# TencentARC/HOSNeRF

Hardware: AMD Instinct MI355X
Metric: train rays/sec (stage3: forward + losses + backward + gradient all-reduce + Adam; LPIPS term OFF in this line -- stages.stage3_with_lpips carries it) (higher is better)
Workload: dtype f32 (fp16/bf16 hi-lo split MFMA x3, fp32 accumulate)

## Files before the change

hosnerf_amd/_lib.py:

```python
from __future__ import annotations

import ctypes
import os
from ctypes import c_char_p, c_float, c_int, c_int64, c_void_p

import torch

_HERE = os.path.dirname(os.path.abspath(__file__))
LIB_PATH = os.environ.get("HOS_LIB_PATH", os.path.join(_HERE, "lib", "libhosrender.so"))


class HosLibraryError(RuntimeError):
    pass


_P, _I, _F, _L = c_void_p, c_int, c_float, c_int64

PROTOTYPES = {
    "hos_version": [],
    "hos_device_count": [],
    "hos_error_string": [_I],
    "hos_set_gemm_mode": [_I],
    "hos_set_thread_gemm_mode": [_I],
    "hos_get_gemm_mode": [],
    "hos_set_range_flag": [_P],
    "hos_linear_fwd": [_P, _I, _I, _P, _I, _I, _P, _I, _P, _P, _I, _I, _I, _I, _P, _I, _F, _F, _P, _P],
    "hos_linear_fwd_splitk": [_P, _I, _P, _I, _P, _I, _I, _I, _I, _P],
    "hos_linear_fwd_splitk_ws_floats": [_I, _I, _I],
    "hos_linear_fwd_splitk_det": [_P, _I, _P, _I, _P, _I, _P, _I, _I, _I, _I, _P, _L, _P],
    "hos_linear_dgrad": [_P, _I, _P, _I, _I, _P, _I, _P, _I, _I, _I, _I, _P],
    "hos_linear_wgrad": [_P, _I, _P, _I, _P, _I, _P, _I, _I, _I, _I, _P],
    "hos_linear_wgrad_rows": [_P, _I, _P, _I, _P, _I, _P, _I, _I, _I, _I, _P, _P],
    "hos_thin_linear_fwd": [_P, _I, _P, _I, _P, _P, _I, _I, _I, _I, _I, _P, _P],
    "hos_thin_linear_dgrad": [_P, _I, _P, _I, _I, _P, _I, _P, _P, _I, _I, _I, _P],
    "hos_thin_linear_fwd_rows": [_P, _I, _P, _I, _P, _P, _I, _I, _I, _I, _I, _P, _P, _P],
    "hos_thin_linear_dgrad_rows": [_P, _I, _P, _I, _I, _P, _I, _P, _P, _I, _I, _I, _P, _P],
    "hos_canonical_fold_pack": [_P, _I, _P, _P, _I, _P, _P, _I, _I, _I, _I, _P, _P, _P, _P, _P],
    "hos_canonical_fold_unfold": [_P, _P, _P, _P, _P, _I, _P, _I, _P, _I, _I, _I, _I, _P, _P, _P, _P, _P, _P],
    "hos_mlp_bwd_defer": [_I],
    "hos_mlp_bwd_flush": [_P],
    "hos_mlp_bwd_ws_floats": [_I, _I, _I, _I],
    "hos_linear_wgrad_tr": [_P, _I, _P, _I, _P, _I, _P, _I, _I, _I, _P, _L, _P],
    "hos_linear_wgrad_tr_rows": [_P, _I, _P, _I, _P, _I, _P, _I, _I, _I, _P, _L, _P, _P],
    "hos_linear_bwd_fused": [_P, _I, _P, _I, _P, _I, _P, _I, _P, _I, _P, _I, _I, _I, _I, _P, _L, _P, _P],
    "hos_stage1_loss_fwd": [_P, _P, _I, _P, _P, _I, _P, _F, _F, _F, _F, _P, _P],
    "hos_stage1_loss_bwd": [_P, _P, _I, _I, _P, _P, _F, _F, _F, _F, _P, _P, _P, _P],
    "hos_lpips_prep": [_P, _L, _P, _P],
    "hos_im2col3x3": [_P, _I, _I, _I, _I, _P, _I, _P],
    "hos_col2im3x3": [_P, _I, _I, _I, _I, _I, _P, _P, _P],
    "hos_maxpool2x2_fwd": [_P, _I, _I, _I, _I, _P, _P],
    "hos_maxpool2x2_bwd": [_P, _P, _I, _I, _I, _I, _P, _P],
    "hos_lpips_head_fwd": [_P, _P, _I, _I, _I, _F, _P, _P],
    "hos_lpips_head_bwd": [_P, _P, _I, _I, _I, _F, _P, _I, _P, _P],
    "hos_lpips_finish": [_P, _I, _P, _P],
    "hos_lpips_part_floats": [_I],
    "hos_bias_relu": [_P, _P, _L, _I, _P],
    "hos_unpack_patches_fwd": [_P, _P, _P, _F, _L, _P, _P],
    "hos_unpack_patches_bwd": [_P, _P, _L, _F, _F, _F, _P, _P],
    "hos_camera_rays": [_P, _P, _P, _I, _I, _P, _P, _P, _P, _P],
    "hos_rays_aabb": [_P, _P, _L, _P, _P, _P, _P, _P],
    "hos_frame_rays_compact": [_P, _P, _P, _P, _I, _I, _P, _P, _P, _P, _P, _P, _P, _P, _P],
    "hos_frame_paint": [_P, _P, _I, _P, _I, _I, _P, _P, _P],
    "hos_raybank_index": [_P, _I, _I, _I, _P, _L, _P, _P, _P, _P],
    "hos_raybank_gather": [_P, _P, _P, _P, _P, _P, _P, _P, _L, _I, _I, _I, _L, _P, _P, _P, _P, _P, _P, _P],
    "hos_raybank_frame": [_P, _F, _I, _I, _L, _L, _P, _P, _P, _P, _P, _P, _P, _P],
    "hos_deconv3d_col2im": [_P, _P, _I, _I, _F, _I, _P, _P],
    "hos_deconv3d_im2col": [_P, _I, _I, _P, _P],
    "hos_bias_lrelu": [_P, _P, _L, _I, _F, _I, _P],
    "hos_shard_interleave": [_P, _I, _I, _I, _P, _P],
    "hos_deconv3d_dpre": [_P, _P, _L, _I, _F, _I, _P, _P, _P],
    "hos_gemv_ws_floats": [_I, _I],
    "hos_gemv_rowvec": [_P, _P, _I, _I, _I, _P, _I, _F, _I, _P, _P, _P],
    "hos_outer_accum": [_P, _I, _P, _I, _P, _I, _I, _I, _I, _P],
    "hos_split_planes": [_P, _I, _I, _I, _I, _P, _I, _P, _I, _P],
    "hos_linearp_fwd": [_P, _I, _I, _P, _I, _I, _P, _I, _P, _I, _I, _I, _P, _I, _P, _I, _P, _P, _I, _I, _P, _I, _F, _P],
    "hos_split_planes_t_batch": [_I, _P, _P, _P, _P, _P, _P, _P],
    "hos_split_planes2": [_P, _I, _I, _I, _P, _I, _P, _I, _P],
    "hos_planes_rowdot": [_P, _I, _I, _P, _P, _F, _I, _L, _P, _P],
    "hos_planes_rowdot_b": [_P, _I, _I, _P, _P, _F, _I, _L, _P, _P],
    "hos_linearp_fwd_b": [_P, _I, _I, _P, _I, _I, _P, _I, _P, _I, _I, _I, _P, _I, _P, _P, _I, _I, _P, _I, _F, _P],
    "hos_linearp_dgrad": [_P, _I, _P, _I, _I, _P, _I, _P, _I, _I, _P, _I, _P],
    "hos_linearp_wgrad": [_P, _I, _P, _I, _I, _P, _I, _P, _I, _I, _I, _I, _P, _L, _P],
    "hos_resample": [_P, _P, _I, _I, _I, _F, _F, _P, _F, _F, _P, _P, _F, _F, _F, _P, _P, _P, _P],
    "hos_encode_ipe": [_P, _P, _P, _P, _P, _P, _I, _I, _P, _I, _P],
    "hos_encode_ipe_planes": [_P, _P, _P, _P, _P, _P, _I, _I, _P, _P, _I, _P],
    "hos_encode_viewdirs": [_P, _I, _I, _P, _I, _I, _P],
    "hos_alpha_weights_fwd": [_P, _P, _P, _I, _I, _I, _P, _P],
    "hos_alpha_weights_bwd": [_P, _P, _P, _P, _I, _I, _I, _P, _P],
    "hos_volrender_fwd": [_P, _P, _I, _I, _F, _P, _P],
    "hos_volrender_bwd": [_P, _P, _P, _I, _I, _F, _P, _P, _P],
    "hos_interlevel_fwd": [_P, _P, _P, _P, _I, _I, _I, _P, _P, _P, _P],
    "hos_interlevel_bwd": [_P, _P, _P, _P, _I, _I, _I, _F, _P, _P],
    "hos_distortion_fwd": [_P, _P, _I, _I, _P, _P],
    "hos_distortion_bwd": [_P, _P, _I, _I, _F, _P, _P],
    "hos_head_grad": [_P, _P, _P, _P, _I, _F, _P, _I, _I, _P, _I, _P],
    "hos_human_sample_warp": [_P, _P, _P, _P, _P, _P, _P, _P, _P, _I, _P, _P, _I, _I, _I, _P, _P, _P, _P, _P],
    "hos_lbs_forward": [_P, _P, _P, _P, _I, _I, _P, _P, _L, _I, _P, _P, _P],
    "hos_embed_hannw": [_P, _P, _I, _P, _I, _L, _P, _I, _P, _I, _P, _P],
    "hos_embed_fourier": [_P, _I, _P, _I, _L, _P, _I, _P, _I, _P],
    "hos_embed_fourier_rows": [_P, _I, _P, _I, _L, _P, _I, _P, _I, _P, _P],
    "hos_human_sample_warp_bwd": [_P, _P, _P, _P, _I, _P, _P, _L, _I, _P, _P, _P, _P, _P, _P, _P, _P, _P],
    "hos_lbs_forward_bwd": [_P, _P, _P, _P, _I, _I, _P, _P, _L, _I, _P, _P, _P, _P, _P, _P, _P],
    "hos_embed_bwd": [_P, _P, _I, _I, _P, _I, _I, _P, _I, _I, _L, _P, _I, _P, _P],
    "hos_slice_mask": [_P, _I, _I, _P, _I, _I, _L, _I, _P, _I, _P, _P],
    "hos_slice_pad": [_P, _I, _I, _L, _I, _P, _I, _P, _P],
    "hos_rgbsigma_grad": [_P, _P, _L, _P, _I, _P],
    "hos_rgbsigma_grad_rows": [_P, _P, _L, _P, _I, _P, _P],
    "hos_raw2outputs_fwd": [_P, _I, _P, _I, _P, _P, _P, _P, _F, _I, _I, _P, _P, _P, _P, _P],
    "hos_raw2outputs_bwd": [_P, _P, _P, _I, _P, _I, _P, _P, _P, _P, _F, _I, _I, _P, _I, _P, _I, _P, _P],
    "hos_merge_composite_fwd": [_P, _P, _P, _P, _P, _P, _P, _P, _P, _P, _I, _I, _I, _F, _P, _P, _P, _P, _P, _P],
    "hos_merge_composite_maps_fwd": [_P, _P, _P, _P, _P, _P, _P, _P, _P, _P, _I, _I, _I, _F, _P, _P, _P, _P, _P, _P, _P, _P, _P, _P],
    "hos_merge_composite_bwd": [_P, _P, _P, _P, _P, _P, _P, _P, _P, _P, _P, _P, _I, _I, _I, _F, _P, _P, _P, _P, _P],
    "hos_mlp_chain_weight_bytes": [],
    "hos_mlp_chain_aux_floats": [],
    "hos_mlp_chain_pack": [_P, _P, _P, _P, _P, _P],
    "hos_mlp_chain_pack_fold": [_P, _P, _P, _P, _I, _I, _P, _P, _P, _P],
    "hos_mlp_chain_unfold_grad": [_P, _P, _P, _I, _I, _P, _I, _P, _P],
    "hos_mlp_chain128_fwd": [_P, _I, _P, _I, _P, _P, _P, _P, _I, _P, _L, _P, _P],
    "hos_mlp_chain_bwd_steps": [_I],
    "hos_mlp_chain_bwd_image_bytes": [_I, _I],
    "hos_mlp_chain_bwd_ws_floats": [_I, _I],
    "hos_mlp_chain_bwd_pack": [_I, _P, _P, _P, _P, _P, _P, _P, _P],
    "hos_mlp_chain_bwd": [_I, _P, _I, _I, _P, _P, _P, _P, _P, _P, _P, _P, _P, _P, _P, _P, _L, _P],
    "hos_compact_workspace_ints": [],
    "hos_compact_rows": [_P, _F, _P, _P, _L, _P, _P, _P, _P, _P, _P],
    "hos_scatter_rows": [_P, _P, _P, _L, _P, _P],
    "hos_select_live_rays": [_P, _F, _I, _I, _P, _P, _P, _P],
    "hos_gather_rays": [_P, _P, _P, _I, _I, _I, _P, _P],
    "hos_scatter_rays": [_P, _P, _P, _P, _I, _I, _I, _P, _P],
    "hos_pose_refine_saved_floats": [],
    "hos_pose_refine_fwd": [_P, _P, _P, _P, _I, _I, _I, _P, _P, _P, _P],
    "hos_pose_refine_workspace_floats": [],
    "hos_pose_refine_bwd": [_P, _P, _P, _P, _P, _P, _P, _I, _I, _I, _P, _P],
    "hos_motion_basis_fwd": [_P, _P, _P, _I, _I, _P, _P, _P, _P, _P],
    "hos_motion_basis_bwd": [_P, _P, _P, _P, _P, _P, _P, _I, _I, _P, _P, _P],
    "hos_train_losses_workspace_floats": [],
    "hos_train_losses_fwd": [_P, _P, _L, _F, _F, _P, _P, _P, _P, _P, _P, _I, _P, _P, _L, _P, _F, _F, _F, _P, _P, _P],
    "hos_train_losses_bwd": [_P, _P, _P, _P, _L, _F, _P, _P, _P, _P, _P, _P, _I, _P, _P, _L, _P, _F, _F, _F, _P, _P, _P, _P, _P],
    "hos_sumsq": [_P, _L, _P, _P],
    "hos_adam_step": [_P, _P, _P, _P, _L, _F, _F, _F, _F, _I, _F, _P, _F, _P],
    "hos_adam_step_dyn": [_P, _P, _P, _P, _L, _P, _F, _F, _F, _F, _P, _F, _P],
    "hos_rowdot_lrelu_fwd": [_P, _P, _I, _P, _I, _I, _F, _P, _P],
    "hos_rowdot_lrelu_bwd": [_P, _P, _P, _P, _I, _I, _I, _F, _P, _I, _P, _P, _P],
    "hos_volume_softmax_fwd": [_P, _P, _I, _L, _P, _P],
    "hos_volume_softmax_bwd": [_P, _P, _I, _L, _P, _P],
    "hos_volume_channel_last": [_P, _I, _L, _P, _P],
    "hos_volume_pair_bwd": [_P, _P, _I, _I, _L, _P, _P],
    "hos_copy_or_zero_n": [_I, _P, _P, _P, _P],
    "hos_debug_stamp": [_P, _I, _P],
    "hos_clear_last_error": [],
    "hos_add_n": [_I, _P, _L, _P, _P],
    "hos_any_abs_below": [_P, _L, _F, _P, _P],
    "hos_state_embed_grad": [_P, _P, _I, _I, _I, _I, _P, _P, _P],
    "hos_embed_bwd_res": [_P, _P, _I, _I, _P, _I, _I, _P, _I, _I, _L, _P, _P, _P, _P],
    "hos_head_grad_padded": [_P, _P, _P, _P, _I, _F, _P, _I, _I, _P, _I, _P],
    "hos_sumsq_blocks": [],
    "hos_sumsq_partials": [_I, _P, _P, _P, _P],
    "hos_adam_multi": [_I, _P, _P, _P, _P, _P, _P, _P, _I, _F, _F, _F, _F, _P, _F, _P, _P, _P],
    "hos_adam_multi_lazy": [_I, _P, _P, _P, _P, _P, _P, _P, _P, _P, _I, _F, _F, _F, _F, _P, _F, _P, _P, _P],
    "hos_adam_lazy_prepare": [_I, _P, _P, _P, _F, _F, _P, _P],
}
_RESTYPES = {"hos_error_string": c_char_p, "hos_mlp_bwd_ws_floats": c_int64, "hos_train_losses_workspace_floats": c_int64,
             "hos_pose_refine_saved_floats": c_int64, "hos_compact_workspace_ints": c_int64,
             "hos_pose_refine_workspace_floats": c_int64, "hos_mlp_chain_weight_bytes": c_int64,
             "hos_mlp_chain_aux_floats": c_int64, "hos_gemv_ws_floats": c_int64,
             "hos_mlp_chain_bwd_image_bytes": c_int64, "hos_mlp_chain_bwd_ws_floats": c_int64,
             "hos_linear_fwd_splitk_ws_floats": c_int64}

_lib = None


def load() -> ctypes.CDLL:
    global _lib
    if _lib is not None:
        return _lib
    if not os.path.exists(LIB_PATH):
        raise HosLibraryError(
            f"{LIB_PATH} not found: build it with `make` (or `python -c 'import __graft_entry__ as g; g.build()'`). "
            "hosnerf_amd has no CPU fallback.")
    try:
        lib = ctypes.CDLL(LIB_PATH)
    except OSError as e:
        raise HosLibraryError(f"cannot load {LIB_PATH}: {e}") from e
    for name, argtypes in PROTOTYPES.items():
        try:
            fn = getattr(lib, name)
        except AttributeError as e:
            raise HosLibraryError(f"{LIB_PATH} does not export {name}; rebuild the library") from e
        fn.argtypes = argtypes
        fn.restype = _RESTYPES.get(name, c_int)
    _lib = lib
    return lib


def check(code: int, what: str):
    if code != 0:
        msg = load().hos_error_string(int(code))
        raise HosLibraryError(f"{what} failed with code {code}: {msg.decode() if msg else '?'}")


def require_gpu():
    if not torch.cuda.is_available():
        raise HosLibraryError("no HIP device visible: hosnerf_amd ops run on MI355X only (no CPU fallback)")


def stream_ptr() -> int:
    return torch.cuda.current_stream().cuda_stream


def ptr(t, dtype=torch.float32) -> int:
    if t is None:
        return 0
    if not isinstance(t, torch.Tensor):
        raise HosLibraryError(f"expected a tensor, got {type(t)}")
    if not t.is_cuda:
        raise HosLibraryError("hosnerf_amd ops take HIP (device='cuda') tensors only -- there is no CPU path")
    if t.dtype != dtype:
        raise HosLibraryError(f"expected dtype {dtype}, got {t.dtype}")
    if not t.is_contiguous():
        raise HosLibraryError("expected a contiguous tensor")
    return t.data_ptr()


def call(name: str, *args):
    lib = load()
    code = getattr(lib, name)(*args, stream_ptr())
    check(code, name)
```

hosnerf_amd/csrc/hos_compact.hip:

```cpp
#include "hos_common.h"

namespace {

constexpr int CT = 256;
constexpr int CPT = 4;
constexpr int CB = CT * CPT;
constexpr int CMAXB = 4096;

__global__ __launch_bounds__(CT) void compact_count_kernel(const float* mask, float thr, long P, int* blk_off, unsigned int* ticket,
                                                          int* count) {
    __shared__ int sh[CT / 64];
    __shared__ bool last;
    const int tid = threadIdx.x;
    const long base = (long)blockIdx.x * CB + tid * CPT;
    int c = 0;
#pragma unroll
    for (int k = 0; k < CPT; ++k) c += (base + k < P && mask[base + k] > thr) ? 1 : 0;
    for (int o = 32; o > 0; o >>= 1) c += __shfl_xor(c, o, 64);
    if ((tid & 63) == 0) sh[tid >> 6] = c;
    __syncthreads();
    if (tid == 0) {
        int tot = 0;
        for (int w = 0; w < CT / 64; ++w) tot += sh[w];
        blk_off[blockIdx.x] = tot;
        __threadfence();
        last = atomicAdd(ticket, 1u) == gridDim.x - 1;
    }
    __syncthreads();
    if (!last) return;
    __threadfence();
    __shared__ int tsum[CT];
    const int nb = gridDim.x, per = (nb + CT - 1) / CT;
    int loc = 0;
    for (int k = 0; k < per; ++k) {
        const int b = tid * per + k;
        if (b < nb) loc += ((volatile int*)blk_off)[b];
    }
    tsum[tid] = loc;
    __syncthreads();
    if (tid == 0) {
        int run = 0;
        for (int t = 0; t < CT; ++t) { const int v = tsum[t]; tsum[t] = run; run += v; }
        *count = run;
        *ticket = 0u;
    }
    __syncthreads();
    int run = tsum[tid];
    for (int k = 0; k < per; ++k) {
        const int b = tid * per + k;
        if (b < nb) { const int v = ((volatile int*)blk_off)[b]; blk_off[b] = run; run += v; }
    }
}

__global__ __launch_bounds__(CT) void compact_scatter_kernel(const float* mask, float thr, long P, const int* blk_off, const int* count,
                                                            const float* src_a, const float* src_b, int* sel, float* out_a, float* out_b) {
    __shared__ int sh[CT / 64];
    const int tid = threadIdx.x, lane = tid & 63, wave = tid >> 6;
    const long base = (long)blockIdx.x * CB + tid * CPT;
    bool f[CPT];
    int c = 0;
#pragma unroll
    for (int k = 0; k < CPT; ++k) { f[k] = base + k < P && mask[base + k] > thr; c += f[k] ? 1 : 0; }
    int incl = c;
    for (int o = 1; o < 64; o <<= 1) { const int n = __shfl_up(incl, o, 64); if (lane >= o) incl += n; }
    if (lane == 63) sh[wave] = incl;
    __syncthreads();
    int pos = blk_off[blockIdx.x] + incl - c;
    for (int w = 0; w < wave; ++w) pos += sh[w];
#pragma unroll
    for (int k = 0; k < CPT; ++k) {
        if (f[k]) {
            const long i = base + k;
            if (sel) sel[pos] = (int)i;
#pragma unroll
            for (int e = 0; e < 3; ++e) {
                if (out_a) out_a[3L * pos + e] = src_a[3 * i + e];
                if (out_b) out_b[3L * pos + e] = src_b[3 * i + e];
            }
            ++pos;
        }
    }
    const int n = *count;
#pragma unroll
    for (int k = 0; k < CPT; ++k) {
        const long i = base + k;
        if (i >= n && i < P) {
            if (sel) sel[i] = -1;
#pragma unroll
            for (int e = 0; e < 3; ++e) {
                if (out_a) out_a[3 * i + e] = 0.f;
                if (out_b) out_b[3 * i + e] = 0.f;
            }
        }
    }
}

__global__ __launch_bounds__(256) void zero_kernel(float* __restrict__ p, long n) {
    for (long i = (long)blockIdx.x * blockDim.x + threadIdx.x; i < n; i += (long)gridDim.x * blockDim.x) p[i] = 0.f;
}

__global__ __launch_bounds__(CT) void scatter_rows_kernel(const float* src, const int* sel, const int* count, long P, float* dst) {
    const long i = (long)blockIdx.x * CT + threadIdx.x;
    if (i >= P) return;
    if (i < *count) {
        const long d = sel[i];
#pragma unroll
        for (int e = 0; e < 3; ++e) dst[3 * d + e] = src[3 * i + e];
    }
}

constexpr int LT = 1024;

__global__ __launch_bounds__(256) void live_flag_kernel(const float* __restrict__ mask, float thr, int B, int S, int* __restrict__ flag) {
    const int lane = threadIdx.x & 63, ray = blockIdx.x * 4 + (threadIdx.x >> 6);
    if (ray >= B) return;
    const bool fg = ray_is_foreground(mask, ray, S, thr, lane);
    if (lane == 0) flag[ray] = fg ? 1 : 0;
}

__global__ __launch_bounds__(LT) void live_scan_kernel(const int* __restrict__ flag, int B, int S, int* __restrict__ ray_ids,
                                                       int* __restrict__ rows_live) {
    __shared__ int wsum[LT / 64];
    __shared__ int total;
    const int t = threadIdx.x, lane = t & 63, wave = t >> 6;
    const int per = (B + LT - 1) / LT;
    const int r0 = t * per;
    int c = 0;
    for (int k = 0; k < per; ++k) c += (r0 + k < B && flag[r0 + k] != 0) ? 1 : 0;
    int incl = c;
    for (int o = 1; o < 64; o <<= 1) { const int n = __shfl_up(incl, o, 64); if (lane >= o) incl += n; }
    if (lane == 63) wsum[wave] = incl;
    __syncthreads();
    int pos = incl - c;
    for (int w = 0; w < wave; ++w) pos += wsum[w];
    if (t == LT - 1) { total = pos + c; *rows_live = (pos + c) * S; }
    for (int k = 0; k < per; ++k)
        if (r0 + k < B && flag[r0 + k] != 0) ray_ids[pos++] = r0 + k;
    __syncthreads();
    const int n = total;
    for (int i = n + t; i < B; i += LT) ray_ids[i] = -1;
}

__global__ __launch_bounds__(256) void gather_rays_kernel(const float* __restrict__ src, const int* __restrict__ ray_ids,
                                                         const int* __restrict__ rows_live, long P, int S, int C, float* __restrict__ dst) {
    const long total = P * C;
    const long live = min((long)*rows_live, P) * C;
    for (long i = (long)blockIdx.x * blockDim.x + threadIdx.x; i < total; i += (long)gridDim.x * blockDim.x) {
        float v = 0.f;
        if (i < live) {
            const long j = i / C;
            const int c = (int)(i - j * C);
            const long ray = ray_ids[j / S];
            v = src[(ray * S + j % S) * C + c];
        }
        dst[i] = v;
    }
}

__global__ __launch_bounds__(256) void scatter_rays_kernel(const float* __restrict__ src, const int* __restrict__ ray_ids,
                                                          const int* __restrict__ flag, const int* __restrict__ rows_live, long P, int S,
                                                          int C, float* __restrict__ dst) {
    const long total = P * C;
    const long live = min((long)*rows_live, P) * C;
    for (long i = (long)blockIdx.x * blockDim.x + threadIdx.x; i < total; i += (long)gridDim.x * blockDim.x) {
        const long j = i / C;
        const int c = (int)(i - j * C);
        if (i < live) {
            const long ray = ray_ids[j / S];
            dst[(ray * S + j % S) * C + c] = src[i];
        }
        if (flag[j / S] == 0) dst[i] = 0.f;
    }
}

inline int rays_grid(long total) {
    long b = (total + 255) / 256;
    return (int)(b > 4096 ? 4096 : (b < 1 ? 1 : b));
}

}

extern "C" int hos_select_live_rays(const float* mask, float thr, int B, int S, int32_t* ray_ids, int32_t* flag, int32_t* rows_live,
                                    hos_stream_t stream) {
    if (!mask || !ray_ids || !flag || !rows_live || B <= 0 || S <= 0) return HOS_E_ARG;
    if ((long long)B * S > 0x7fffffffLL) return HOS_E_SHAPE;
    hipStream_t s = static_cast<hipStream_t>(stream);
    hipLaunchKernelGGL(live_flag_kernel, dim3((unsigned)((B + 3) / 4)), dim3(256), 0, s, mask, thr, B, S, flag);
    hipLaunchKernelGGL(live_scan_kernel, dim3(1), dim3(LT), 0, s, flag, B, S, ray_ids, rows_live);
    return hos_launch_status();
}

extern "C" int hos_gather_rays(const float* src, const int32_t* ray_ids, const int32_t* rows_live, int B, int S, int C, float* dst,
                               hos_stream_t stream) {
    if (!src || !ray_ids || !rows_live || !dst || B <= 0 || S <= 0 || C <= 0) return HOS_E_ARG;
    const long P = (long)B * S;
    hipLaunchKernelGGL(gather_rays_kernel, dim3(rays_grid(P * C)), dim3(256), 0, static_cast<hipStream_t>(stream), src, ray_ids, rows_live,
                       P, S, C, dst);
    return hos_launch_status();
}

extern "C" int hos_scatter_rays(const float* src, const int32_t* ray_ids, const int32_t* flag, const int32_t* rows_live, int B, int S,
                                int C, float* dst, hos_stream_t stream) {
    if (!src || !ray_ids || !flag || !rows_live || !dst || B <= 0 || S <= 0 || C <= 0) return HOS_E_ARG;
    const long P = (long)B * S;
    hipLaunchKernelGGL(scatter_rays_kernel, dim3(rays_grid(P * C)), dim3(256), 0, static_cast<hipStream_t>(stream), src, ray_ids, flag,
                       rows_live, P, S, C, dst);
    return hos_launch_status();
}

extern "C" long long hos_compact_workspace_ints(void) { return CMAXB + 4; }

extern "C" int hos_compact_rows(const float* mask, float thr, const float* src_a, const float* src_b, int64_t P, int32_t* count,
                                int32_t* sel, float* out_a, float* out_b, int32_t* workspace, hos_stream_t stream) {
    if (!mask || !count || !workspace || P <= 0) return HOS_E_ARG;
    if ((out_a && !src_a) || (out_b && !src_b)) return HOS_E_ARG;
    const long nb = (P + CB - 1) / CB;
    if (nb > CMAXB) return HOS_E_SHAPE;
    hipStream_t s = static_cast<hipStream_t>(stream);
    hipLaunchKernelGGL(compact_count_kernel, dim3((unsigned)nb), dim3(CT), 0, s, mask, thr, (long)P, workspace,
                       reinterpret_cast<unsigned int*>(workspace + CMAXB), count);
    hipLaunchKernelGGL(compact_scatter_kernel, dim3((unsigned)nb), dim3(CT), 0, s, mask, thr, (long)P, workspace, count, src_a, src_b,
                       sel, out_a, out_b);
    return hos_launch_status();
}

extern "C" int hos_scatter_rows(const float* src, const int32_t* sel, const int32_t* count, int64_t P, float* dst, hos_stream_t stream) {
    if (!src || !sel || !count || !dst || P <= 0) return HOS_E_ARG;
    hipStream_t s = static_cast<hipStream_t>(stream);
    {
        long blocks = (P * 3 + 255) / 256;
        if (blocks > 2048) blocks = 2048;
        hipLaunchKernelGGL(zero_kernel, dim3((unsigned)blocks), dim3(256), 0, s, dst, (long)P * 3);
    }
    hipLaunchKernelGGL(scatter_rows_kernel, dim3((unsigned)((P + CT - 1) / CT)), dim3(CT), 0, s, src, sel, count, (long)P, dst);
    return hos_launch_status();
}
```

hosnerf_amd/csrc/hos_human.hip:

```cpp
#include "hos_common.h"

constexpr long persist_grid = 768;

namespace {

constexpr int KMAX = 32;

__device__ __forceinline__ float trilinear_zero(const float* __restrict__ vol, int V, float gx, float gy, float gz) {
    const float ix = ((gx + 1.f) / 2.f) * (float)(V - 1);
    const float iy = ((gy + 1.f) / 2.f) * (float)(V - 1);
    const float iz = ((gz + 1.f) / 2.f) * (float)(V - 1);
    const float fx = floorf(ix), fy = floorf(iy), fz = floorf(iz);
    if (!(fx >= -1.f && fx <= (float)V && fy >= -1.f && fy <= (float)V && fz >= -1.f && fz <= (float)V)) return 0.f;
    const int x0 = (int)fx, y0 = (int)fy, z0 = (int)fz;
    const float wx1 = ix - fx, wy1 = iy - fy, wz1 = iz - fz;
    const float wx0 = (fx + 1.f) - ix, wy0 = (fy + 1.f) - iy, wz0 = (fz + 1.f) - iz;
    float out = 0.f;
#pragma unroll
    for (int dz = 0; dz < 2; ++dz)
#pragma unroll
        for (int dy = 0; dy < 2; ++dy)
#pragma unroll
            for (int dx = 0; dx < 2; ++dx) {
                const int x = x0 + dx, y = y0 + dy, z = z0 + dz;
// ... 99 lines not shown
            const float qy = (r[3] * px + r[4] * py + r[5] * pz) + sT[i * 3 + 1];
            const float qz = (r[6] * px + r[7] * py + r[8] * pz) + sT[i * 3 + 2];
            wsum += w[i];
            ax += w[i] * qx; ay += w[i] * qy; az += w[i] * qz;
        }
    }
    const float den = fmaxf(wsum, 1e-4f);
    x_def[p * 3] = ax / den; x_def[p * 3 + 1] = ay / den; x_def[p * 3 + 2] = az / den;
}

__global__ __launch_bounds__(256) void embed_hannw_kernel(const float* __restrict__ x, const float* __restrict__ band_w,
                                                          int F, const float* __restrict__ cond, int C, long P,
                                                          float* __restrict__ E, int lde, float* __restrict__ PE, int ldpe,
                                                          const int* __restrict__ p_dev) {
    if (p_dev) P = min(P, (long)*p_dev);
    const int W = max(lde, PE ? C + ldpe : 0);
    const long total = P * W;
    for (long it = (long)blockIdx.x * blockDim.x + threadIdx.x; it < total; it += (long)gridDim.x * blockDim.x) {
        const long p = it / W;
        const int c = (int)(it % W);
        float v = 0.f;
        const int f = c - C;
        if (c < C) {
            v = cond[c];
        } else if (f < 6 * F) {
            const int j = f / 6, r = f % 6, ax = r % 3;
            const float a = x[p * 3 + ax] * (float)(1 << j);
            v = band_w[j] * ((r < 3) ? sinf(a) : cosf(a));
        }
        if (c < lde) E[p * lde + c] = v;
        if (PE && f >= 0 && f < ldpe) PE[p * ldpe + f] = v;
    }
}

__global__ __launch_bounds__(256) void embed_fourier_kernel(const float* __restrict__ x, int F,
                                                            const float* __restrict__ state, int NE, long P,
                                                            float* __restrict__ E, int lde, float* __restrict__ E2, int lde2,
                                                            const int* __restrict__ p_dev) {
    if (p_dev) P = min(P, (long)*p_dev);
    const long total = P * lde;
    const int nf = 3 + 6 * F;
    for (long it = (long)blockIdx.x * blockDim.x + threadIdx.x; it < total; it += (long)gridDim.x * blockDim.x) {
        const long p = it / lde;
        const int c = (int)(it % lde);
        float v = 0.f;
        if (c < 3) {
            v = x[p * 3 + c];
        } else if (c < nf) {
            const int f = c - 3, j = f / 6, r = f % 6, ax = r % 3;
            const float a = x[p * 3 + ax] * (float)(1 << j);
            v = (r < 3) ? sinf(a) : cosf(a);
        } else if (c < nf + NE) {
            v = state[c - nf];
        }
        E[it] = v;
        if (E2 && c < nf + NE) E2[p * lde2 + c] = v;
    }
}

constexpr int EM_RB = 64;
constexpr int EM_FMAX = 100;

__global__ __launch_bounds__(256) void embed_hannw_tiled_kernel(const float* __restrict__ x, const float* __restrict__ band_w,
                                                                int F, const float* __restrict__ cond, int C, long P,
                                                                float* __restrict__ E, int lde, float* __restrict__ PE, int ldpe,
                                                                const int* __restrict__ p_dev) {
    __shared__ float sF[EM_RB][EM_FMAX + 1];
    if (p_dev) P = min(P, (long)*p_dev);
    const int t = threadIdx.x, nf = 6 * F;
    for (long row0 = (long)blockIdx.x * EM_RB; row0 < P; row0 += (long)gridDim.x * EM_RB) {
        const int rows = (int)min((long)EM_RB, P - row0);
        for (int i = t; i < rows * 3 * F; i += 256) {
            const int r = i / (3 * F), e = i - r * (3 * F);
            const int j = e / 3, ax = e - j * 3;
            const float a = x[(row0 + r) * 3 + ax] * (float)(1 << j);
            float sn, cs;
            sincosf(a, &sn, &cs);
            sF[r][j * 6 + ax] = band_w[j] * sn;
            sF[r][j * 6 + 3 + ax] = band_w[j] * cs;
        }
        __syncthreads();
        const int qe = lde >> 2;
        for (int i = t; i < rows * qe; i += 256) {
            const int r = i / qe, c0 = (i - r * qe) * 4;
            float v[4];
#pragma unroll
            for (int k = 0; k < 4; ++k) {
                const int c = c0 + k, f = c - C;
                v[k] = c < C ? cond[c] : (f < nf ? sF[r][f] : 0.f);
            }
            *reinterpret_cast<float4*>(E + (row0 + r) * lde + c0) = make_float4(v[0], v[1], v[2], v[3]);
        }
        if (PE != nullptr) {
            const int qp = ldpe >> 2;
            for (int i = t; i < rows * qp; i += 256) {
                const int r = i / qp, c0 = (i - r * qp) * 4;
                float v[4];
#pragma unroll
                for (int k = 0; k < 4; ++k) v[k] = (c0 + k < nf) ? sF[r][c0 + k] : 0.f;
                *reinterpret_cast<float4*>(PE + (row0 + r) * ldpe + c0) = make_float4(v[0], v[1], v[2], v[3]);
            }
        }
        __syncthreads();
    }
}

__global__ __launch_bounds__(256) void embed_fourier_tiled_kernel(const float* __restrict__ x, int F,
                                                                  const float* __restrict__ state, int NE, long P,
                                                                  float* __restrict__ E, int lde, float* __restrict__ E2, int lde2,
                                                                  const int* __restrict__ p_dev) {
    __shared__ float sF[EM_RB][EM_FMAX + 1];
    if (p_dev) P = min(P, (long)*p_dev);
    const int t = threadIdx.x, nf = 3 + 6 * F, nv = nf + NE;
    for (long row0 = (long)blockIdx.x * EM_RB; row0 < P; row0 += (long)gridDim.x * EM_RB) {
        const int rows = (int)min((long)EM_RB, P - row0);
        for (int i = t; i < rows * 3 * (F + 1); i += 256) {
            const int r = i / (3 * (F + 1)), e = i - r * (3 * (F + 1));
            if (e < 3) {
                sF[r][e] = x[(row0 + r) * 3 + e];
            } else {
                const int j = (e - 3) / 3, ax = (e - 3) - j * 3;
                const float a = x[(row0 + r) * 3 + ax] * (float)(1 << j);
                float sn, cs;
                sincosf(a, &sn, &cs);
                sF[r][3 + j * 6 + ax] = sn;
                sF[r][3 + j * 6 + 3 + ax] = cs;
            }
        }
        __syncthreads();
        const int qe = lde >> 2;
        for (int i = t; i < rows * qe; i += 256) {
            const int r = i / qe, c0 = (i - r * qe) * 4;
            float v[4];
#pragma unroll
            for (int k = 0; k < 4; ++k) {
                const int c = c0 + k;
                v[k] = c < nf ? sF[r][c] : (c < nv ? state[c - nf] : 0.f);
            }
            *reinterpret_cast<float4*>(E + (row0 + r) * lde + c0) = make_float4(v[0], v[1], v[2], v[3]);
            if (E2 != nullptr && c0 < nv) {
                float* d = E2 + (row0 + r) * lde2 + c0;
                if (c0 + 3 < nv) *reinterpret_cast<float4*>(d) = make_float4(v[0], v[1], v[2], v[3]);
                else {
#pragma unroll
                    for (int k = 0; k < 4; ++k) if (c0 + k < nv) d[k] = v[k];
                }
            }
        }
        __syncthreads();
    }
}

inline bool em_al16(const void* p) { return (reinterpret_cast<uintptr_t>(p) & 15u) == 0; }
inline int em_grid(long P) {
    const long b = (P + EM_RB - 1) / EM_RB;
    return (int)(b > 4096 ? 4096 : (b < 1 ? 1 : b));
}

inline int grid_for(long total) {
    long b = (total + 255) / 256;
    return (int)(b > 8192 ? 8192 : (b < 1 ? 1 : b));
}

}

extern "C" int hos_human_sample_warp(const float* rays_o, const float* rays_d, const float* near_, const float* far_,
                                     const float* t_vals, const float* t_rand, const float* R, const float* T,
                                     const float* vol, int V, const float* bbox_min, const float* bbox_scale,
                                     int B, int N, int K, float* z_vals, float* pts, float* x_skel, float* mask,
                                     hos_stream_t stream) {
    if (!rays_o || !rays_d || !near_ || !far_ || !t_vals || !R || !T || !vol || !bbox_min || !bbox_scale || !x_skel || !mask)
        return HOS_E_ARG;
    if (B <= 0 || N <= 0 || K <= 0 || K > KMAX || V < 2) return HOS_E_SHAPE;
    const long P = (long)B * N;
    hipLaunchKernelGGL(human_sample_warp_kernel, dim3((unsigned)((P + 255) / 256)), dim3(256), 0,
                       static_cast<hipStream_t>(stream), rays_o, rays_d, near_, far_, t_vals, t_rand, R, T, vol, V,
                       bbox_min, bbox_scale, B, N, K, z_vals, pts, x_skel, mask);
    return hos_launch_status();
}

extern "C" int hos_lbs_forward(const float* cnl_pts, const float* R_fwd, const float* T_fwd, const float* vol_cl,
                               int V, int CL, const float* bbox_min, const float* bbox_scale, int64_t P, int K,
                               float* x_deform, const int32_t* rows_dev, hos_stream_t stream) {
    if (!cnl_pts || !R_fwd || !T_fwd || !vol_cl || !bbox_min || !bbox_scale || !x_deform || P <= 0) return HOS_E_ARG;
    if (K <= 0 || K > KMAX || CL < K || (CL & 3) || V < 2) return HOS_E_SHAPE;
    HOS_CHECK_ALIGN16(vol_cl);
    hipLaunchKernelGGL(lbs_forward_kernel, dim3((unsigned)((P + 255) / 256)), dim3(256), 0,
                       static_cast<hipStream_t>(stream), cnl_pts, R_fwd, T_fwd, vol_cl, V, CL, bbox_min, bbox_scale,
                       (long)P, K, x_deform, rows_dev);
    return hos_launch_status();
}

extern "C" int hos_embed_hannw(const float* x, const float* band_w, int num_freqs, const float* cond, int cond_size,
                               int64_t P, float* E, int lde, float* PE, int ldpe, const int32_t* rows_dev, hos_stream_t stream) {
    if (!x || !band_w || !E || P <= 0 || (cond_size > 0 && !cond)) return HOS_E_ARG;
    if (num_freqs < 1 || num_freqs > 16 || lde < cond_size + 6 * num_freqs || (PE && ldpe < 6 * num_freqs)) return HOS_E_SHAPE;
    if (!(lde & 3) && em_al16(E) && (!PE || (!(ldpe & 3) && em_al16(PE))) && 6 * num_freqs <= EM_FMAX) {
        hipLaunchKernelGGL(embed_hannw_tiled_kernel, dim3(em_grid(P)), dim3(256), 0, static_cast<hipStream_t>(stream),
                           x, band_w, num_freqs, cond, cond_size, (long)P, E, lde, PE, ldpe, rows_dev);
        return hos_launch_status();
    }
    hipLaunchKernelGGL(embed_hannw_kernel, dim3(grid_for(P * (lde > cond_size + ldpe ? lde : cond_size + ldpe))), dim3(256), 0, static_cast<hipStream_t>(stream),
                       x, band_w, num_freqs, cond, cond_size, (long)P, E, lde, PE, ldpe, rows_dev);
    return hos_launch_status();
}

extern "C" int hos_embed_fourier_rows(const float* x, int num_freqs, const float* state, int state_size, int64_t P,
                                      float* E, int lde, float* E2, int lde2, const int32_t* rows_dev, hos_stream_t stream) {
    if (!x || !E || P <= 0 || (state_size > 0 && !state)) return HOS_E_ARG;
    if (num_freqs < 1 || num_freqs > 16 || lde < 3 + 6 * num_freqs + state_size) return HOS_E_SHAPE;
    if (E2 && lde2 < 3 + 6 * num_freqs + state_size) return HOS_E_SHAPE;
    if (!(lde & 3) && em_al16(E) && (!E2 || (!(lde2 & 3) && em_al16(E2))) && 3 + 6 * num_freqs <= EM_FMAX) {
        hipLaunchKernelGGL(embed_fourier_tiled_kernel, dim3(em_grid(P)), dim3(256), 0, static_cast<hipStream_t>(stream),
                           x, num_freqs, state, state_size, (long)P, E, lde, E2, lde2, rows_dev);
        return hos_launch_status();
    }
    hipLaunchKernelGGL(embed_fourier_kernel, dim3(grid_for(P * lde)), dim3(256), 0, static_cast<hipStream_t>(stream),
                       x, num_freqs, state, state_size, (long)P, E, lde, E2, lde2, rows_dev);
    return hos_launch_status();
}

extern "C" int hos_embed_fourier(const float* x, int num_freqs, const float* state, int state_size, int64_t P,
                                 float* E, int lde, float* E2, int lde2, hos_stream_t stream) {
    return hos_embed_fourier_rows(x, num_freqs, state, state_size, P, E, lde, E2, lde2, nullptr, stream);
}

namespace {

__device__ __forceinline__ float trilinear_zero_grad(const float* __restrict__ vol, float* __restrict__ g_vol, int V,
                                                     float gx, float gy, float gz, float g_out, float (&dgrid)[3], bool scatter) {
    const int lane = threadIdx.x & 63;
    const float half = 0.5f * (float)(V - 1);
    const float ix = ((gx + 1.f) / 2.f) * (float)(V - 1);
    const float iy = ((gy + 1.f) / 2.f) * (float)(V - 1);
    const float iz = ((gz + 1.f) / 2.f) * (float)(V - 1);
    const float fx = floorf(ix), fy = floorf(iy), fz = floorf(iz);
    dgrid[0] = dgrid[1] = dgrid[2] = 0.f;
    const bool inside = (fx >= -1.f && fx <= (float)V && fy >= -1.f && fy <= (float)V && fz >= -1.f && fz <= (float)V);
    const int x0 = inside ? (int)fx : 0, y0 = inside ? (int)fy : 0, z0 = inside ? (int)fz : 0;
    const float wx1 = ix - fx, wy1 = iy - fy, wz1 = iz - fz;
    const float wx0 = (fx + 1.f) - ix, wy0 = (fy + 1.f) - iy, wz0 = (fz + 1.f) - iz;
    float out = 0.f;
    float contrib[8];
#pragma unroll
    for (int dz = 0; dz < 2; ++dz)
#pragma unroll
        for (int dy = 0; dy < 2; ++dy)
#pragma unroll
            for (int dx = 0; dx < 2; ++dx) {
                const int x = x0 + dx, y = y0 + dy, z = z0 + dz;
                float cw = 0.f;
                if (inside && x >= 0 && x < V && y >= 0 && y < V && z >= 0 && z < V) {
                    const float wx = dx ? wx1 : wx0, wy = dy ? wy1 : wy0, wz = dz ? wz1 : wz0;
                    const size_t idx = ((size_t)z * V + y) * V + x;
                    const float v = vol[idx];
                    out += v * (wx * wy * wz);
                    dgrid[0] += v * (dx ? 1.f : -1.f) * wy * wz;
                    dgrid[1] += v * wx * (dy ? 1.f : -1.f) * wz;
                    dgrid[2] += v * wx * wy * (dz ? 1.f : -1.f);
                    cw = g_out * (wx * wy * wz);
                }
                contrib[dz * 4 + dy * 2 + dx] = cw;
            }
    dgrid[0] *= half; dgrid[1] *= half; dgrid[2] *= half;
    if (g_vol != nullptr) {
        const bool act = scatter && inside && g_out != 0.f;
        const int key = act ? ((z0 + 1) * (V + 2) + (y0 + 1)) * (V + 2) + (x0 + 1) : -1 - lane;
        const int key_prev = __shfl_up(key, 1, 64);
        int flag = (lane == 0 || key != key_prev) ? 1 : 0;
        const int key_next = __shfl_down(key, 1, 64);
        const bool tail = (lane == 63) || (key_next != key);
#pragma unroll
        for (int off = 1; off < 64; off <<= 1) {
            const int f_up = __shfl_up(flag, off, 64);
#pragma unroll
            for (int t = 0; t < 8; ++t) {
                const float v_up = __shfl_up(contrib[t], off, 64);
                if (lane >= off && !flag) contrib[t] += v_up;
            }
            if (lane >= off) flag |= f_up;
        }
        if (act && tail) {
#pragma unroll
            for (int dz = 0; dz < 2; ++dz)
#pragma unroll
                for (int dy = 0; dy < 2; ++dy)
#pragma unroll
                    for (int dx = 0; dx < 2; ++dx) {
                        const int x = x0 + dx, y = y0 + dy, z = z0 + dz;
                        const float cw = contrib[dz * 4 + dy * 2 + dx];
                        if (x >= 0 && x < V && y >= 0 && y < V && z >= 0 && z < V && cw != 0.f)
                            __hip_atomic_fetch_add(g_vol + ((size_t)z * V + y) * V + x, cw, __ATOMIC_RELAXED, __HIP_MEMORY_SCOPE_AGENT);
                    }
        }
    }
    return out;
}

__global__ __launch_bounds__(256) void human_sample_warp_bwd_kernel(
    const float* __restrict__ pts, const float* __restrict__ R, const float* __restrict__ T,
    const float* __restrict__ vol, int V, const float* __restrict__ bbox_min, const float* __restrict__ bbox_scale,
    long P, int K, const float* __restrict__ g_xskel, const float* __restrict__ g_mask,
    float* __restrict__ g_vol, float* __restrict__ g_R, float* __restrict__ g_T, float* __restrict__ aux,
    const float* __restrict__ fwd_xskel, const float* __restrict__ fwd_mask) {
    __shared__ float sR[KMAX * 9], sT[KMAX * 3], sB[6], sAcc[KMAX * 12];
    for (int i = threadIdx.x; i < K * 9; i += blockDim.x) sR[i] = R[i];
    for (int i = threadIdx.x; i < K * 3; i += blockDim.x) sT[i] = T[i];
    for (int i = threadIdx.x; i < K * 12; i += blockDim.x) sAcc[i] = 0.f;
    if (threadIdx.x < 3) { sB[threadIdx.x] = bbox_min[threadIdx.x]; sB[3 + threadIdx.x] = bbox_scale[threadIdx.x]; }
    __syncthreads();
    const long nchunks = (P + 255) / 256;
    for (long chunk = blockIdx.x; chunk < nchunks; chunk += gridDim.x) {
    const long p = chunk * 256 + threadIdx.x;
    const bool live = p < P;
    const long pp = live ? p : P - 1;
    const int lane = threadIdx.x & 63;
    const float px = pts[pp * 3], py = pts[pp * 3 + 1], pz = pts[pp * 3 + 2];
    const size_t V3 = (size_t)V * V * V;
    float wsum, xs, ys, zs;
    if (fwd_xskel != nullptr) {
        wsum = fwd_mask[pp];
        xs = fwd_xskel[pp * 3]; ys = fwd_xskel[pp * 3 + 1]; zs = fwd_xskel[pp * 3 + 2];
    } else {
        float ax = 0.f, ay = 0.f, az = 0.f;
        wsum = 0.f;
        for (int i = 0; i < K; ++i) {
            const float* r = sR + i * 9;
            const float qx = (r[0] * px + r[1] * py + r[2] * pz) + sT[i * 3 + 0];
            const float qy = (r[3] * px + r[4] * py + r[5] * pz) + sT[i * 3 + 1];
            const float qz = (r[6] * px + r[7] * py + r[8] * pz) + sT[i * 3 + 2];
            const float w = trilinear_zero(vol + i * V3, V, (qx - sB[0]) * sB[3] - 1.f, (qy - sB[1]) * sB[4] - 1.f, (qz - sB[2]) * sB[5] - 1.f);
            wsum += w; ax += w * qx; ay += w * qy; az += w * qz;
        }
        const float d0 = fmaxf(wsum, 1e-4f);
        xs = ax / d0; ys = ay / d0; zs = az / d0;
    }
    const float den = fmaxf(wsum, 1e-4f);
    const float clampg = (wsum >= 1e-4f) ? 1.f : 0.f;
    const float gx_ = live ? g_xskel[pp * 3] : 0.f, gy_ = live ? g_xskel[pp * 3 + 1] : 0.f, gz_ = live ? g_xskel[pp * 3 + 2] : 0.f;
    const float gm = live ? g_mask[pp] : 0.f;
    const float gdot_xs = gx_ * xs + gy_ * ys + gz_ * zs;
    if (aux != nullptr && live) { aux[pp * 2] = den; aux[pp * 2 + 1] = clampg * gdot_xs; }
    __shared__ float sQ[256][49];
    __shared__ float sP[256][3];
    sP[threadIdx.x][0] = px; sP[threadIdx.x][1] = py; sP[threadIdx.x][2] = pz;
    for (int i0 = 0; i0 < K; i0 += 16) {
        for (int ii = 0; ii < 16; ++ii) {
            const int i = i0 + ii;
            float gq[3] = {0.f, 0.f, 0.f};
            if (i < K) {
                const float* r = sR + i * 9;
                const float qx = (r[0] * px + r[1] * py + r[2] * pz) + sT[i * 3 + 0];
                const float qy = (r[3] * px + r[4] * py + r[5] * pz) + sT[i * 3 + 1];
                const float qz = (r[6] * px + r[7] * py + r[8] * pz) + sT[i * 3 + 2];
                const float gw = ((gx_ * qx + gy_ * qy + gz_ * qz) - clampg * gdot_xs) / den + gm;
                float dg[3];
                const float w = trilinear_zero_grad(vol + i * V3, g_vol + i * V3, V, (qx - sB[0]) * sB[3] - 1.f,
                                                    (qy - sB[1]) * sB[4] - 1.f, (qz - sB[2]) * sB[5] - 1.f, gw, dg, live);
                gq[0] = gx_ * w / den + gw * dg[0] * sB[3];
                gq[1] = gy_ * w / den + gw * dg[1] * sB[4];
                gq[2] = gz_ * w / den + gw * dg[2] * sB[5];
            }
            sQ[threadIdx.x][ii * 3 + 0] = gq[0]; sQ[threadIdx.x][ii * 3 + 1] = gq[1]; sQ[threadIdx.x][ii * 3 + 2] = gq[2];
        }
        __syncthreads();
        {
            const int e = threadIdx.x & 63, chunk = threadIdx.x >> 6;
            const int bone = i0 + e / 3, comp = e % 3;
            if (e < 48 && bone < K) {
                float a0 = 0.f, a1 = 0.f, a2 = 0.f, a3 = 0.f;
                for (int j = 0; j < 64; ++j) {
                    const int q = chunk * 64 + j;
                    const float v = sQ[q][e];
                    a0 += v * sP[q][0]; a1 += v * sP[q][1]; a2 += v * sP[q][2]; a3 += v;
                }
                atomicAdd(&sAcc[bone * 12 + comp * 3 + 0], a0);
                atomicAdd(&sAcc[bone * 12 + comp * 3 + 1], a1);
                atomicAdd(&sAcc[bone * 12 + comp * 3 + 2], a2);
                atomicAdd(&sAcc[bone * 12 + 9 + comp], a3);
            }
        }
        __syncthreads();
    }
    }
    __syncthreads();
    for (int i = threadIdx.x; i < K * 12; i += blockDim.x) {
        const int b = i / 12, c = i % 12;
        const float v = sAcc[i];
        if (v != 0.f) {
            if (c < 9) __hip_atomic_fetch_add(g_R + b * 9 + c, v, __ATOMIC_RELAXED, __HIP_MEMORY_SCOPE_AGENT);
            else __hip_atomic_fetch_add(g_T + b * 3 + (c - 9), v, __ATOMIC_RELAXED, __HIP_MEMORY_SCOPE_AGENT);
        }
    }
}

__global__ __launch_bounds__(1024) void sample_warp_vol_scatter_kernel(
    const float* __restrict__ pts, const float* __restrict__ R, const float* __restrict__ T, int V,
    const float* __restrict__ bbox_min, const float* __restrict__ bbox_scale, long P,
    const float* __restrict__ g_xskel, const float* __restrict__ g_mask, const float* __restrict__ aux,
    float* __restrict__ g_vol) {
    extern __shared__ float s_gvol[];
    const int i = blockIdx.y;
    const int V3 = V * V * V;
    for (int k = threadIdx.x; k < V3; k += blockDim.x) s_gvol[k] = 0.f;
    float r[9], tt[3], bm[3], bs[3];
#pragma unroll
    for (int k = 0; k < 9; ++k) r[k] = R[i * 9 + k];
#pragma unroll
    for (int k = 0; k < 3; ++k) { tt[k] = T[i * 3 + k]; bm[k] = bbox_min[k]; bs[k] = bbox_scale[k]; }
    __syncthreads();
    const int lane = threadIdx.x & 63;
    const long span = (long)gridDim.x * blockDim.x;
    const long p_end = ((P + span - 1) / span) * span;
    for (long p = (long)blockIdx.x * blockDim.x + threadIdx.x; p < p_end; p += span) {
        const bool live = p < P;
        const long pp = live ? p : P - 1;
        const float px = pts[pp * 3], py = pts[pp * 3 + 1], pz = pts[pp * 3 + 2];
        const float qx = (r[0] * px + r[1] * py + r[2] * pz) + tt[0];
        const float qy = (r[3] * px + r[4] * py + r[5] * pz) + tt[1];
        const float qz = (r[6] * px + r[7] * py + r[8] * pz) + tt[2];
        const float gw = ((g_xskel[pp * 3] * qx + g_xskel[pp * 3 + 1] * qy + g_xskel[pp * 3 + 2] * qz) - aux[pp * 2 + 1]) / aux[pp * 2] + g_mask[pp];
        const float gx = (qx - bm[0]) * bs[0] - 1.f, gy = (qy - bm[1]) * bs[1] - 1.f, gz = (qz - bm[2]) * bs[2] - 1.f;
        const float ix = ((gx + 1.f) / 2.f) * (float)(V - 1), iy = ((gy + 1.f) / 2.f) * (float)(V - 1), iz = ((gz + 1.f) / 2.f) * (float)(V - 1);
        const float fx = floorf(ix), fy = floorf(iy), fz = floorf(iz);
        const bool act = live && gw != 0.f && (fx >= -1.f && fx <= (float)V && fy >= -1.f && fy <= (float)V && fz >= -1.f && fz <= (float)V);
        const int x0 = act ? (int)fx : 0, y0 = act ? (int)fy : 0, z0 = act ? (int)fz : 0;
        const float wx1 = ix - fx, wy1 = iy - fy, wz1 = iz - fz;
        const float wx0 = (fx + 1.f) - ix, wy0 = (fy + 1.f) - iy, wz0 = (fz + 1.f) - iz;
        float contrib[8];
#pragma unroll
        for (int t8 = 0; t8 < 8; ++t8) {
            const int dx = t8 & 1, dy = (t8 >> 1) & 1, dz = t8 >> 2;
            contrib[t8] = act ? gw * ((dx ? wx1 : wx0) * (dy ? wy1 : wy0) * (dz ? wz1 : wz0)) : 0.f;
        }
        const int key = act ? ((z0 + 1) * (V + 2) + (y0 + 1)) * (V + 2) + (x0 + 1) : -1 - lane;
        const int key_prev = __shfl_up(key, 1, 64);
        int flag = (lane == 0 || key != key_prev) ? 1 : 0;
        const int key_next = __shfl_down(key, 1, 64);
        const bool tail = (lane == 63) || (key_next != key);
#pragma unroll
        for (int off = 1; off < 64; off <<= 1) {
            const int f_up = __shfl_up(flag, off, 64);
#pragma unroll
            for (int t8 = 0; t8 < 8; ++t8) {
                const float v_up = __shfl_up(contrib[t8], off, 64);
                if (lane >= off && !flag) contrib[t8] += v_up;
            }
            if (lane >= off) flag |= f_up;
        }
        if (act && tail) {
#pragma unroll
            for (int t8 = 0; t8 < 8; ++t8) {
                const int x = x0 + (t8 & 1), y = y0 + ((t8 >> 1) & 1), z = z0 + (t8 >> 2);
                if (x >= 0 && x < V && y >= 0 && y < V && z >= 0 && z < V && contrib[t8] != 0.f)
                    atomicAdd(&s_gvol[(z * V + y) * V + x], contrib[t8]);
            }
        }
    }
    __syncthreads();
    float* const out = g_vol + (size_t)i * V3;
    for (int k = threadIdx.x; k < V3; k += blockDim.x) {
        const float v = s_gvol[k];
        if (v != 0.f) __hip_atomic_fetch_add(out + k, v, __ATOMIC_RELAXED, __HIP_MEMORY_SCOPE_AGENT);
    }
}

__global__ __launch_bounds__(256) void lbs_forward_bwd_kernel(
    const float* __restrict__ cnl, const float* __restrict__ R, const float* __restrict__ T,
    const float* __restrict__ vol_cl, int V, int CL, const float* __restrict__ bbox_min,
    const float* __restrict__ bbox_scale, long P, int K, const float* __restrict__ g_xdef,
    float* __restrict__ g_cnl, float* __restrict__ g_vol_cl, float* __restrict__ g_R, float* __restrict__ g_T,
    const int* __restrict__ p_dev) {
    __shared__ float sR[KMAX * 9], sT[KMAX * 3], sB[6], sAcc[KMAX * 12];
    if (p_dev) P = min(P, (long)*p_dev);
    for (int i = threadIdx.x; i < K * 9; i += blockDim.x) sR[i] = R[i];
    for (int i = threadIdx.x; i < K * 3; i += blockDim.x) sT[i] = T[i];
    for (int i = threadIdx.x; i < K * 12; i += blockDim.x) sAcc[i] = 0.f;
    if (threadIdx.x < 3) { sB[threadIdx.x] = bbox_min[threadIdx.x]; sB[3 + threadIdx.x] = bbox_scale[threadIdx.x]; }
    __syncthreads();
    const long nchunks = (P + 255) / 256;
    for (long chunk = blockIdx.x; chunk < nchunks; chunk += gridDim.x) {
    const long p = chunk * 256 + threadIdx.x;
    const bool live = p < P;
    const long pp = live ? p : P - 1;
    const int lane = threadIdx.x & 63;
    const float px = cnl[pp * 3], py = cnl[pp * 3 + 1], pz = cnl[pp * 3 + 2];
    const float gx = (px - sB[0]) * sB[3] - 1.f, gy = (py - sB[1]) * sB[4] - 1.f, gz = (pz - sB[2]) * sB[5] - 1.f;
    const float half = 0.5f * (float)(V - 1);
    const float ix = ((gx + 1.f) / 2.f) * (float)(V - 1), iy = ((gy + 1.f) / 2.f) * (float)(V - 1), iz = ((gz + 1.f) / 2.f) * (float)(V - 1);
    const float fx = floorf(ix), fy = floorf(iy), fz = floorf(iz);
    const bool inside = (fx >= -1.f && fx <= (float)V && fy >= -1.f && fy <= (float)V && fz >= -1.f && fz <= (float)V);
    const int x0 = inside ? (int)fx : 0, y0 = inside ? (int)fy : 0, z0 = inside ? (int)fz : 0;
    const float wx1 = ix - fx, wy1 = iy - fy, wz1 = iz - fz;
    const float wx0 = (fx + 1.f) - ix, wy0 = (fy + 1.f) - iy, wz0 = (fz + 1.f) - iz;
    float w[KMAX];
#pragma unroll
    for (int i = 0; i < KMAX; ++i) w[i] = 0.f;
    if (inside) {
        for (int t = 0; t < 8; ++t) {
            const int dx = t & 1, dy = (t >> 1) & 1, dz = t >> 2;
            const int x = x0 + dx, y = y0 + dy, z = z0 + dz;
            if (x >= 0 && x < V && y >= 0 && y < V && z >= 0 && z < V) {
                const float tw = (dx ? wx1 : wx0) * (dy ? wy1 : wy0) * (dz ? wz1 : wz0);
                const float4* vp = reinterpret_cast<const float4*>(vol_cl + (((size_t)z * V + y) * V + x) * CL);
#pragma unroll
                for (int q = 0; q < KMAX / 4; ++q) {
                    if (q * 4 < K) { const float4 v = vp[q]; w[q * 4] += v.x * tw; w[q * 4 + 1] += v.y * tw; w[q * 4 + 2] += v.z * tw; w[q * 4 + 3] += v.w * tw; }
                }
            }
        }
    }
    float wsum = 0.f, ax = 0.f, ay = 0.f, az = 0.f;
#pragma unroll
    for (int i = 0; i < KMAX; ++i) {
        if (i < K) {
            const float* r = sR + i * 9;
            wsum += w[i];
            ax += w[i] * ((r[0] * px + r[1] * py + r[2] * pz) + sT[i * 3 + 0]);
            ay += w[i] * ((r[3] * px + r[4] * py + r[5] * pz) + sT[i * 3 + 1]);
            az += w[i] * ((r[6] * px + r[7] * py + r[8] * pz) + sT[i * 3 + 2]);
        }
    }
    const float den = fmaxf(wsum, 1e-4f);
    const float xd = ax / den, yd = ay / den, zd = az / den;
    const float clampg = (wsum >= 1e-4f) ? 1.f : 0.f;
    const float g0 = live ? g_xdef[pp * 3] : 0.f, g1 = live ? g_xdef[pp * 3 + 1] : 0.f, g2 = live ? g_xdef[pp * 3 + 2] : 0.f;
    const float gdot = g0 * xd + g1 * yd + g2 * zd;
    __shared__ float sGw[256][33];
    __shared__ float sPG[256][6];
    float gw[KMAX];
    float gc[3] = {0.f, 0.f, 0.f};
#pragma unroll
    for (int i = 0; i < KMAX; ++i) {
        gw[i] = 0.f;
        float sfac = 0.f;
        if (i < K) {
            const float* r = sR + i * 9;
            const float qx = (r[0] * px + r[1] * py + r[2] * pz) + sT[i * 3 + 0];
            const float qy = (r[3] * px + r[4] * py + r[5] * pz) + sT[i * 3 + 1];
            const float qz = (r[6] * px + r[7] * py + r[8] * pz) + sT[i * 3 + 2];
            gw[i] = ((g0 * qx + g1 * qy + g2 * qz) - clampg * gdot) / den;
            sfac = w[i] / den;
            const float gq[3] = {g0 * sfac, g1 * sfac, g2 * sfac};
            gc[0] += r[0] * gq[0] + r[3] * gq[1] + r[6] * gq[2];
            gc[1] += r[1] * gq[0] + r[4] * gq[1] + r[7] * gq[2];
            gc[2] += r[2] * gq[0] + r[5] * gq[1] + r[8] * gq[2];
        }
        if (i < 32) sGw[threadIdx.x][i] = sfac;
    }
    sPG[threadIdx.x][0] = px; sPG[threadIdx.x][1] = py; sPG[threadIdx.x][2] = pz;
    sPG[threadIdx.x][3] = g0; sPG[threadIdx.x][4] = g1; sPG[threadIdx.x][5] = g2;
    __syncthreads();
    {
        const int bone = threadIdx.x & 31, chunk = threadIdx.x >> 5;
        if (bone < K) {
            float a[12];
#pragma unroll
            for (int c = 0; c < 12; ++c) a[c] = 0.f;
            for (int j = 0; j < 32; ++j) {
                const int q = chunk * 32 + j;
                const float sf = sGw[q][bone];
                const float qx_ = sPG[q][0], qy_ = sPG[q][1], qz_ = sPG[q][2];
                const float e0 = sPG[q][3] * sf, e1 = sPG[q][4] * sf, e2 = sPG[q][5] * sf;
                a[0] += e0 * qx_; a[1] += e0 * qy_; a[2] += e0 * qz_;
                a[3] += e1 * qx_; a[4] += e1 * qy_; a[5] += e1 * qz_;
                a[6] += e2 * qx_; a[7] += e2 * qy_; a[8] += e2 * qz_;
                a[9] += e0; a[10] += e1; a[11] += e2;
            }
#pragma unroll
            for (int c = 0; c < 12; ++c) atomicAdd(&sAcc[bone * 12 + c], a[c]);
        }
    }
    __syncthreads();
    __shared__ int sBase[256][8];
    __shared__ float sTw[256][8];
    __shared__ int sKey[256];
    {
        const bool act = inside && live;
        sKey[threadIdx.x] = act ? (((z0 + 1) * (V + 2) + (y0 + 1)) * (V + 2) + (x0 + 1)) : -1;
#pragma unroll
        for (int i = 0; i < KMAX; ++i) if (i < 32) sGw[threadIdx.x][i] = (act && i < K) ? gw[i] : 0.f;
        float dgx = 0.f, dgy = 0.f, dgz = 0.f;
        for (int t = 0; t < 8; ++t) {
            const int dx = t & 1, dy = (t >> 1) & 1, dz = t >> 2;
            const int x = x0 + dx, y = y0 + dy, z = z0 + dz;
            int tap_base = -1;
            float tap_w = 0.f;
            if (act && x >= 0 && x < V && y >= 0 && y < V && z >= 0 && z < V) {
                const float wx = dx ? wx1 : wx0, wy = dy ? wy1 : wy0, wz = dz ? wz1 : wz0;
                const size_t base = (((size_t)z * V + y) * V + x) * CL;
                float dot = 0.f;
                for (int i = 0; i < K; ++i) dot += gw[i] * vol_cl[base + i];
                tap_base = (int)base;
                tap_w = wx * wy * wz;
                dgx += dot * (dx ? 1.f : -1.f) * wy * wz;
                dgy += dot * wx * (dy ? 1.f : -1.f) * wz;
                dgz += dot * wx * wy * (dz ? 1.f : -1.f);
            }
            sBase[threadIdx.x][t] = tap_base;
            sTw[threadIdx.x][t] = tap_w;
        }
        if (act) { gc[0] += dgx * half * sB[3]; gc[1] += dgy * half * sB[4]; gc[2] += dgz * half * sB[5]; }
    }
    __syncthreads();
    if (g_vol_cl != nullptr) {
        const int c = lane & 31, hw = lane >> 5, w0 = (threadIdx.x >> 6) * 64 + 32 * hw;
        float run[8];
        int rbase[8];
#pragma unroll
        for (int t = 0; t < 8; ++t) { run[t] = 0.f; rbase[t] = -1; }
        int rkey = -1;
        auto flush = [&]() {
#pragma unroll
            for (int t = 0; t < 8; ++t) {
                if (rbase[t] >= 0 && c < K) __hip_atomic_fetch_add(g_vol_cl + rbase[t] + c, run[t], __ATOMIC_RELAXED, __HIP_MEMORY_SCOPE_AGENT);
                run[t] = 0.f;
            }
        };
        for (int j = 0; j < 32; ++j) {
            const int q = w0 + j;
            const int key = sKey[q];
            if (key != rkey) {
                if (rkey >= 0) flush();
                rkey = key;
#pragma unroll
                for (int t = 0; t < 8; ++t) rbase[t] = sBase[q][t];
            }
            if (key >= 0) {
                const float gv = sGw[q][c];
#pragma unroll
                for (int t = 0; t < 8; ++t) run[t] += gv * sTw[q][t];
            }
        }
        if (rkey >= 0) flush();
    }
    if (live && g_cnl) { g_cnl[pp * 3] = gc[0]; g_cnl[pp * 3 + 1] = gc[1]; g_cnl[pp * 3 + 2] = gc[2]; }
    __syncthreads();
    }
    for (int i = threadIdx.x; i < K * 12; i += blockDim.x) {
        const int b = i / 12, c = i % 12;
        const float v = sAcc[i];
        if (v != 0.f) {
            if (c < 9) __hip_atomic_fetch_add(g_R + b * 9 + c, v, __ATOMIC_RELAXED, __HIP_MEMORY_SCOPE_AGENT);
            else __hip_atomic_fetch_add(g_T + b * 3 + (c - 9), v, __ATOMIC_RELAXED, __HIP_MEMORY_SCOPE_AGENT);
        }
    }
}

__global__ __launch_bounds__(256) void embed_bwd_tiled_kernel(const float* __restrict__ x, const float* __restrict__ band_w, int F,
                                                              int identity, const float* __restrict__ dA, int lda, int colA,
                                                              const float* __restrict__ dB, int ldb, int colB, long P,
                                                              float* __restrict__ g_x, int accumulate, const int* __restrict__ p_dev,
                                                              const float* __restrict__ res) {
    __shared__ float sG[64][101];
    const long P_full = P;
    if (p_dev) P = min(P, (long)*p_dev);
    const int t = threadIdx.x, nf = (identity ? 3 : 0) + 6 * F;
    if (res != nullptr)
        for (long it = P * 3 + (long)blockIdx.x * 256 + t; it < P_full * 3; it += (long)gridDim.x * 256) g_x[it] = res[it];
    for (long row0 = (long)blockIdx.x * 64; row0 < P; row0 += (long)gridDim.x * 64) {
        const int rows = (int)min(64L, P - row0);
        for (int i = t; i < rows * nf; i += 256) {
            const int r = i / nf, c = i - r * nf;
            float v = dA[(row0 + r) * lda + colA + c];
            if (dB) v += dB[(row0 + r) * ldb + colB + c];
            sG[r][c] = v;
        }
        __syncthreads();
        if (t < rows * 3) {
            const int r = t / 3, ax = t - r * 3;
            const long it = (row0 + r) * 3 + ax;
            const float xv = x[it];
            float g = 0.f;
            int base = 0;
            if (identity) { g += sG[r][ax]; base = 3; }
            for (int j = 0; j < F; ++j) {
                const float fr = (float)(1 << j);
                const float a = xv * fr;
                const float wj = band_w ? band_w[j] : 1.f;
                float sn, cs;
                sincosf(a, &sn, &cs);
                g += wj * fr * (cs * sG[r][base + j * 6 + ax] - sn * sG[r][base + j * 6 + 3 + ax]);
            }
            g_x[it] = res != nullptr ? res[it] + g : (accumulate ? g_x[it] + g : g);
        }
        __syncthreads();
    }
}

__global__ __launch_bounds__(256) void slice_mask_kernel(const float* __restrict__ src, int lds, int col0,
                                                         const float* __restrict__ msk, int ldm, int mcol0, long P,
                                                         int width, float* __restrict__ out, int ldo, const int* __restrict__ p_dev) {
    if (p_dev) P = min(P, (long)*p_dev);
    const long total = P * width;
    for (long it = (long)blockIdx.x * blockDim.x + threadIdx.x; it < total; it += (long)gridDim.x * blockDim.x) {
        const long p = it / width;
        const int c = (int)(it % width);
        float v = src[p * lds + col0 + c];
        if (msk && !(msk[p * ldm + mcol0 + c] > 0.f)) v = 0.f;
        out[p * ldo + c] = v;
    }
}

__global__ __launch_bounds__(256) void rgbsigma_grad_kernel(const float* __restrict__ g, const float* __restrict__ y, long P,
                                                            float* __restrict__ out, int ldo, const int* __restrict__ p_dev) {
    if (p_dev) P = min(P, (long)*p_dev);
    const int q = ldo >> 2;
    const long total = P * q;
    for (long it = (long)blockIdx.x * blockDim.x + threadIdx.x; it < total; it += (long)gridDim.x * blockDim.x) {
        const long p = it / q;
        const int c4 = (int)(it % q);
        float4 o = make_float4(0.f, 0.f, 0.f, 0.f);
        if (c4 == 0) {
            const float4 yv = *reinterpret_cast<const float4*>(y + p * 4), gv = *reinterpret_cast<const float4*>(g + p * 4);
            o = make_float4(gv.x * yv.x * (1.f - yv.x), gv.y * yv.y * (1.f - yv.y), gv.z * yv.z * (1.f - yv.z), yv.w > 0.f ? gv.w : 0.f);
        }
        *reinterpret_cast<float4*>(out + p * ldo + c4 * 4) = o;
    }
}

__global__ __launch_bounds__(256) void slice_pad_kernel(const float* __restrict__ src, int lds, int col0, long P, int width,
                                                        float* __restrict__ out, int ldo, const int* __restrict__ p_dev) {
    if (p_dev) P = min(P, (long)*p_dev);
    const int q = ldo >> 2;
    const long total = P * q;
    for (long it = (long)blockIdx.x * blockDim.x + threadIdx.x; it < total; it += (long)gridDim.x * blockDim.x) {
        const long p = it / q;
        const int c4 = (int)(it % q);
        float v[4] = {0.f, 0.f, 0.f, 0.f};
        if (c4 == 0) {
#pragma unroll
            for (int c = 0; c < 4; ++c) if (c < width) v[c] = src[p * lds + col0 + c];
        }
        *reinterpret_cast<float4*>(out + p * ldo + c4 * 4) = make_float4(v[0], v[1], v[2], v[3]);
    }
}

}

extern "C" int hos_human_sample_warp_bwd(const float* pts, const float* R, const float* T, const float* vol, int V,
                                         const float* bbox_min, const float* bbox_scale, int64_t P, int K,
                                         const float* g_x_skel, const float* g_mask, float* g_vol, float* g_R,
                                         float* g_T, float* scratch, const float* fwd_x_skel, const float* fwd_mask,
                                         hos_stream_t stream) {
    if (!pts || !R || !T || !vol || !bbox_min || !bbox_scale || !g_x_skel || !g_mask || !g_vol || !g_R || !g_T || P <= 0)
        return HOS_E_ARG;
    if (K <= 0 || K > KMAX || V < 2) return HOS_E_SHAPE;
    hipStream_t s = static_cast<hipStream_t>(stream);
    const long sw_chunks = (P + 255) / 256;
    const dim3 grid((unsigned)(sw_chunks < persist_grid ? sw_chunks : persist_grid));
    const size_t vol_bytes = (size_t)V * V * V * sizeof(float);
    const bool split = scratch != nullptr && vol_bytes <= 128 * 1024 && P >= 8192;
    hipLaunchKernelGGL(human_sample_warp_bwd_kernel, grid, dim3(256), 0, s, pts, R, T, vol, V, bbox_min, bbox_scale, (long)P, K,
                       g_x_skel, g_mask, split ? (float*)nullptr : g_vol, g_R, g_T, split ? scratch : (float*)nullptr,
                       (fwd_x_skel && fwd_mask) ? fwd_x_skel : (const float*)nullptr, (fwd_x_skel && fwd_mask) ? fwd_mask : (const float*)nullptr);
    if (split) {
        static bool attr_set = false;
        if (!attr_set) {
            hipError_t e = hipFuncSetAttribute(reinterpret_cast<const void*>(&sample_warp_vol_scatter_kernel),
                                               hipFuncAttributeMaxDynamicSharedMemorySize, 128 * 1024);
            if (e != hipSuccess) return (int)e;
            attr_set = true;
        }
        const int nb = 256 / K > 0 ? 256 / K : 1;
        hipLaunchKernelGGL(sample_warp_vol_scatter_kernel, dim3(nb, K), dim3(1024), vol_bytes, s, pts, R, T, V, bbox_min,
                           bbox_scale, (long)P, g_x_skel, g_mask, scratch, g_vol);
    }
    return hos_launch_status();
}

extern "C" int hos_lbs_forward_bwd(const float* cnl_pts, const float* R_fwd, const float* T_fwd, const float* vol_cl,
                                   int V, int CL, const float* bbox_min, const float* bbox_scale, int64_t P, int K,
                                   const float* g_x_deform, float* g_cnl, float* g_vol_cl, float* g_R, float* g_T,
                                   const int32_t* rows_dev, hos_stream_t stream) {
    if (!cnl_pts || !R_fwd || !T_fwd || !vol_cl || !bbox_min || !bbox_scale || !g_x_deform || !g_R || !g_T || P <= 0)
        return HOS_E_ARG;
    if (K <= 0 || K > KMAX || CL < K || (CL & 3) || V < 2) return HOS_E_SHAPE;
    const long lb_chunks = (P + 255) / 256;
    hipLaunchKernelGGL(lbs_forward_bwd_kernel, dim3((unsigned)(lb_chunks < persist_grid ? lb_chunks : persist_grid)), dim3(256), 0,
                       static_cast<hipStream_t>(stream), cnl_pts, R_fwd, T_fwd, vol_cl, V, CL, bbox_min, bbox_scale,
                       (long)P, K, g_x_deform, g_cnl, g_vol_cl, g_R, g_T, rows_dev);
    return hos_launch_status();
}

static int embed_bwd_launch(const float* x, const float* band_w, int num_freqs, int identity, const float* dA, int lda,
                            int colA, const float* dB, int ldb, int colB, int64_t P, float* g_x, int accumulate,
                            const int32_t* rows_dev, const float* res, hos_stream_t stream);

extern "C" int hos_embed_bwd(const float* x, const float* band_w, int num_freqs, int identity, const float* dA, int lda,
                             int colA, const float* dB, int ldb, int colB, int64_t P, float* g_x, int accumulate,
                             const int32_t* rows_dev, hos_stream_t stream) {
    return embed_bwd_launch(x, band_w, num_freqs, identity, dA, lda, colA, dB, ldb, colB, P, g_x, accumulate, rows_dev, nullptr, stream);
}

extern "C" int hos_embed_bwd_res(const float* x, const float* band_w, int num_freqs, int identity, const float* dA, int lda,
                                 int colA, const float* dB, int ldb, int colB, int64_t P, const float* res, float* g_x,
                                 const int32_t* rows_dev, hos_stream_t stream) {
    if (!res) return HOS_E_ARG;
    return embed_bwd_launch(x, band_w, num_freqs, identity, dA, lda, colA, dB, ldb, colB, P, g_x, 0, rows_dev, res, stream);
}

static int embed_bwd_launch(const float* x, const float* band_w, int num_freqs, int identity, const float* dA, int lda,
                            int colA, const float* dB, int ldb, int colB, int64_t P, float* g_x, int accumulate,
                            const int32_t* rows_dev, const float* res, hos_stream_t stream) {
    if (!x || !dA || !g_x || P <= 0) return HOS_E_ARG;
    if (num_freqs < 1 || num_freqs > 16) return HOS_E_SHAPE;
    const long b = (P + 63) / 64;
    hipLaunchKernelGGL(embed_bwd_tiled_kernel, dim3((unsigned)(b > 8192 ? 8192 : b)), dim3(256), 0, static_cast<hipStream_t>(stream), x,
                       band_w, num_freqs, identity, dA, lda, colA, dB, ldb, colB, (long)P, g_x, accumulate, rows_dev, res);
    return hos_launch_status();
}

extern "C" int hos_slice_mask(const float* src, int lds, int col0, const float* mask_src, int ldm, int mcol0, int64_t P,
                              int width, float* out, int ldo, const int32_t* rows_dev, hos_stream_t stream) {
    if (!src || !out || P <= 0 || width <= 0) return HOS_E_ARG;
    hipLaunchKernelGGL(slice_mask_kernel, dim3(grid_for(P * width)), dim3(256), 0, static_cast<hipStream_t>(stream), src, lds,
                       col0, mask_src, ldm, mcol0, (long)P, width, out, ldo, rows_dev);
    return hos_launch_status();
}

extern "C" int hos_rgbsigma_grad_rows(const float* g_rgbsigma, const float* rgbsigma, int64_t P, float* dz, int ldz,
                                      const int32_t* rows_dev, hos_stream_t stream) {
    if (!g_rgbsigma || !rgbsigma || !dz || P <= 0 || ldz < 4) return HOS_E_ARG;
    if ((ldz & 3) || (((uintptr_t)g_rgbsigma | (uintptr_t)rgbsigma | (uintptr_t)dz) & 15u)) return HOS_E_ALIGN;
    hipLaunchKernelGGL(rgbsigma_grad_kernel, dim3(grid_for(P * (ldz >> 2))), dim3(256), 0, static_cast<hipStream_t>(stream),
                       g_rgbsigma, rgbsigma, (long)P, dz, ldz, rows_dev);
    return hos_launch_status();
}

extern "C" int hos_rgbsigma_grad(const float* g_rgbsigma, const float* rgbsigma, int64_t P, float* dz, int ldz,
                                 hos_stream_t stream) {
    return hos_rgbsigma_grad_rows(g_rgbsigma, rgbsigma, P, dz, ldz, nullptr, stream);
}

extern "C" int hos_slice_pad(const float* src, int lds, int col0, int64_t P, int width, float* out, int ldo,
                             const int32_t* rows_dev, hos_stream_t stream) {
    if (!src || !out || P <= 0 || width <= 0) return HOS_E_ARG;
    if (width > 4 || ldo < 4) return HOS_E_SHAPE;
    if ((ldo & 3) || ((uintptr_t)out & 15u)) return HOS_E_ALIGN;
    hipLaunchKernelGGL(slice_pad_kernel, dim3(grid_for(P * (ldo >> 2))), dim3(256), 0, static_cast<hipStream_t>(stream), src, lds,
                       col0, (long)P, width, out, ldo, rows_dev);
    return hos_launch_status();
}
```

hosnerf_amd/human_nerf.py:

```python
from __future__ import annotations

import json
import math
import os
from types import SimpleNamespace
from typing import Dict, List, Optional

import numpy as np
import torch
import torch.nn as nn
import torch.nn.functional as F

from . import ops
from .flat import FlatModule, FlatStore, Region
from .mipnerf360 import select_state, _Lin

SMPL_PARENT = {1: 0, 2: 0, 3: 0, 4: 1, 5: 2, 6: 3, 7: 4, 8: 5, 9: 6, 10: 7, 11: 8, 12: 9, 13: 9, 14: 9, 15: 12,
               16: 13, 17: 14, 18: 16, 19: 17, 20: 18, 21: 19, 22: 20, 23: 21, 24: 23, 25: 22}


class Cfg(dict):

    def __getattr__(self, k):
        try:
# ... 423 lines not shown
        ops.embed_hannw(x, band_w, cond.reshape(-1), E, PE, rows_dev=rows_dev)
        if chain:
            key = id(specs)
            bufs = self._chain_bufs.get(key)
            if bufs is None or bufs[0].device != dev:
                bufs = self._chain_bufs[key] = ops.mlp_chain_buffers(dev)
            ws = [self._w(L) for L in specs]
            ops.mlp_chain_pack([w for w, _ in ws], [b_ for _, b_ in ws], bufs[0], bufs[1])
            acts = [torch.empty(Pn, 128, device=dev) for _ in range(6)]
            xyz = torch.empty(Pn, 3, device=dev)
            ops.mlp_chain128_fwd(E, PE, x, bufs[0], bufs[1], acts, xyz, rows_dev=rows_dev)
            return xyz, ((E, PE, acts, None) if save else None)
        acts = []
        h = E
        for i in range(6):
            L = specs[i]
            Wt, bt = self._w(L)
            out = torch.empty(Pn, 128, device=dev)
            if i == 4:
                ops.linear_fwd(h, 128, Wt, bt, 128, out, ops.EPI_RELU, A1=PE, K1=NR_LDPE, rows_dev=rows_dev)
            else:
                ops.linear_fwd(h, L.Kpad, Wt, bt, 128, out, ops.EPI_RELU, rows_dev=rows_dev)
            acts.append(out)
            h = out
        Wt, bt = self._w(specs[6])
        xyz = torch.empty(Pn, 3, device=dev)
        ops.linear_fwd(h, 128, Wt, bt, 3, xyz, ops.EPI_RESIDUAL, aux=x, rows_dev=rows_dev)
        return xyz, ((E, PE, acts, None) if save else None)

    def _canonical_fwd(self, cnl: torch.Tensor, state: int, save: bool, rows_dev=None):
        Pn = cnl.shape[0]
        dev = cnl.device
        embed = self._embeds.view(self.store.param)[state]
        fold = None
        if rows_dev is not None and not ops.thin_dgrad_rows(Pn):
            raise ValueError("_canonical_fwd(rows_dev=...): the row bound exists on the thin-kernel path only (ops.thin_dgrad_rows)")
        if ops.CNL_FOLD and ops.thin_dgrad_rows(Pn):
            fkey = ("cnl_fold",) + ops._stream_key(dev)
            fb = self._chain_bufs.get(fkey)
            if fb is None:
                fb = self._chain_bufs[fkey] = torch.empty(256 * (2 * CNL_NFP + 256 + 2), device=dev)
            fw = ops.cnl_fold_views(fb, 256, CNL_NFP, 256)
            (W0, b0), (W5, b5) = self._w(self._cnl[0]), self._w(self._cnl[5])
            ops.canonical_fold_pack(W0, b0, W5, b5, embed, 256, CNL_NF, 256, fw)
            E = torch.empty(Pn, CNL_NFP, device=dev)
            CAT = torch.empty(Pn, CNL_NFP + 256, device=dev)
            ops.embed_fourier(cnl, 10, ops.zero1(dev), E, CAT, rows_dev=rows_dev)
            fold = (fw, embed)
        else:
            E = torch.empty(Pn, CNL_LDE, device=dev)
            CAT = torch.empty(Pn, CNL_CAT, device=dev)
            CAT[:, CNL_CAT - 1].zero_()
            ops.embed_fourier(cnl, 10, embed, E, CAT, rows_dev=rows_dev)
        acts, bits = [], []
        h = E
        want_bits = save and ops.thin_dgrad_rows(Pn)
        for i in range(8):
            L = self._cnl[i]
            Wt, bt = self._w(L)
            K = L.Kpad
            if fold is not None and i in (0, 5):
                Wt, bt = (fold[0][0], fold[0][1]) if i == 0 else (fold[0][2], fold[0][3])
                K = Wt.shape[1]
            rb = ops.thin_relu_bits(Pn, dev) if (want_bits and K <= 320) else None
            if i == 4:
                ops.linear_fwd(h, K, Wt, bt, 256, CAT, ops.EPI_RELU, out_col0=CNL_NFP if fold is not None else 127, relu_bits=rb,
                               rows_dev=rows_dev)
                acts.append(CAT)
                h = CAT
            else:
                out = torch.empty(Pn, 256, device=dev)
                ops.linear_fwd(h, K, Wt, bt, 256, out, ops.EPI_RELU, relu_bits=rb, rows_dev=rows_dev)
                acts.append(out)
                h = out
            bits.append(rb)
        Wt, bt = self._w(self._cnl[8])
        raw = torch.empty(Pn, 4, device=dev)
        ops.linear_fwd(h, 256, Wt, bt, 4, raw, ops.EPI_SIGMOID_RELU4, rows_dev=rows_dev)
        return raw, ((E, acts, bits, fold) if save else None)

    def _nonrigid_bwd(self, specs: List[_LayerSpec], saved, x: torch.Tensor, band_w: torch.Tensor, g_xyz: torch.Tensor, rows_dev=None):
        E, PE, acts, fold = saved
        Pn, dev = x.shape[0], x.device

        def layer_bwd(dz, X, spec, N, K, out, relu_mask, w_col0=0, bias=True, override=None):
            if override is not None:
                Wt, gW, gb = override
            else:
                Wt, _ = self._w(spec)
                gW, gb = self._w(spec, grad=True)
            ops.linear_bwd_fused(dz, X, Wt, gW, gb if bias else None, N, K, out, relu_mask, w_col0=w_col0, rows_dev=rows_dev)
            return out

        dz6 = torch.empty(Pn, 32, device=dev)
        ops.slice_pad(g_xyz, 0, 3, dz6, rows_dev=rows_dev)
        if fold is not None:
            gfold = ops.zero_(ops.fold_grad_workspace(dev))
            gw0h, db0 = gfold[:128 * 64].view(128, 64), gfold[128 * 64:]
        if (fold is not None and ops.MLP_CHAIN_BWD and Pn >= ops.MLP_CHAIN_BWD_MIN_ROWS
                and ops.get_gemm_mode() != ops.GEMM_FP32):
            Wm = [self._w(L)[0] for L in specs]
            G = [self._w(L, grad=True) for L in specs]
            im = ops.mlp_chain_bwd_images(id(specs), (0, 1, 2), dev)
            ops.mlp_chain_bwd_pack([
                (0, 0, Wm[6], 0, 3, 128, im[0][0]), (0, 1, Wm[5], 0, 128, 128, im[0][1]),
                (1, 0, Wm[4], 128, 128, NR_LDPE, im[1][0]), (1, 1, Wm[4], 0, 128, 128, im[1][1]), (1, 2, Wm[3], 0, 128, 128, im[1][2]),
                (2, 0, Wm[2], 0, 128, 128, im[2][0]), (2, 1, Wm[1], 0, 128, 128, im[2][1]), (2, 2, fold[0], 0, 128, NR_LDPE, im[2][2])])
            dPE = torch.empty(Pn, NR_LDPE, device=dev)
            dE = torch.empty(Pn, NR_LDPE, device=dev)
            dz4 = torch.empty(Pn, 128, device=dev)
            dz2 = torch.empty(Pn, 128, device=dev)
            with ops.deferred_bwd_reduce():
                ops.mlp_chain_bwd(0, dz6, [acts[5], acts[4]], im[0], [None, dz4], [G[6][0], G[5][0]], [0, 0], [G[6][1], G[5][1]],
                                  [3, 128], [128, 128], rows_dev=rows_dev)
                ops.mlp_chain_bwd(1, dz4, [PE, acts[3], acts[2]], im[1], [dPE, None, dz2], [G[4][0], G[4][0], G[3][0]], [128, 0, 0],
                                  [None, G[4][1], G[3][1]], [128, 128, 128], [NR_LDPE, 128, 128], rows_dev=rows_dev)
                ops.mlp_chain_bwd(2, dz2, [acts[1], acts[0], PE], im[2], [None, None, dE], [G[2][0], G[1][0], gw0h], [0, 0, 0],
                                  [G[2][1], G[1][1], db0], [128, 128, 128], [128, 128, NR_LDPE], rows_dev=rows_dev)
            res = g_xyz.contiguous()
            gW0, gb0 = self._w(specs[0], grad=True)
            ops.mlp_chain_unfold_grad(gw0h, db0, fold[1], 6 * band_w.numel(), gW0, gb0)
            return ops.embed_bwd_res(x, band_w, band_w.numel(), False, dE, 0, dPE, 0, res, rows_dev=rows_dev)
        with ops.deferred_bwd_reduce():
            dz = layer_bwd(dz6, acts[5], specs[6], 3, 128, torch.empty(Pn, 128, device=dev), True)
            dPE = dE = None
            for i in range(5, -1, -1):
                if i == 4:
                    dPE = layer_bwd(dz, PE, specs[4], 128, NR_LDPE, torch.empty(Pn, NR_LDPE, device=dev), False, w_col0=128, bias=False)
                    dz = layer_bwd(dz, acts[3], specs[4], 128, 128, torch.empty(Pn, 128, device=dev), True)
                elif i == 0 and fold is not None:
                    dE = layer_bwd(dz, PE, specs[0], 128, NR_LDPE, torch.empty(Pn, NR_LDPE, device=dev), False, override=(fold[0], gw0h, db0))
                elif i == 0:
                    dE = layer_bwd(dz, E, specs[0], 128, NR_LDE, torch.empty(Pn, NR_LDE, device=dev), False)
                else:
                    dz = layer_bwd(dz, acts[i - 1], specs[i], 128, 128, torch.empty(Pn, 128, device=dev), True)
        res = g_xyz.contiguous()
        if fold is not None:
            gW0, gb0 = self._w(specs[0], grad=True)
            ops.mlp_chain_unfold_grad(gw0h, db0, fold[1], 6 * band_w.numel(), gW0, gb0)
            return ops.embed_bwd_res(x, band_w, band_w.numel(), False, dE, 0, dPE, 0, res, rows_dev=rows_dev)
        return ops.embed_bwd_res(x, band_w, band_w.numel(), False, dE, 75, dPE, 0, res, rows_dev=rows_dev)

    def _canonical_bwd(self, saved, cnl: torch.Tensor, raw: torch.Tensor, g_raw: torch.Tensor, state: int, rows_dev=None):
        E, acts, bits, fold = saved
        rd = rows_dev
        CAT = acts[4]
        Pn, dev = cnl.shape[0], cnl.device
        dz8 = torch.empty(Pn, 32, device=dev)
        ops.rgbsigma_grad(g_raw.contiguous(), raw, dz8, rows_dev=rd)
        Wt, _ = self._w(self._cnl[8])
        gW, gb = self._w(self._cnl[8], grad=True)
        ops.linear_wgrad(dz8, acts[7], gW, gb, 4, 256, rows_dev=rd)
        dz = torch.empty(Pn, 256, device=dev)
        ops.linear_dgrad(dz8, Wt, 32, 256, dz, mask_src=acts[7], mask_bits=bits[7], rows_dev=rd)
        dCAT = dE = None
        tmp_b = {}
        if fold is not None:
            gws = ops.zero_(ops.cnl_fold_grad_workspace(dev, 256, CNL_NFP, 256))
            gfold = ops.cnl_fold_views(gws, 256, CNL_NFP, 256)
        with ops.deferred_bwd_reduce():
            for i in range(7, -1, -1):
                L = self._cnl[i]
                Wt, _ = self._w(L)
                gW, gb = self._w(L, grad=True)
                if i == 5 and fold is not None:
                    W5f = fold[0][2]
                    ops.linear_wgrad(dz, CAT, gfold[2], gfold[3], 256, CNL_NFP + 256, rows_dev=rd)
                    nxt = torch.empty(Pn, 256, device=dev)
                    dCAT = torch.empty(Pn, CNL_NFP, device=dev)
                    ops.linear_dgrad(dz, W5f, 256, CNL_NFP, dCAT, thin=True, rows_dev=rd)
                    ops.linear_dgrad(dz, W5f, 256, 256, nxt, mask_src=CAT, w_col0=CNL_NFP, mask_col0=CNL_NFP, mask_bits=bits[4], rows_dev=rd)
                    dz = nxt
                elif i == 0 and fold is not None:
                    ops.linear_wgrad(dz, E, gfold[0], gfold[1], 256, CNL_NFP, rows_dev=rd)
                    dE = torch.empty(Pn, CNL_NFP, device=dev)
                    ops.linear_dgrad(dz, fold[0][0], 256, CNL_NFP, dE, thin=True, rows_dev=rd)
                elif i == 5:
                    tmp_b[5] = ops.zeros(L.Npad, dev)
                    ops.linear_wgrad(dz, CAT, gW, tmp_b[5], 256, CNL_CAT, rows_dev=rd)
                    nxt = torch.empty(Pn, 256, device=dev)
                    if ops.thin_dgrad_rows(Pn):
                        dCAT = torch.empty(Pn, 64, device=dev)
                        ops.linear_dgrad(dz, Wt, 256, 64, dCAT, thin=True, rows_dev=rd)
                        ops.linear_dgrad(dz, Wt, 256, 256, nxt, mask_src=CAT, w_col0=127, mask_col0=127, mask_bits=bits[4], rows_dev=rd)
                    else:
                        dCAT = torch.empty(Pn, CNL_CAT, device=dev)
                        ops.linear_dgrad(dz, Wt, 256, CNL_CAT, dCAT, rows_dev=rd)
                        ops.slice_mask(dCAT, 127, CAT, 127, 256, nxt, rows_dev=rd)
                    dz = nxt
                elif i == 0:
                    tmp_b[0] = ops.zeros(L.Npad, dev)
                    ops.linear_wgrad(dz, E, gW, tmp_b[0], 256, CNL_LDE, rows_dev=rd)
                    dE = torch.empty(Pn, CNL_LDE, device=dev)
                    ops.linear_dgrad(dz, Wt, 256, CNL_LDE, dE, rows_dev=rd)
                else:
                    inp = acts[i - 1]
                    ops.linear_wgrad(dz, inp, gW, gb, 256, 256, rows_dev=rd)
                    nxt = torch.empty(Pn, 256, device=dev)
                    ops.linear_dgrad(dz, Wt, 256, 256, nxt, mask_src=inp, mask_bits=bits[i - 1], rows_dev=rd)
                    dz = nxt
        g_embed = self._embeds.view(self.store.grad)[state]
        if fold is not None:
            (W0, _), (W5, _) = self._w(self._cnl[0]), self._w(self._cnl[5])
            (gW0, gb0), (gW5, gb5) = self._w(self._cnl[0], grad=True), self._w(self._cnl[5], grad=True)
            ops.canonical_fold_unfold(gfold, W0, W5, fold[1], 256, CNL_NF, 256, gW0, gb0, gW5, gb5, g_embed)
        else:
            for i in (0, 5):
                Wt, _ = self._w(self._cnl[i])
                _, gb = self._w(self._cnl[i], grad=True)
                gb += tmp_b[i]
                g_embed.addmv_(Wt[:256, 63:127].t(), tmp_b[i][:256])
        g_cnl = torch.empty(Pn, 3, device=dev)
        ops.embed_bwd(cnl, None, 10, True, dE, 0, dCAT, 0, g_cnl, False, rows_dev=rd)
        return g_cnl

    def frame_prologue(self, dst_Rs, dst_Ts, cnl_gtfms, motion_weights_priors, dst_posevec=None, iter_val=1e7, **kwargs):
        cfg = self.cfg
        K = cfg.total_bones
        iter_v = float(torch.as_tensor(iter_val).reshape(-1)[0])
        time = float(kwargs["time"])
        is_train = bool(kwargs["is_train"])
        flow = time > 0.005 and is_train
        nr_kick = cfg.non_rigid_motion_mlp.kick_in_iter

        def cond_of(pv):
            return torch.zeros_like(pv) * pv if iter_v < nr_kick else pv

        if flow and dst_Rs.is_cuda and not (dst_Rs.requires_grad or dst_Ts.requires_grad or dst_posevec.requires_grad):
            nR, nT, nP = dst_Rs.numel(), dst_Ts.numel(), dst_posevec.numel()
            pad4 = lambda n: (2 * n + 3) // 4 * 4
            buf = torch.empty(pad4(nR) + pad4(nT) + pad4(nP), device=dst_Rs.device)
            Rs = buf[:2 * nR].view((2,) + tuple(dst_Rs.shape))
            Ts = buf[pad4(nR):pad4(nR) + 2 * nT].view((2,) + tuple(dst_Ts.shape))
            pv = buf[pad4(nR) + pad4(nT):pad4(nR) + pad4(nT) + 2 * nP].view(2, nP)
            c = lambda t_: t_.detach().float().contiguous()
            ops.copy_or_zero_n([Rs[0], Rs[1], Ts[0], Ts[1], pv[0], pv[1]],
                               [c(dst_Rs), c(kwargs["dst_Rs_prev"]), c(dst_Ts), c(kwargs["dst_Ts_prev"]), c(dst_posevec).reshape(-1),
                                c(kwargs["dst_posevec_prev"]).reshape(-1)])
        elif flow:
            Rs = torch.stack([dst_Rs, kwargs["dst_Rs_prev"]], 0)
            Ts = torch.stack([dst_Ts, kwargs["dst_Ts_prev"]], 0)
            pv = torch.stack([dst_posevec.reshape(-1), kwargs["dst_posevec_prev"].reshape(-1)], 0)
        else:
            Rs, Ts, pv = dst_Rs[None], dst_Ts[None], dst_posevec.reshape(1, -1)
        if iter_v >= cfg.pose_decoder.get("kick_in_iter", 0):
            Rs, Ts = self._pose_refine(Rs, Ts, pv)
        Rb_, Tb_, Rf_, Tf_ = self._motion_basis(Rs, Ts, cnl_gtfms)
        vol = self._motion_weight_volume(motion_weights_priors)
        if self.split_decoder_backward and torch.is_grad_enabled() and vol.requires_grad:
            self._fwd_stream = torch.cuda.current_stream(vol.device) if vol.is_cuda else None
            leaf = vol.detach().requires_grad_(True)
            self._pending_vol = (vol, leaf)
            vol = leaf
        Rb, Tb, Rf, Tf = ops.unbind_frames_many(Rb_, Tb_, Rf_, Tf_)
        vol, vol_cl = ops.volume_pair(vol, K)
        pro = {"flow": flow, "state": select_state(time, self.transitions_times), "R_b": Rb[0], "T_b": Tb[0],
               "R_f": Rf[0], "T_f": Tf[0], "band_w": self._band_weights(iter_v, dst_Rs.device),
               "cond": cond_of(dst_posevec).contiguous(), "vol": vol, "vol_cl": vol_cl}
        if flow:
            pro.update(R_fp=Rf[1], T_fp=Tf[1], cond_prev=cond_of(kwargs["dst_posevec_prev"]).contiguous())
        return pro

    def forward(self, rays, dst_Rs=None, dst_Ts=None, cnl_gtfms=None, motion_weights_priors=None, dst_posevec=None, near=None,
                far=None, iter_val=1e7, t_rand=None, prologue=None, with_cycle: bool = True, static_cycle: bool = False,
                live_rays: bool = False, **kwargs):
        return ops.guarded_forward(self, rays.device, lambda: self._forward(
            rays, dst_Rs, dst_Ts, cnl_gtfms, motion_weights_priors, dst_posevec, near, far, iter_val, t_rand, prologue, with_cycle,
            static_cycle, live_rays, **kwargs))

    def _forward(self, rays, dst_Rs=None, dst_Ts=None, cnl_gtfms=None, motion_weights_priors=None, dst_posevec=None, near=None,
                 far=None, iter_val=1e7, t_rand=None, prologue=None, with_cycle: bool = True, static_cycle: bool = False,
                 live_rays: bool = False, **kwargs):
        cfg = self.cfg
        dev = rays.device
        K = cfg.total_bones
        pro = prologue if prologue is not None else self.frame_prologue(
            dst_Rs, dst_Ts, cnl_gtfms, motion_weights_priors, dst_posevec=dst_posevec, iter_val=iter_val, **kwargs)
        flow, state, band_w, cond, vol, vol_cl = pro["flow"], pro["state"], pro["band_w"], pro["cond"], pro["vol"], pro["vol_cl"]
        R_b, T_b, R_f, T_f = pro["R_b"], pro["T_b"], pro["R_f"], pro["T_f"]
        if flow:
            R_fp, T_fp, cond_prev = pro["R_fp"], pro["T_fp"], pro["cond_prev"]
        bmin = kwargs["cnl_bbox_min_xyz"].contiguous()
        bscale = kwargs["cnl_bbox_scale_xyz"].contiguous()

        rays_o = rays[0].reshape(-1, 3).float().contiguous()
        rays_d = rays[1].reshape(-1, 3).float().contiguous()
        B = rays_o.shape[0]
        N = cfg.N_samples
        if t_rand is None and cfg.perturb > 0.0:
            t_rand = torch.rand(B, N, device=dev)
        outs: Dict[str, List[torch.Tensor]] = {}
        chunk = int(cfg.chunk)
        live_rays = bool(live_rays and self.stage == 3 and B <= chunk and torch.is_grad_enabled() and ops.thin_dgrad_rows(B * N))
        for c0 in range(0, B, chunk):
            sl = slice(c0, min(B, c0 + chunk))
            tr = None if t_rand is None else t_rand[sl].contiguous()
            grad = torch.is_grad_enabled()
            live = rows_live = None
            if live_rays:
                z, pts, x_skel, mask = ops.human_sample_warp_ad(vol, R_b, T_b, rays_o[sl], rays_d[sl], near[sl].contiguous(),
                                                                far[sl].contiguous(), N, bmin, bscale, tr, K)
                live = ops.select_live_rays(mask.detach().view(-1, N))
                rows_live = live.rows
                x_c = ops.gather_rays(x_skel.reshape(-1, 3), live)
                mask_c = ops.gather_rays(mask.detach().reshape(-1, 1), live).view(-1)
                pts_c = ops.gather_rays(pts.detach().reshape(-1, 3), live)
                cnl = _NonRigidFn.apply(self._token, self, "nr", x_c, cond, band_w, rows_live)
                n_use = 1 + int(flow) + int(with_cycle)
                cnl_uses = list(ops.fanout(cnl, n_use))
                raw = ops.scatter_rays(_CanonicalFn.apply(self._token, self, cnl_uses.pop(), state, rows_live), live)
            elif grad:
                z, pts, x_skel, mask = ops.human_sample_warp_ad(vol, R_b, T_b, rays_o[sl], rays_d[sl], near[sl].contiguous(),
                                                                far[sl].contiguous(), N, bmin, bscale, tr, K)
                cnl = _NonRigidFn.apply(self._token, self, "nr", x_skel, cond, band_w, None)
                n_use = 1 + int(flow) + int(with_cycle)
                cnl_uses = list(ops.fanout(cnl, n_use))
                raw = _CanonicalFn.apply(self._token, self, cnl_uses.pop(), state)
            else:
                z, pts, x_skel, mask = ops.human_sample_warp(rays_o[sl], rays_d[sl], near[sl].contiguous(), far[sl].contiguous(),
                                                             N, R_b, T_b, vol, bmin, bscale, tr, K)
                cnl, _ = self._nonrigid_fwd(self._nr, x_skel, cond, band_w, save=False)
                cnl_uses = [cnl, cnl, cnl]
                raw, _ = self._canonical_fwd(cnl, state, save=False)
            b = z.shape[0]
            if self.stage == 2:
                rgb_map, acc_map, weights, depth_map = ops.raw2outputs(raw.view(b, N, 4), z, rays_d[sl], mask.view(b, N),
                                                                       kwargs["bgcolor"].to(dev))
                ret = {"rgb": rgb_map, "alpha": acc_map, "depth": depth_map, "weights": weights}
            else:
                ret = {"human_rgb": raw[:, :3].reshape(b, N, 3), "human_density": raw[:, 3].reshape(b, N),
                       "human_rgbsigma": raw.view(b, N, 4), "newsmpl_pts": pts, "pts_mask": mask.view(b, N)}

            def fwd_branch(c_pts, Rf_, Tf_, cond_, rows_dev=None):
                if grad:
                    d_ = ops.lbs_forward_ad(c_pts, vol_cl, Rf_, Tf_, bmin, bscale, K, rows_dev=rows_dev)
                    return _NonRigidFn.apply(self._token, self, "nrf", d_, cond_, band_w, rows_dev)
                d_ = ops.lbs_forward(c_pts, Rf_, Tf_, vol_cl, bmin, bscale, K, rows_dev=rows_dev)
                return self._nonrigid_fwd(self._nrf, d_, cond_, band_w, save=False, rows_dev=rows_dev)[0]

            if flow and live is not None:
                ret["deform_pts_prev_final"] = ops.scatter_rays(fwd_branch(cnl_uses.pop(), R_fp, T_fp, cond_prev, rows_dev=rows_live),
                                                                live).view(b, N, 3)
            elif flow:
                ret["deform_pts_prev_final"] = fwd_branch(cnl_uses.pop(), R_fp, T_fp, cond_prev).view(b, N, 3)
            cyc_mask, cyc_pts = (mask_c, pts_c) if live is not None else (mask, pts)
            if with_cycle and static_cycle:
                if B > chunk:
                    raise ValueError("static_cycle needs the whole ray batch in one chunk (cfg.chunk >= number of rays)")
                sel_cnl, observe, _, count = ops.compact_rows(cyc_mask, 0.005, cnl_uses.pop(), cyc_pts)
                ret["deform_pts_final"] = fwd_branch(sel_cnl, R_f, T_f, cond, rows_dev=count)
                ret["observe_pts"] = observe
                ret["cycle_count"] = count
                if live is not None:
                    ret["live_ray_rows"] = rows_live
            elif with_cycle:
                sel = torch.nonzero(cyc_mask.detach().reshape(-1) > 0.005).reshape(-1)
                if sel.numel() > 0:
                    ret["deform_pts_final"] = fwd_branch(cnl_uses.pop().index_select(0, sel), R_f, T_f, cond)
                    ret["observe_pts"] = cyc_pts.view(-1, 3).index_select(0, sel)
                else:
                    ret["deform_pts_final"] = pts[0, 0][None]
                    ret["observe_pts"] = pts[0, 0][None]
            if not flow and self.stage != 2:
                ret["z_vals"] = z
                ret["rays_d"] = rays_d[sl]
            for k, v in ret.items():
                outs.setdefault(k, []).append(v)
        all_ret = {k: (v[0] if len(v) == 1 else torch.cat(v, 0)) for k, v in outs.items()}
        if self.stage != 2:
            all_ret["bgcolor"] = kwargs.get("bgcolor")
        return all_ret


class _NonRigidFn(torch.autograd.Function):

    @staticmethod
    def forward(ctx, token, net: Network, which: str, x, cond, band_w, rows_dev=None):
        specs = net._nr if which == "nr" else net._nrf
        x = x.contiguous()
        xyz, saved = net._nonrigid_fwd(specs, x, cond, band_w, save=True, rows_dev=rows_dev)
        ctx.net, ctx.specs, ctx.saved, ctx.x, ctx.band_w, ctx.rows_dev = net, specs, saved, x, band_w, rows_dev
        ctx.mode = ops.get_gemm_mode()
        return xyz

    @staticmethod
    def backward(ctx, g):
        with ops.gemm_mode(ctx.mode):
            g_x = ctx.net._nonrigid_bwd(ctx.specs, ctx.saved, ctx.x, ctx.band_w, g.contiguous(), rows_dev=ctx.rows_dev)
        ctx.saved = None
        return None, None, None, g_x, None, None, None


class _CanonicalFn(torch.autograd.Function):
    @staticmethod
    def forward(ctx, token, net: Network, cnl, state, rows_dev=None):
        cnl = cnl.contiguous()
        raw, saved = net._canonical_fwd(cnl, state, save=True, rows_dev=rows_dev)
        ctx.net, ctx.saved, ctx.cnl, ctx.raw, ctx.state, ctx.rows_dev = net, saved, cnl, raw, state, rows_dev
        ctx.mode = ops.get_gemm_mode()
        return raw

    @staticmethod
    def backward(ctx, g):
        with ops.gemm_mode(ctx.mode):
            g_cnl = ctx.net._canonical_bwd(ctx.saved, ctx.cnl, ctx.raw, g.contiguous(), ctx.state, rows_dev=ctx.rows_dev)
        ctx.saved = ctx.raw = None
        return None, None, g_cnl, None, None
```

hosnerf_amd/ops.py:

```python
from __future__ import annotations

import os
import threading

import math
from typing import Optional, Tuple

import numpy as np
import torch

from . import _lib
from ._lib import call, ptr

EPS = 1.1920929e-07

EPI_NONE, EPI_RELU, EPI_DENSITY, EPI_RGB, EPI_NERF_HEAD, EPI_SIGMOID_RELU4, EPI_RESIDUAL = 0, 1, 2, 3, 4, 5, 6


def round_up(x: int, m: int) -> int:
    return (x + m - 1) // m * m


class KernelEvents:

# ... 984 lines not shown


def sumsq_partials(spans, partial: torch.Tensor):
    import ctypes
    call("hos_sumsq_partials", len(spans), _table([ptr(t) for t in spans]), _table([t.numel() for t in spans], ctypes.c_longlong), ptr(partial))


def adam_multi(spans, step: int, beta1: float, beta2: float, eps: float, grad_scale: float, partial, max_norm: float, guard=(None, None)):
    import ctypes
    n = len(spans)
    col = lambda i: _table([ptr(sp[i]) for sp in spans])
    lazy = _table([ptr(sp[6]) if len(sp) > 6 else None for sp in spans]) if any(len(sp) > 6 and sp[6] is not None for sp in spans) else None
    rows = _table([int(sp[7]) if len(sp) > 7 and sp[7] else 0 for sp in spans], ctypes.c_int) if lazy is not None else None
    call("hos_adam_multi_lazy", n, col(0), col(1), col(2), col(3), _table([sp[0].numel() for sp in spans], ctypes.c_longlong),
         col(4), lazy, rows, _table([float(sp[5]) for sp in spans], ctypes.c_float), int(step), float(beta1), float(beta2), float(eps),
         float(grad_scale), ptr(partial), float(max_norm), ptr(guard[0], torch.int32), ptr(guard[1], torch.int32))


def adam_lazy_prepare(grads, states, beta1: float, beta2: float, guard=None):
    import ctypes
    for i in range(0, len(grads), 32):
        g_, s_ = grads[i:i + 32], states[i:i + 32]
        call("hos_adam_lazy_prepare", len(g_), _table([ptr(g) for g in g_]), _table([g.numel() for g in g_], ctypes.c_longlong),
             _table([ptr(s) for s in s_]), float(beta1), float(beta2), ptr(guard, torch.int32))


def adam_step(p, g, m, v, lr, beta1, beta2, eps, step, grad_scale=1.0, sumsq_buf=None, max_norm=0.0):
    call("hos_adam_step", ptr(p), ptr(g), ptr(m), ptr(v), p.numel(), float(lr), float(beta1), float(beta2),
         float(eps), int(step), float(grad_scale), ptr(sumsq_buf), float(max_norm))


_T_CACHE = {}


def _t_vals(N: int, device) -> torch.Tensor:
    key = (N, str(device))
    if key not in _T_CACHE:
        _T_CACHE[key] = torch.linspace(0.0, 1.0, steps=N).to(device)
    return _T_CACHE[key]


def human_sample_warp(rays_o, rays_d, near, far, N: int, R, T, vol, bbox_min, bbox_scale, t_rand=None, K: int = 26):
    B = rays_o.shape[0]
    dev = rays_o.device
    z = torch.empty(B, N, device=dev)
    pts = torch.empty(B, N, 3, device=dev)
    x_skel = torch.empty(B * N, 3, device=dev)
    mask = torch.empty(B * N, device=dev)
    V = vol.shape[-1]
    call("hos_human_sample_warp", ptr(rays_o), ptr(rays_d), ptr(near.reshape(-1)), ptr(far.reshape(-1)),
         ptr(_t_vals(N, dev)), ptr(None if t_rand is None else t_rand.reshape(-1)), ptr(R), ptr(T), ptr(vol), V,
         ptr(bbox_min), ptr(bbox_scale), B, N, K, ptr(z), ptr(pts), ptr(x_skel), ptr(mask))
    return z, pts, x_skel, mask


def lbs_forward(cnl_pts, R_f, T_f, vol_cl, bbox_min, bbox_scale, K: int = 26, rows_dev=None):
    P = cnl_pts.shape[0]
    out = torch.empty(P, 3, device=cnl_pts.device)
    V, CL = vol_cl.shape[0], vol_cl.shape[-1]
    call("hos_lbs_forward", ptr(cnl_pts), ptr(R_f), ptr(T_f), ptr(vol_cl), V, CL, ptr(bbox_min), ptr(bbox_scale), P, K, ptr(out),
         ptr(rows_dev, torch.int32))
    return out


def embed_hannw(x, band_w, cond, E, PE=None, rows_dev=None):
    P = x.shape[0]
    call("hos_embed_hannw", ptr(x), ptr(band_w), band_w.numel(), ptr(cond), 0 if cond is None else cond.numel(), P,
         ptr(E), E.stride(0), ptr(PE), 0 if PE is None else PE.stride(0), ptr(rows_dev, torch.int32))


def embed_fourier(x, num_freqs, state, E, E2=None, rows_dev=None):
    P = x.shape[0]
    call("hos_embed_fourier_rows", ptr(x), num_freqs, ptr(state), 0 if state is None else state.numel(), P,
         ptr(E), E.stride(0), ptr(E2), 0 if E2 is None else E2.stride(0), ptr(rows_dev, torch.int32))


class _Raw2Outputs(torch.autograd.Function):

    @staticmethod
    def forward(ctx, rgbsigma, z_vals, rays_d, mask, bgcolor, last_dist):
        B, S = z_vals.shape
        dev = z_vals.device
        rgb = torch.empty(B, 3, device=dev)
        acc = torch.empty(B, device=dev)
        w = torch.empty(B, S, device=dev)
        depth = torch.empty(B, device=dev)
        call("hos_raw2outputs_fwd", ptr(rgbsigma), 4, ptr(rgbsigma) + 12, 4, ptr(z_vals), ptr(rays_d), ptr(mask), ptr(bgcolor),
             float(last_dist), B, S, ptr(rgb), ptr(acc), ptr(w), ptr(depth))
        ctx.save_for_backward(rgbsigma, z_vals, rays_d, mask, bgcolor)
        ctx.last_dist = float(last_dist)
        ctx.mark_non_differentiable(acc, depth)
        ctx.set_materialize_grads(False)
        return rgb, acc, w, depth

    @staticmethod
    def backward(ctx, g_rgb, g_acc, g_w, g_depth):
        rgbsigma, z_vals, rays_d, mask, bgcolor = ctx.saved_tensors
        B, S = z_vals.shape
        g_rs = torch.empty_like(rgbsigma)
        g_mask = torch.empty(B, S, device=z_vals.device) if mask is not None else None
        g_rgb = zeros((rgbsigma.shape[0], 3), rgbsigma.device) if g_rgb is None else g_rgb.contiguous()
        g_w = None if g_w is None else g_w.contiguous()
        call("hos_raw2outputs_bwd", ptr(g_rgb), ptr(g_w), ptr(rgbsigma), 4,
             ptr(rgbsigma) + 12, 4, ptr(z_vals), ptr(rays_d), ptr(mask), ptr(bgcolor), ctx.last_dist, B, S,
             ptr(g_rs), 4, ptr(g_rs) + 12, 4, ptr(g_mask))
        return g_rs, None, None, g_mask, None, None


def raw2outputs(rgbsigma, z_vals, rays_d, mask=None, bgcolor=None, last_dist: float = 1e10):
    return _Raw2Outputs.apply(rgbsigma.contiguous(), z_vals.contiguous(), rays_d.contiguous(),
                              None if mask is None else mask.contiguous(),
                              None if bgcolor is None else bgcolor.contiguous().float(), last_dist)


class _MergeComposite(torch.autograd.Function):
    @staticmethod
    def forward(ctx, bkg_rgb, bkg_density, human_rgbsigma, pts_mask, bkg_tdist, pts, rays_o, rays_d, A, tiny_flag, thre_fg):
        B, Sb = bkg_density.shape
        Sh = pts_mask.shape[1]
        dev = bkg_density.device
        rgb = torch.empty(B, 3, device=dev)
        idx_fg = torch.empty(B, dtype=torch.int32, device=dev)
        order = torch.empty(B, Sb + Sh, dtype=torch.int32, device=dev)
        hw = torch.empty(B, Sh, device=dev)
        zh = torch.empty(B, Sh, device=dev)
        call("hos_merge_composite_fwd", ptr(bkg_tdist), ptr(bkg_rgb), ptr(bkg_density), ptr(human_rgbsigma), ptr(pts),
             ptr(pts_mask), ptr(rays_o), ptr(rays_d), ptr(A), ptr(tiny_flag, torch.int32), B, Sb, Sh, float(thre_fg),
             ptr(rgb), ptr(idx_fg, torch.int32), ptr(order, torch.int32), ptr(hw), ptr(zh))
        ctx.save_for_backward(bkg_rgb, bkg_density, human_rgbsigma, pts_mask, bkg_tdist, pts, rays_o, rays_d, A, tiny_flag)
        ctx.thre = float(thre_fg)
        ctx.mark_non_differentiable(idx_fg, order, zh)
        ctx.set_materialize_grads(False)
        return rgb, hw, idx_fg, order, zh

    @staticmethod
    def backward(ctx, g_rgb, g_hw, *_):
        bkg_rgb, bkg_density, human, mask, tdist, pts, ro, rd, A, flag = ctx.saved_tensors
        B, Sb = bkg_density.shape
        Sh = mask.shape[1]
        g_brgb = torch.empty_like(bkg_rgb)
        g_bden = torch.empty_like(bkg_density)
        g_h = torch.empty_like(human)
        g_m = torch.empty_like(mask)
        g_rgb = zeros((B, 3), mask.device) if g_rgb is None else g_rgb.contiguous()
        g_hw = None if g_hw is None else g_hw.contiguous()
        call("hos_merge_composite_bwd", ptr(g_rgb), ptr(g_hw),
             ptr(tdist), ptr(bkg_rgb), ptr(bkg_density), ptr(human), ptr(pts), ptr(mask), ptr(ro), ptr(rd), ptr(A),
             ptr(flag, torch.int32), B, Sb, Sh, ctx.thre, ptr(g_brgb), ptr(g_bden), ptr(g_h), ptr(g_m))
        return g_brgb, g_bden, g_h, g_m, None, None, None, None, None, None, None


def merge_composite(bkg_tdist, bkg_rgb, bkg_density, human_rgbsigma, newsmpl_pts, pts_mask, rays_o_bkg, rays_d_bkg,
                    newsmpl_to_scale_world, thre_fg: float = 5e-3):
    rd = rays_d_bkg.contiguous()
    tiny = torch.empty(1, dtype=torch.int32, device=rd.device)
    call("hos_any_abs_below", ptr(rd), rd.numel(), 1e-5, ptr(tiny, torch.int32))
    return _MergeComposite.apply(bkg_rgb.contiguous(), bkg_density.contiguous(), human_rgbsigma.contiguous(),
                                 pts_mask.contiguous(), bkg_tdist.contiguous(), newsmpl_pts.contiguous(),
                                 rays_o_bkg.contiguous(), rd, newsmpl_to_scale_world.contiguous().float(), tiny, thre_fg)


MAP_KEYS = ("acc", "depth", "rgb_human", "acc_human", "rgb_bkg", "acc_bkg")


def merge_composite_maps(bkg_tdist, bkg_rgb, bkg_density, human_rgbsigma, newsmpl_pts, pts_mask, rays_o_bkg, rays_d_bkg,
                         newsmpl_to_scale_world, thre_fg: float = 5e-3, want=MAP_KEYS):
    unknown = [k for k in want if k not in MAP_KEYS]
    if unknown:
        raise ValueError(f"merge_composite_maps: unknown map(s) {unknown}; choose from {MAP_KEYS}")
    det = lambda t: t.detach().contiguous()
    rd = det(rays_d_bkg)
    dev = rd.device
    B, Sb = bkg_density.shape
    Sh = pts_mask.shape[1]
    tiny = torch.empty(1, dtype=torch.int32, device=dev)
    call("hos_any_abs_below", ptr(rd), rd.numel(), 1e-5, ptr(tiny, torch.int32))
    out = {"rgb": torch.empty(B, 3, device=dev), "idx_fg": torch.empty(B, dtype=torch.int32, device=dev),
           "total_order": torch.empty(B, Sb + Sh, dtype=torch.int32, device=dev)}
    for k in want:
        out[k] = torch.empty((B, 3) if k.startswith("rgb") else (B,), device=dev)
    tens = [det(t) for t in (bkg_tdist, bkg_rgb, bkg_density, human_rgbsigma, newsmpl_pts, pts_mask, rays_o_bkg)]
    A = det(newsmpl_to_scale_world).float()
    call("hos_merge_composite_maps_fwd", *[ptr(t) for t in tens], ptr(rd), ptr(A), ptr(tiny, torch.int32), B, Sb, Sh,
         float(thre_fg), ptr(out["rgb"]), ptr(out["idx_fg"], torch.int32), ptr(out["total_order"], torch.int32),
         *[ptr(out.get(k)) for k in MAP_KEYS])
    return out


POSE_PARAM_ORDER = ("block_mlps.0", "block_mlps.2", "block_mlps.4", "block_mlps_dstR.0", "block_mlps_dstR.2", "block_mlps_dstT.0",
                    "block_mlps_dstT.2")


def _ptr_array(tensors):
    import ctypes
    return (ctypes.c_void_p * len(tensors))(*[ptr(t) for t in tensors])


class _PoseRefine(torch.autograd.Function):

    @staticmethod
    def forward(ctx, token, Rs, Ts, posevec, weights, grads):
        F_, K = Rs.shape[0], Rs.shape[1]
        Rs, Ts, posevec = Rs.contiguous(), Ts.contiguous(), posevec.contiguous()
        Ro, To = torch.empty_like(Rs), torch.empty_like(Ts)
        saved = torch.empty(F_, int(_lib.load().hos_pose_refine_saved_floats()), device=Rs.device)
        width = weights[0].shape[0]
        call("hos_pose_refine_fwd", ptr(posevec), ptr(Rs), ptr(Ts), _ptr_array(weights), F_, K, width, ptr(Ro), ptr(To), ptr(saved))
        ctx.save_for_backward(Rs, posevec, saved)
        ctx.weights, ctx.grads, ctx.dims = weights, grads, (F_, K, width)
        return Ro, To

    @staticmethod
    def backward(ctx, gR, gT):
        Rs, posevec, saved = ctx.saved_tensors
        F_, K, width = ctx.dims
        gR = zeros(tuple(Rs.shape), Rs.device) if gR is None else gR.contiguous()
        gT = zeros((F_, K, 3), Rs.device) if gT is None else gT.contiguous()
        ws = torch.empty(F_, int(_lib.load().hos_pose_refine_workspace_floats()), device=Rs.device)
        call("hos_pose_refine_bwd", ptr(gR), ptr(gT), ptr(posevec), ptr(Rs), ptr(saved), _ptr_array(ctx.weights), _ptr_array(ctx.grads),
             F_, K, width, ptr(ws))
        return None, None, None, None, None, None


def pose_refine(token, Rs, Ts, posevec, weights, grads):
    return _PoseRefine.apply(token, Rs, Ts, posevec, list(weights), list(grads))


class _MotionBasis(torch.autograd.Function):

    @staticmethod
    def forward(ctx, Rs, Ts, cnl_gtfms):
        F_, K = Rs.shape[0], Rs.shape[1]
        Rs, Ts, cnl = Rs.contiguous(), Ts.contiguous(), cnl_gtfms.contiguous()
        dev = Rs.device
        Rb, Tb = torch.empty(F_, K, 3, 3, device=dev), torch.empty(F_, K, 3, device=dev)
        Rf, Tf = torch.empty(F_, K, 3, 3, device=dev), torch.empty(F_, K, 3, device=dev)
        call("hos_motion_basis_fwd", ptr(Rs), ptr(Ts), ptr(cnl), F_, K, ptr(Rb), ptr(Tb), ptr(Rf), ptr(Tf))
        ctx.save_for_backward(Rs, Ts, cnl)
        return Rb, Tb, Rf, Tf

    @staticmethod
    def backward(ctx, gRb, gTb, gRf, gTf):
        Rs, Ts, cnl = ctx.saved_tensors
        F_, K = Rs.shape[0], Rs.shape[1]
        gRb, gTb, gRf, gTf = (None if g is None else g.contiguous() for g in (gRb, gTb, gRf, gTf))
        gRs, gTs = torch.empty_like(Rs), torch.empty_like(Ts)
        call("hos_motion_basis_bwd", ptr(gRb), ptr(gTb), ptr(gRf), ptr(gTf), ptr(Rs), ptr(Ts), ptr(cnl), F_, K, ptr(gRs), ptr(gTs))
        return gRs, gTs, None


def motion_basis(Rs, Ts, cnl_gtfms):
    return _MotionBasis.apply(Rs, Ts, cnl_gtfms)


_COMPACT_WS = {}


def _compact_workspace(device) -> torch.Tensor:
    key = _stream_key(device)
    if key not in _COMPACT_WS:
        _COMPACT_WS[key] = torch.zeros(int(_lib.load().hos_compact_workspace_ints()), dtype=torch.int32, device=device)
    return _COMPACT_WS[key]


class _CompactRows(torch.autograd.Function):

    @staticmethod
    def forward(ctx, mask, thr, a, b):
        P = mask.numel()
        dev = mask.device
        a_sel, b_sel = torch.empty(P, 3, device=dev), torch.empty(P, 3, device=dev)
        sel = torch.empty(P, dtype=torch.int32, device=dev)
        count = torch.empty(1, dtype=torch.int32, device=dev)
        call("hos_compact_rows", ptr(mask), float(thr), ptr(a), ptr(b), P, ptr(count, torch.int32), ptr(sel, torch.int32), ptr(a_sel),
             ptr(b_sel), ptr(_compact_workspace(dev), torch.int32))
        ctx.save_for_backward(sel, count)
        ctx.mark_non_differentiable(b_sel, sel, count)
        ctx.set_materialize_grads(False)
        return a_sel, b_sel, sel, count

    @staticmethod
    def backward(ctx, g_a, *_):
        if g_a is None:
            return None, None, None, None
        sel, count = ctx.saved_tensors
        P = sel.numel()
        g = torch.empty(P, 3, device=sel.device)
        g_a = g_a.contiguous()
        call("hos_scatter_rows", ptr(g_a), ptr(sel, torch.int32), ptr(count, torch.int32), P, ptr(g))
        return None, None, g, None


def compact_rows(mask, thr: float, a, b):
    return _CompactRows.apply(mask.detach().reshape(-1).contiguous(), thr, a.reshape(-1, 3).contiguous(), b.detach().reshape(-1, 3).contiguous())


class LiveRays:

    def __init__(self, mask: torch.Tensor, thr: float = 5e-3):
        B, S = mask.shape
        dev = mask.device
        self.B, self.S = B, S
        self.ray_ids = torch.empty(B, dtype=torch.int32, device=dev)
        self.flag = torch.empty(B, dtype=torch.int32, device=dev)
        self.rows = torch.empty(1, dtype=torch.int32, device=dev)
        call("hos_select_live_rays", ptr(mask.detach().contiguous()), float(thr), B, S, ptr(self.ray_ids, torch.int32),
             ptr(self.flag, torch.int32), ptr(self.rows, torch.int32))


def select_live_rays(mask: torch.Tensor, thr: float = 5e-3) -> LiveRays:
    return LiveRays(mask, thr)


def _gather_rays_raw(src: torch.Tensor, live: LiveRays) -> torch.Tensor:
    src = src.contiguous()
    C = src.numel() // (live.B * live.S)
    dst = torch.empty(live.B * live.S, C, device=src.device)
    call("hos_gather_rays", ptr(src), ptr(live.ray_ids, torch.int32), ptr(live.rows, torch.int32), live.B, live.S, C, ptr(dst))
    return dst


def _scatter_rays_raw(src: torch.Tensor, live: LiveRays) -> torch.Tensor:
    src = src.contiguous()
    C = src.numel() // (live.B * live.S)
    dst = torch.empty(live.B * live.S, C, device=src.device)
    call("hos_scatter_rays", ptr(src), ptr(live.ray_ids, torch.int32), ptr(live.flag, torch.int32), ptr(live.rows, torch.int32),
         live.B, live.S, C, ptr(dst))
    return dst


class _GatherRays(torch.autograd.Function):
    @staticmethod
    def forward(ctx, src, live):
        ctx.live = live
        return _gather_rays_raw(src, live)

    @staticmethod
    def backward(ctx, g):
        return _scatter_rays_raw(g, ctx.live), None


class _ScatterRays(torch.autograd.Function):
    @staticmethod
    def forward(ctx, src, live):
        ctx.live = live
        return _scatter_rays_raw(src, live)

    @staticmethod
    def backward(ctx, g):
        return _gather_rays_raw(g, ctx.live), None


def gather_rays(src: torch.Tensor, live: LiveRays) -> torch.Tensor:
    return _GatherRays.apply(src, live) if (src.requires_grad and torch.is_grad_enabled()) else _gather_rays_raw(src, live)


def scatter_rays(src: torch.Tensor, live: LiveRays) -> torch.Tensor:
    return _ScatterRays.apply(src, live) if (src.requires_grad and torch.is_grad_enabled()) else _scatter_rays_raw(src, live)


_LOSS_WS = {}


def _loss_workspace(device) -> torch.Tensor:
    key = _stream_key(device)
    if key not in _LOSS_WS:
        _LOSS_WS[key] = torch.zeros(int(_lib.load().hos_train_losses_workspace_floats()), device=device)
    return _LOSS_WS[key]


class _TrainLosses(torch.autograd.Function):

    @staticmethod
    def forward(ctx, rgb, target, mse_const, mse_count, pts_prev, weights, ray_grid, fg, cam, Kin, observe, deform, n_cyc_dev,
                w_mse, w_flow, w_cycle):
        B = rgb.shape[0]
        S = 0 if pts_prev is None else pts_prev.shape[1]
        n_cyc = 0 if observe is None else observe.shape[0]
        out = torch.empty(8, device=rgb.device)
        call("hos_train_losses_fwd", ptr(rgb), ptr(target), B, float(mse_const), float(mse_count), ptr(pts_prev), ptr(weights),
             ptr(ray_grid), ptr(fg, torch.int32), ptr(cam), ptr(Kin), S, ptr(observe), ptr(deform), n_cyc, ptr(n_cyc_dev, torch.int32),
             float(w_mse), float(w_flow), float(w_cycle), ptr(_loss_workspace(rgb.device)), ptr(out))
        ctx.save_for_backward(rgb, target, pts_prev, weights, ray_grid, fg, cam, Kin, observe, deform, n_cyc_dev, out)
        ctx.cfg = (float(mse_count), float(w_mse), float(w_flow), float(w_cycle))
        parts = out.detach().clone()
        ctx.mark_non_differentiable(parts)
        ctx.set_materialize_grads(False)
        return out[0], parts

    @staticmethod
    def backward(ctx, g_total, _g_parts):
        if g_total is None:
            return (None,) * 16
        rgb, target, pts_prev, weights, ray_grid, fg, cam, Kin, observe, deform, n_cyc_dev, out = ctx.saved_tensors
        mse_count, w_mse, w_flow, w_cycle = ctx.cfg
        B = rgb.shape[0]
        S = 0 if pts_prev is None else pts_prev.shape[1]
        n_cyc = 0 if observe is None else observe.shape[0]
        need = ctx.needs_input_grad
        g_rgb = torch.empty_like(rgb) if need[0] else None
        g_pts = torch.empty_like(pts_prev) if (pts_prev is not None and need[4]) else None
        g_w = torch.empty_like(weights) if (weights is not None and need[5]) else None
        g_def = torch.empty_like(deform) if (deform is not None and need[11]) else None
        g_total = g_total.contiguous()
        call("hos_train_losses_bwd", ptr(g_total), ptr(out), ptr(rgb), ptr(target), B, mse_count, ptr(pts_prev), ptr(weights),
             ptr(ray_grid), ptr(fg, torch.int32), ptr(cam), ptr(Kin), S, ptr(observe), ptr(deform), n_cyc, ptr(n_cyc_dev, torch.int32),
             w_mse, w_flow, w_cycle, ptr(g_rgb), ptr(g_pts), ptr(g_w), ptr(g_def))
        return (g_rgb, None, None, None, g_pts, g_w, None, None, None, None, None, g_def, None, None, None, None)


def train_losses(rgb, target, mse_const=0.0, mse_count=None, pts_prev=None, weights=None, ray_grid=None, fg=None, cam_prev=None,
                 intrinsics_prev=None, observe=None, deform=None, n_cyc_dev=None, w_mse=0.2, w_flow=0.01, w_cycle=0.01):
    c = lambda t: None if t is None else t.contiguous()
    mse_count = float(rgb.numel()) if mse_count is None else mse_count
    if pts_prev is None:
        weights = ray_grid = fg = cam_prev = intrinsics_prev = None
    return _TrainLosses.apply(c(rgb), c(target).to(rgb.dtype), mse_const, mse_count, c(pts_prev), c(weights), c(ray_grid),
                              None if fg is None else fg.to(torch.int32).contiguous(), c(cam_prev), c(intrinsics_prev),
                              c(observe), c(deform), n_cyc_dev, w_mse, w_flow, w_cycle)


def _zeros_like_many(*ts):
    return zeros_many([tuple(t.shape) for t in ts], ts[0].device, ts[0].dtype)


class _UnbindFrames(torch.autograd.Function):

    @staticmethod
    def forward(ctx, x):
        ctx.shape = x.shape
        return tuple(x[f] for f in range(x.shape[0]))

    @staticmethod
    def backward(ctx, *gs):
        if all(g is None for g in gs):
            return None
        ref = next(g for g in gs if g is not None)
        if len(gs) == 1:
            return gs[0].unsqueeze(0)
        return torch.stack([torch.zeros_like(ref) if g is None else g for g in gs], 0)


def unbind_frames(x: torch.Tensor):
    return _UnbindFrames.apply(x)


class _UnbindFramesMany(torch.autograd.Function):

    @staticmethod
    def forward(ctx, *xs):
        ctx.shapes = [tuple(x.shape) for x in xs]
        ctx.set_materialize_grads(False)
        out = []
        for x in xs:
            out += [x[f] for f in range(x.shape[0])]
        return tuple(out)

    @staticmethod
    def backward(ctx, *gs):
        if all(g is None for g in gs):
            return (None,) * len(ctx.shapes)
        dev = next(g for g in gs if g is not None).device
        outs = [torch.empty(sh, device=dev) for sh in ctx.shapes] if len(ctx.shapes) > 8 else None
        sizes = [int(np.prod(sh)) for sh in ctx.shapes]
        buf = torch.empty(sum((n + 3) // 4 * 4 for n in sizes), device=dev)
        outs, o = [], 0
        for sh, n in zip(ctx.shapes, sizes):
            outs.append(buf[o:o + n].view(sh))
            o += (n + 3) // 4 * 4
        dsts, srcs, k = [], [], 0
        for x_out in outs:
            for f in range(x_out.shape[0]):
                dsts.append(x_out[f])
                g = gs[k]
                srcs.append(None if g is None else g.contiguous())
                k += 1
        copy_or_zero_n(dsts, srcs)
        return tuple(outs)


def unbind_frames_many(*xs):
    F_ = xs[0].shape[0]
    if F_ == 1 or not (torch.is_grad_enabled() and any(x.requires_grad for x in xs)):
        return [tuple(x[f] for f in range(x.shape[0])) for x in xs]
    flat = _UnbindFramesMany.apply(*xs)
    out, k = [], 0
    for x in xs:
        out.append(tuple(flat[k:k + x.shape[0]]))
        k += x.shape[0]
    return out


class _SampleWarp(torch.autograd.Function):

    @staticmethod
    def forward(ctx, vol, R, T, rays_o, rays_d, near, far, N, bmin, bscale, t_rand, K):
        z, pts, x_skel, mask = human_sample_warp(rays_o, rays_d, near, far, N, R, T, vol, bmin, bscale, t_rand, K)
        ctx.save_for_backward(vol, R, T, pts, bmin, bscale, x_skel, mask)
        ctx.K = K
        ctx.mark_non_differentiable(z, pts)
        ctx.set_materialize_grads(False)
        return z, pts, x_skel, mask

    @staticmethod
    def backward(ctx, gz, gpts, g_xskel, g_mask):
        vol, R, T, pts, bmin, bscale, x_skel, mask = ctx.saved_tensors
        K = ctx.K
        P = pts.shape[0] * pts.shape[1]
        g_vol, g_R, g_T = _zeros_like_many(vol, R, T)
        gx = zeros((P, 3), pts.device) if g_xskel is None else g_xskel.contiguous()
        gm = zeros(P, pts.device) if g_mask is None else g_mask.contiguous()
        scratch = torch.empty(P, 2, device=pts.device)
        call("hos_human_sample_warp_bwd", ptr(pts), ptr(R), ptr(T), ptr(vol), vol.shape[-1], ptr(bmin), ptr(bscale), P, K,
             ptr(gx), ptr(gm), ptr(g_vol), ptr(g_R), ptr(g_T), ptr(scratch),
             ptr(x_skel), ptr(mask))
        return g_vol, g_R, g_T, None, None, None, None, None, None, None, None, None


def human_sample_warp_ad(vol, R, T, rays_o, rays_d, near, far, N, bmin, bscale, t_rand=None, K: int = 26):
    return _SampleWarp.apply(vol.contiguous(), R.contiguous(), T.contiguous(), rays_o, rays_d, near, far, N, bmin, bscale, t_rand, K)


class _LbsForward(torch.autograd.Function):
    @staticmethod
    def forward(ctx, cnl, vol_cl, R_f, T_f, bmin, bscale, K, rows_dev):
        out = lbs_forward(cnl, R_f, T_f, vol_cl, bmin, bscale, K, rows_dev)
        ctx.save_for_backward(cnl, vol_cl, R_f, T_f, bmin, bscale, rows_dev)
        ctx.K = K
        return out

    @staticmethod
    def backward(ctx, g):
        cnl, vol_cl, R_f, T_f, bmin, bscale, rows_dev = ctx.saved_tensors
        P = cnl.shape[0]
        g_cnl = torch.empty_like(cnl)
        g_vol, g_R, g_T = _zeros_like_many(vol_cl, R_f, T_f)
        g = g.contiguous()
        call("hos_lbs_forward_bwd", ptr(cnl), ptr(R_f), ptr(T_f), ptr(vol_cl), vol_cl.shape[0], vol_cl.shape[-1], ptr(bmin),
             ptr(bscale), P, ctx.K, ptr(g), ptr(g_cnl), ptr(g_vol), ptr(g_R), ptr(g_T), ptr(rows_dev, torch.int32))
        return g_cnl, g_vol, g_R, g_T, None, None, None, None


def lbs_forward_ad(cnl, vol_cl, R_f, T_f, bmin, bscale, K: int = 26, rows_dev=None):
    return _LbsForward.apply(cnl.contiguous(), vol_cl.contiguous(), R_f.contiguous(), T_f.contiguous(), bmin, bscale, K, rows_dev)


def embed_bwd(x, band_w, num_freqs, identity, dA, colA, dB, colB, g_x, accumulate, rows_dev=None):
    call("hos_embed_bwd", ptr(x), ptr(band_w), num_freqs, int(identity), ptr(dA), dA.stride(0), colA,
         ptr(dB), 0 if dB is None else dB.stride(0), colB, x.shape[0], ptr(g_x), int(accumulate), ptr(rows_dev, torch.int32))


def embed_bwd_res(x, band_w, num_freqs, identity, dA, colA, dB, colB, res, rows_dev=None):
    g_x = torch.empty(x.shape[0], 3, device=x.device)
    call("hos_embed_bwd_res", ptr(x), ptr(band_w), num_freqs, int(identity), ptr(dA), dA.stride(0), colA,
         ptr(dB), 0 if dB is None else dB.stride(0), colB, x.shape[0], ptr(res), ptr(g_x), ptr(rows_dev, torch.int32))
    return g_x


def slice_mask(src, col0, mask_src, mcol0, width, out, rows_dev=None):
    call("hos_slice_mask", ptr(src), src.stride(0), col0, ptr(mask_src), 0 if mask_src is None else mask_src.stride(0), mcol0,
         src.shape[0], width, ptr(out), out.stride(0), ptr(rows_dev, torch.int32))


def slice_pad(src, col0, width, out, rows_dev=None):
    call("hos_slice_pad", ptr(src), src.stride(0), col0, src.shape[0], width, ptr(out), out.stride(0), ptr(rows_dev, torch.int32))


def rgbsigma_grad(g, y, dz, rows_dev=None):
    call("hos_rgbsigma_grad_rows", ptr(g), ptr(y), y.shape[0], ptr(dz), dz.stride(0), ptr(rows_dev, torch.int32))


def adam_step_dyn(p, g, m, v, hyper, beta1, beta2, eps, grad_scale=1.0, sumsq_buf=None, max_norm=0.0):
    call("hos_adam_step_dyn", ptr(p), ptr(g), ptr(m), ptr(v), p.numel(), ptr(hyper), float(beta1), float(beta2),
         float(eps), float(grad_scale), ptr(sumsq_buf), float(max_norm))


class Planes:

    __slots__ = ("t", "rows", "cols", "bits")

    def __init__(self, t: torch.Tensor, rows: int, cols: int, bits: Optional[torch.Tensor] = None):
        assert t.dim() == 4 and t.shape[2] == 2 and t.shape[3] == 32
        self.t, self.rows, self.cols, self.bits = t, rows, cols, bits

    @staticmethod
    def empty(rows: int, ld: int, dtype, device, cols: Optional[int] = None, relu_bits: bool = False):
        assert ld % 32 == 0, "planes need a leading dimension that is a multiple of 32"
        bits = torch.empty((rows + 31) // 32, (ld + 63) // 64, 64, dtype=torch.int32, device=device) if relu_bits else None
        return Planes(torch.empty(rows, ld // 32, 2, 32, dtype=dtype, device=device), rows, ld if cols is None else cols, bits)

    @staticmethod
    def from_flat(flat16: torch.Tensor, offset: int, rows: int, ld: int, cols: Optional[int] = None):
        return Planes(flat16[2 * offset:2 * (offset + rows * ld)].view(rows, ld // 32, 2, 32), rows, ld if cols is None else cols)

    @property
    def hi(self):
        return self.t[:, :, 0, :].reshape(self.rows, -1)

    @property
    def lo(self):
        return self.t[:, :, 1, :].reshape(self.rows, -1)

    @property
    def ld(self) -> int:
        return self.t.shape[1] * 32

    def float(self) -> torch.Tensor:
        return (self.t[:, :, 0, :].float() + self.t[:, :, 1, :].float()).reshape(self.rows, -1)[:, :self.cols]


def _pp(x):
    if x is None:
        return 0
    t = x.t if isinstance(x, Planes) else x
    if not (t.is_cuda and t.is_contiguous() and t.element_size() == 2):
        raise _lib.HosLibraryError("expected a contiguous 16-bit HIP planes tensor")
    return t.data_ptr()


def split_planes(src: torch.Tensor, C: Optional[int] = None, dtype=torch.float16, ldo: Optional[int] = None,
                 transposed: bool = False, ldt: Optional[int] = None, row_major: bool = True):
    R = src.shape[0]
    C = src.shape[1] if C is None else C
    dev = src.device
    out = outT = None
    if row_major:
        ldo = round_up(C, 32) if ldo is None else ldo
        out = Planes.empty(R, ldo, dtype, dev, C)
    if transposed:
        ldt = round_up(R, 32) if ldt is None else ldt
        outT = Planes.empty(C, ldt, dtype, dev, R)
    call("hos_split_planes", ptr(src), src.stride(0), R, C, 0 if dtype == torch.float16 else 1,
         _pp(out), 0 if out is None else out.ld, _pp(outT), 0 if outT is None else outT.ld)
    return out, outT


def split_planes_T_batch(mats):
    import ctypes
    outs = []
    for i0 in range(0, len(mats), 12):
        chunk = mats[i0:i0 + 12]
        planes = [Planes.empty(m.shape[1], round_up(m.shape[0], 32), torch.bfloat16, m.device, m.shape[0]) for m in chunk]
        n = len(chunk)
        src = (ctypes.c_void_p * n)(*[ptr(m) for m in chunk])
        out = (ctypes.c_void_p * n)(*[_pp(p) for p in planes])
        ia = lambda vals: (ctypes.c_int * n)(*vals)
        call("hos_split_planes_t_batch", n, src, ia([m.stride(0) for m in chunk]), ia([m.shape[0] for m in chunk]),
             ia([m.shape[1] for m in chunk]), out, ia([p.ld for p in planes]))
        outs += planes
    return outs


def split_planes2(src: torch.Tensor, C: Optional[int] = None, ld: Optional[int] = None, want16: bool = True, wantb: bool = True):
    R = src.shape[0]
    C = src.shape[1] if C is None else C
    ld = round_up(C, 32) if ld is None else ld
    p16 = Planes.empty(R, ld, torch.float16, src.device, C) if want16 else None
    pb = Planes.empty(R, ld, torch.bfloat16, src.device, C) if wantb else None
    call("hos_split_planes2", ptr(src), src.stride(0), R, C, _pp(p16), ld, _pp(pb), ld)
    return p16, pb


def linearp_fwd(A: Planes, K0: int, W: Planes, bias, M: int, N: int, relu: bool = True, Y: Optional[Planes] = None,
                Yb: Optional[Planes] = None, A1: Optional[Planes] = None, K1: int = 0, C: Optional[torch.Tensor] = None,
                epilogue: int = EPI_NONE, aux=None, aux_col: int = -1, p0: float = 0.0):
    if epilogue == EPI_RESIDUAL:
        aux_col = aux.stride(0)
    if A.t.dtype == torch.bfloat16:
        if Y is not None or W.t.dtype != torch.bfloat16 or (A1 is not None and A1.t.dtype != torch.bfloat16):
            raise _lib.HosLibraryError("linearp_fwd: bf16 operands take bf16 weights and write ONE output format (Yb)")
        _timed(f"gemmp_fwd[M={M},N={N},K={K0 + K1}]", 2.0 * M * N * (K0 + K1), lambda: call(
            "hos_linearp_fwd_b", _pp(A), A.ld, K0, _pp(A1), 0 if A1 is None else A1.ld, K1, _pp(W), W.ld, ptr(bias), M, N, int(relu),
            _pp(Yb), 0 if Yb is None else Yb.ld,
            ptr(Yb.bits, torch.int32) if (relu and Yb is not None and Yb.bits is not None) else 0,
            ptr(C), 0 if C is None else C.stride(0), epilogue, ptr(aux), aux_col, float(p0)))
        return
    _timed(f"gemmp_fwd[M={M},N={N},K={K0 + K1}]", 2.0 * M * N * (K0 + K1), lambda: call(
        "hos_linearp_fwd", _pp(A), A.ld, K0, _pp(A1), 0 if A1 is None else A1.ld, K1, _pp(W), W.ld, ptr(bias), M, N, int(relu),
        _pp(Y), 0 if Y is None else Y.ld, _pp(Yb), 0 if Yb is None else Yb.ld,
        ptr(Y.bits, torch.int32) if (relu and Y is not None and Y.bits is not None) else 0,
        ptr(C), 0 if C is None else C.stride(0), epilogue, ptr(aux), aux_col, float(p0)))


def planes_rowdot(A: Planes, K: int, w: torch.Tensor, bias: Optional[torch.Tensor], out: torch.Tensor, p0: float = 0.0, softplus: bool = True):
    M = A.rows
    fn = "hos_planes_rowdot_b" if A.t.dtype == torch.bfloat16 else "hos_planes_rowdot"
    _timed(f"planes_rowdot[M={M},K={K}]", 2.0 * M * K, lambda: call(
        fn, _pp(A), A.ld, K, ptr(w), ptr(bias), float(p0), int(softplus), M, ptr(out)))
    return out


def linearp_dgrad(dZ: Planes, WT: Planes, Npad: int, M: int, K: int, mask: Optional[Planes] = None,
                  dX: Optional[Planes] = None):
    bits = None if mask is None else mask.bits
    _timed(f"gemmp_dgrad[M={M},N={K},K={Npad}]", 2.0 * M * K * Npad, lambda: call(
        "hos_linearp_dgrad", _pp(dZ), dZ.ld, _pp(WT), WT.ld, Npad, _pp(None if bits is not None else mask),
        0 if mask is None else mask.ld, ptr(bits, torch.int32), M, K, _pp(dX), dX.ld))


_wgrad_ws = {}
WGRAD_WS_FLOATS = 16 * 1024 * 1024 + 4096


def _wgrad_workspace(device: torch.device) -> torch.Tensor:
    key = _stream_key(device)
    ws = _wgrad_ws.get(key)
    if ws is None:
        ws = torch.empty(WGRAD_WS_FLOATS, dtype=torch.float32, device=device)
        _wgrad_ws[key] = ws
    return ws


def linearp_wgrad(dZ: Planes, X: Planes, dW: torch.Tensor, db, M: int, N: int, K: int, w_col0: int = 0, splits: int = 0,
                  x_col0: int = 0, use_ws: bool = False):
    ws = _wgrad_workspace(dW.device)
    _timed(f"gemmp_wgrad[M={N},N={K},K={M}]", 2.0 * M * N * K, lambda: call(
        "hos_linearp_wgrad", _pp(dZ), dZ.ld, _pp(X), X.ld, x_col0,
        ptr(dW) + 4 * w_col0, dW.stride(0), ptr(db), M, N, K, splits, ptr(ws), ws.numel()))
```

include/hosrender.h:

```cpp
#ifndef HOSRENDER_H
#define HOSRENDER_H

#include <stdint.h>

#ifdef __cplusplus
extern "C" {
#endif

#define HOS_OK 0
#define HOS_E_ARG (-1)
#define HOS_E_ALIGN (-2)
#define HOS_E_SHAPE (-3)
#define HOS_E_NODEVICE (-4)

typedef void* hos_stream_t;

int hos_version(void);
int hos_device_count(void);
const char* hos_error_string(int code);


#define HOS_GEMM_MODE_FP32 0
#define HOS_GEMM_MODE_BF16X3 1
int hos_set_gemm_mode(int mode);
int hos_set_thread_gemm_mode(int mode);
int hos_get_gemm_mode(void);

int hos_set_range_flag(unsigned int* flag);

#define HOS_EPI_NONE 0
#define HOS_EPI_RELU 1
#define HOS_EPI_DENSITY 2
#define HOS_EPI_RGB 3
#define HOS_EPI_NERF_HEAD 4
#define HOS_EPI_SIGMOID_RELU4 5
#define HOS_EPI_RESIDUAL 6

int hos_linear_fwd(const float* A0, int lda0, int K0, const float* A1, int lda1, int K1,
                   const float* W, int ldw, const float* bias, float* C, int ldc,
                   int M, int N, int epilogue, float* aux, int aux_col, float p0, float p1,
                   const int32_t* rows_dev, hos_stream_t stream);

int hos_linear_fwd_splitk(const float* A, int lda, const float* W, int ldw, float* C, int ldc, int M, int N, int K,
                          hos_stream_t stream);
long long hos_linear_fwd_splitk_ws_floats(int M, int N, int K);
int hos_linear_fwd_splitk_det(const float* A, int lda, const float* W, int ldw, const float* bias, int relu, float* C, int ldc,
                              int M, int N, int K, float* ws, long long ws_floats, hos_stream_t stream);

int hos_linear_dgrad(const float* dY, int lddy, const float* W, int ldw, int Npad,
                     const float* Xact, int ldx, float* dX, int lddx, int M, int K,
                     int accumulate, hos_stream_t stream);

int hos_linear_wgrad(const float* dY, int lddy, const float* X, int ldx, float* dW, int ldw,
                     float* db, int M, int N, int K, int splits, hos_stream_t stream);
int hos_linear_wgrad_rows(const float* dY, int lddy, const float* X, int ldx, float* dW, int ldw,
                          float* db, int M, int N, int K, int splits, const int32_t* rows_dev, hos_stream_t stream);

int hos_linear_bwd_fused(const float* dY, int lddy, const float* X, int ldx, const float* W, int ldw,
                         float* dX, int lddx, float* dW, int lddw, float* db, int M, int N, int K,
                         int relu_mask, float* ws, int64_t ws_floats, const int32_t* rows_dev,
                         hos_stream_t stream);

int hos_mlp_bwd_defer(int on);
int hos_mlp_bwd_flush(hos_stream_t stream);
long long hos_mlp_bwd_ws_floats(int M, int N, int K, int fused);

int hos_linear_wgrad_tr(const float* dY, int lddy, const float* X, int ldx, float* dW, int lddw, float* db,
                        int M, int N, int K, float* ws, int64_t ws_floats, hos_stream_t stream);
int hos_linear_wgrad_tr_rows(const float* dY, int lddy, const float* X, int ldx, float* dW, int lddw, float* db,
                             int M, int N, int K, float* ws, int64_t ws_floats, const int32_t* rows_dev, hos_stream_t stream);

int hos_thin_linear_fwd(const float* X, int ldx, const float* W, int ldw, const float* bias, float* Y, int ldy,
                        int M, int N, int K, int epilogue, void* relu_bits, hos_stream_t stream);
int hos_thin_linear_dgrad(const float* dY, int lddy, const float* W, int ldw, int Npad, const float* mask, int ldmask,
                          const void* mask_bits, float* dX, int lddx, int M, int K, hos_stream_t stream);
int hos_thin_linear_fwd_rows(const float* X, int ldx, const float* W, int ldw, const float* bias, float* Y, int ldy,
                             int M, int N, int K, int epilogue, void* relu_bits, const int32_t* rows_dev, hos_stream_t stream);
int hos_thin_linear_dgrad_rows(const float* dY, int lddy, const float* W, int ldw, int Npad, const float* mask, int ldmask,
                               const void* mask_bits, float* dX, int lddx, int M, int K, const int32_t* rows_dev, hos_stream_t stream);

int hos_canonical_fold_pack(const float* W0, int ld0, const float* b0, const float* W5, int ld5, const float* b5,
                            const float* embed, int n_out, int nf, int ne, int nh,
                            float* W0f, float* b0f, float* W5f, float* b5f, hos_stream_t stream);
int hos_canonical_fold_unfold(const float* gW0f, const float* db0, const float* gW5f, const float* db5,
                              const float* W0, int ld0, const float* W5, int ld5, const float* embed,
                              int n_out, int nf, int ne, int nh,
                              float* gW0, float* gb0, float* gW5, float* gb5, float* g_embed, hos_stream_t stream);


int hos_split_planes(const float* src, int lds, int R, int C, int dtype, void* out, int ldo,
                     void* outT, int ldt, hos_stream_t stream);

int hos_split_planes_t_batch(int n, const float* const* src, const int* lds, const int* R, const int* C, void* const* outT,
                             const int* ldt, hos_stream_t stream);

int hos_split_planes2(const float* src, int lds, int R, int C, void* p16, int ld16, void* pb, int ldb,
                      hos_stream_t stream);

int hos_linearp_fwd(const void* A, int lda, int K0, const void* A1, int lda1, int K1, const void* W, int ldw,
                    const float* bias, int M, int N, int relu, void* Y, int ldy, void* Yb, int ldyb, void* relu_bits,
                    float* C, int ldc, int epilogue, float* aux, int aux_col, float p0, hos_stream_t stream);

int hos_planes_rowdot(const void* A, int lda, int K, const float* w, const float* bias, float p0, int softplus, int64_t M,
                      float* out, hos_stream_t stream);

int hos_linearp_fwd_b(const void* A, int lda, int K0, const void* A1, int lda1, int K1, const void* W, int ldw,
                      const float* bias, int M, int N, int relu, void* Y, int ldy, void* relu_bits,
                      float* C, int ldc, int epilogue, float* aux, int aux_col, float p0, hos_stream_t stream);
int hos_planes_rowdot_b(const void* A, int lda, int K, const float* w, const float* bias, float p0, int softplus, int64_t M,
                        float* out, hos_stream_t stream);

int hos_linearp_dgrad(const void* dZ, int lddz, const void* WT, int ldwt, int Npad, const void* mask, int ldmask,
                      const void* mask_bits, int M, int K, void* dX, int lddx, hos_stream_t stream);

int hos_linearp_wgrad(const void* dZ, int lddz, const void* X, int ldx, int x_col0, float* dW, int ldw, float* db,
                      int M, int N, int K, int splits, float* ws, long long ws_floats, hos_stream_t stream);


int hos_camera_rays(const float* Kinv9, const float* R9, const float* T3, int H, int W, float* rays_o, float* rays_d,
                    float* viewdirs, float* radii, hos_stream_t stream);

int hos_rays_aabb(const float* rays_o, float* rays_d, int64_t n, const float* bounds6, float* near, float* far,
                  unsigned char* mask, hos_stream_t stream);

int hos_frame_rays_compact(const float* Kinv9, const float* R9, const float* T3, const float* bounds6, int H, int W,
                           float* rays_o, float* rays_d, float* near, float* far, int32_t* pix, int32_t* slot,
                           int32_t* count, int32_t* ws, hos_stream_t stream);

int hos_frame_paint(const int32_t* slot, const float* rgb, int count, const float* bg01, int H, int W, float* out_f32,
                    unsigned char* out_u8, hos_stream_t stream);


int hos_raybank_index(const unsigned char* keep, int N, int H, int W, int32_t* pix, int64_t cap, int32_t* counts,
                      int64_t* offsets, int32_t* ws, hos_stream_t stream);

int hos_raybank_gather(const float* cams, const float* times, const unsigned char* images, const int32_t* pix,
                       const int64_t* offsets, const int32_t* counts, const int32_t* img_id, const int32_t* rank,
                       int64_t B, int N, int H, int W, int64_t cap, float* rays_o, float* rays_d, float* viewdirs,
                       float* radii, float* times_out, float* target, hos_stream_t stream);

int hos_raybank_frame(const float* cam16, float time, int H, int W, int64_t start, int64_t n, const unsigned char* image,
                      float* rays_o, float* rays_d, float* viewdirs, float* radii, float* times_out, float* target,
                      hos_stream_t stream);


int hos_deconv3d_col2im(const float* ycol, const float* bias, int D, int Cout, float leaky_slope, int leaky,
                        float* out, hos_stream_t stream);

int hos_deconv3d_im2col(const float* dpre, int D, int Cout, float* dycol, hos_stream_t stream);
int hos_bias_lrelu(float* y, const float* bias, long long M, int N, float leaky_slope, int leaky, hos_stream_t stream);
int hos_shard_interleave(const float* parts, int world, int M, int cs, float* out, hos_stream_t stream);

int hos_deconv3d_dpre(const float* g, const float* out, long long R, int C, float leaky_slope, int leaky, float* dpre, float* db,
                      hos_stream_t stream);
int hos_outer_accum(const float* x, int ldx, const float* dy, int lddy, float* gW, int ldw, int M, int K, int N,
                    hos_stream_t stream);
long long hos_gemv_ws_floats(int K, int N);
int hos_gemv_rowvec(const float* x, const float* W, int ldw, int K, int N, const float* bias, int bias_mod,
                    float leaky_slope, int leaky, float* ws, float* y, hos_stream_t stream);


int hos_resample(const float* sdist_prev, const float* w_prev, int n_prev, int B, int S,
                 float dilation, float anneal, const float* train_frac_dev, float anneal_slope,
                 float resample_padding, const float* u_base, const float* jitter, float jitter_scale,
                 float near_, float far_, float* sdist, float* tdist, int32_t* bin_idx,
                 hos_stream_t stream);

int hos_encode_ipe(const float* tdist, const float* rays_o, const float* rays_d, const float* radii,
                   const float* basis, const float* embed, int B, int S, float* X, int ldx,
                   hos_stream_t stream);

int hos_encode_ipe_planes(const float* tdist, const float* rays_o, const float* rays_d, const float* radii,
                          const float* basis, const float* embed, int B, int S, void* p16, void* pb, int ld,
                          hos_stream_t stream);

int hos_encode_viewdirs(const float* viewdirs, int B, int S, float* Xv, int ldx, int col0,
                        hos_stream_t stream);

int hos_alpha_weights_fwd(const float* density, const float* tdist, const float* dirs, int B, int S,
                          int opaque_background, float* weights, hos_stream_t stream);
int hos_alpha_weights_bwd(const float* g_weights, const float* density, const float* tdist,
                          const float* dirs, int B, int S, int opaque_background, float* g_density,
                          hos_stream_t stream);

int hos_volrender_fwd(const float* rgbs, const float* weights, int B, int S, float bg, float* rgb,
                      hos_stream_t stream);
int hos_volrender_bwd(const float* g_rgb, const float* rgbs, const float* weights, int B, int S,
                      float bg, float* g_rgbs, float* g_weights, hos_stream_t stream);

int hos_interlevel_fwd(const float* c, const float* w, const float* cp, const float* wp, int B,
                       int Sc, int Sp, float* loss_ray, int32_t* idx_lo, int32_t* idx_hi,
                       hos_stream_t stream);
int hos_interlevel_bwd(const float* c, const float* w, const float* cp, const float* wp, int B,
                       int Sc, int Sp, float scale, float* g_wp, hos_stream_t stream);
int hos_distortion_fwd(const float* t, const float* w, int B, int S, float* loss_ray,
                       hos_stream_t stream);
int hos_distortion_bwd(const float* t, const float* w, int B, int S, float scale, float* g_w,
                       hos_stream_t stream);

int hos_head_grad(const float* g_density, const float* density, const float* g_rgb, const float* rgb,
                  int P, float rgb_padding, float* dz_density, int ld_dd, int col_dd,
                  float* dz_rgb, int ld_dr, hos_stream_t stream);


int hos_human_sample_warp(const float* rays_o, const float* rays_d, const float* near_, const float* far_,
                          const float* t_vals, const float* t_rand, const float* R, const float* T,
                          const float* vol, int V, const float* bbox_min, const float* bbox_scale,
                          int B, int N, int K, float* z_vals, float* pts, float* x_skel, float* mask,
                          hos_stream_t stream);

int hos_lbs_forward(const float* cnl_pts, const float* R_fwd, const float* T_fwd, const float* vol_cl,
                    int V, int CL, const float* bbox_min, const float* bbox_scale, int64_t P, int K,
                    float* x_deform, const int32_t* rows_dev, hos_stream_t stream);

int hos_embed_hannw(const float* x, const float* band_w, int num_freqs, const float* cond, int cond_size,
                    int64_t P, float* E, int lde, float* PE, int ldpe, const int32_t* rows_dev, hos_stream_t stream);

int hos_embed_fourier(const float* x, int num_freqs, const float* state, int state_size, int64_t P,
                      float* E, int lde, float* E2, int lde2, hos_stream_t stream);
int hos_embed_fourier_rows(const float* x, int num_freqs, const float* state, int state_size, int64_t P,
                           float* E, int lde, float* E2, int lde2, const int32_t* rows_dev, hos_stream_t stream);

int hos_human_sample_warp_bwd(const float* pts, const float* R, const float* T, const float* vol, int V,
                              const float* bbox_min, const float* bbox_scale, int64_t P, int K,
                              const float* g_x_skel, const float* g_mask, float* g_vol, float* g_R, float* g_T,
                              float* scratch, const float* fwd_x_skel, const float* fwd_mask, hos_stream_t stream);
int hos_lbs_forward_bwd(const float* cnl_pts, const float* R_fwd, const float* T_fwd, const float* vol_cl,
                        int V, int CL, const float* bbox_min, const float* bbox_scale, int64_t P, int K,
                        const float* g_x_deform, float* g_cnl, float* g_vol_cl, float* g_R, float* g_T,
                        const int32_t* rows_dev, hos_stream_t stream);
int hos_embed_bwd(const float* x, const float* band_w, int num_freqs, int identity, const float* dA, int lda,
                  int colA, const float* dB, int ldb, int colB, int64_t P, float* g_x, int accumulate,
                  const int32_t* rows_dev, hos_stream_t stream);
int hos_slice_mask(const float* src, int lds, int col0, const float* mask_src, int ldm, int mcol0, int64_t P,
                   int width, float* out, int ldo, const int32_t* rows_dev, hos_stream_t stream);
int hos_slice_pad(const float* src, int lds, int col0, int64_t P, int width, float* out, int ldo,
                  const int32_t* rows_dev, hos_stream_t stream);
int hos_rgbsigma_grad(const float* g_rgbsigma, const float* rgbsigma, int64_t P, float* dz, int ldz,
                      hos_stream_t stream);
int hos_rgbsigma_grad_rows(const float* g_rgbsigma, const float* rgbsigma, int64_t P, float* dz, int ldz,
                           const int32_t* rows_dev, hos_stream_t stream);

int hos_raw2outputs_fwd(const float* rgbs, int rgb_ld, const float* sigma, int sigma_ld, const float* z_vals,
                        const float* rays_d, const float* mask, const float* bgcolor, float last_dist,
                        int B, int S, float* rgb, float* acc, float* weights, float* depth, hos_stream_t stream);
int hos_raw2outputs_bwd(const float* g_rgb, const float* g_weights, const float* rgbs, int rgb_ld,
                        const float* sigma, int sigma_ld, const float* z_vals, const float* rays_d,
                        const float* mask, const float* bgcolor, float last_dist, int B, int S,
                        float* g_rgbs, int g_rgb_ld, float* g_sigma, int g_sigma_ld, float* g_mask,
                        hos_stream_t stream);

int hos_merge_composite_fwd(const float* bkg_tdist, const float* bkg_rgb, const float* bkg_density,
                            const float* human_rgbsigma, const float* newsmpl_pts, const float* pts_mask,
                            const float* rays_o_bkg, const float* rays_d_bkg, const float* smpl_to_world,
                            const int32_t* tiny_d_flag, int B, int Sb, int Sh, float thre_fg,
                            float* rgb, int32_t* idx_fg, int32_t* total_order, float* human_weights_sorted,
                            float* z_human, hos_stream_t stream);
int hos_merge_composite_maps_fwd(const float* bkg_tdist, const float* bkg_rgb, const float* bkg_density,
                                 const float* human_rgbsigma, const float* newsmpl_pts, const float* pts_mask,
                                 const float* rays_o_bkg, const float* rays_d_bkg, const float* smpl_to_world,
                                 const int32_t* tiny_d_flag, int B, int Sb, int Sh, float thre_fg,
                                 float* rgb, int32_t* idx_fg, int32_t* total_order,
                                 float* acc, float* depth, float* rgb_human, float* acc_human,
                                 float* rgb_bkg, float* acc_bkg, hos_stream_t stream);
int hos_merge_composite_bwd(const float* g_rgb, const float* g_human_weights_sorted,
                            const float* bkg_tdist, const float* bkg_rgb, const float* bkg_density,
                            const float* human_rgbsigma, const float* newsmpl_pts, const float* pts_mask,
                            const float* rays_o_bkg, const float* rays_d_bkg, const float* smpl_to_world,
                            const int32_t* tiny_d_flag, int B, int Sb, int Sh, float thre_fg,
                            float* g_bkg_rgb, float* g_bkg_density, float* g_human_rgbsigma, float* g_pts_mask,
                            hos_stream_t stream);

long long hos_pose_refine_saved_floats(void);
long long hos_pose_refine_workspace_floats(void);
int hos_pose_refine_fwd(const float* posevec, const float* Rs, const float* Ts, const float* const* weights14,
                        int F, int K, int width, float* Rs_out, float* Ts_out, float* saved, hos_stream_t stream);
int hos_pose_refine_bwd(const float* g_Rs_out, const float* g_Ts_out, const float* posevec, const float* Rs,
                        const float* saved, const float* const* weights14, float* const* grads14, int F, int K, int width,
                        float* workspace, hos_stream_t stream);

int hos_motion_basis_fwd(const float* dst_Rs, const float* dst_Ts, const float* cnl_gtfms, int F, int K,
                         float* R_bwd, float* T_bwd, float* R_fwd, float* T_fwd, hos_stream_t stream);
int hos_motion_basis_bwd(const float* g_R_bwd, const float* g_T_bwd, const float* g_R_fwd, const float* g_T_fwd,
                         const float* dst_Rs, const float* dst_Ts, const float* cnl_gtfms, int F, int K,
                         float* g_dst_Rs, float* g_dst_Ts, hos_stream_t stream);

long long hos_mlp_chain_weight_bytes(void);
long long hos_mlp_chain_aux_floats(void);
int hos_mlp_chain_pack(const float* const* weights7, const int* ldw7, const float* const* biases7, void* chain_planes,
                       float* aux, hos_stream_t stream);
int hos_mlp_chain_pack_fold(const float* const* weights7, const int* ldw7, const float* const* biases7, const float* cond,
                            int ncond, int nfeat, void* chain_planes, float* aux, float* w0h, hos_stream_t stream);
int hos_mlp_chain_unfold_grad(const float* gw0h, const float* db, const float* cond, int ncond, int nfeat,
                              float* gW0, int ldw, float* gb0, hos_stream_t stream);
int hos_mlp_chain128_fwd(const float* E, int lde, const float* PE, int ldpe, const float* x, const void* chain_planes,
                         const float* aux, float* const* acts6, int ldact, float* xyz, int64_t P,
                         const int32_t* rows_dev, hos_stream_t stream);

int hos_mlp_chain_bwd_steps(int cfg);
long long hos_mlp_chain_bwd_image_bytes(int cfg, int step);
long long hos_mlp_chain_bwd_ws_floats(int cfg, int M);
int hos_mlp_chain_bwd_pack(int n, const int* cfg, const int* step, const float* const* W, const int* ldw, const int* N, const int* K,
                           void* const* image, hos_stream_t stream);
int hos_mlp_chain_bwd(int cfg, const float* dZ, int lddz, int M, const int32_t* rows_dev, const float* const* X, const int* ldx,
                      const void* const* images, float* const* dXout, const int* lddx, float* const* dW, const int* lddw,
                      float* const* db, const int* N, const int* K, float* ws, int64_t ws_floats, hos_stream_t stream);

long long hos_compact_workspace_ints(void);
int hos_compact_rows(const float* mask, float thr, const float* src_a, const float* src_b, int64_t P, int32_t* count,
                     int32_t* sel, float* out_a, float* out_b, int32_t* workspace, hos_stream_t stream);
int hos_scatter_rows(const float* src, const int32_t* sel, const int32_t* count, int64_t P, float* dst, hos_stream_t stream);

int hos_select_live_rays(const float* mask, float thr, int B, int S, int32_t* ray_ids, int32_t* flag, int32_t* rows_live,
                         hos_stream_t stream);
int hos_gather_rays(const float* src, const int32_t* ray_ids, const int32_t* rows_live, int B, int S, int C, float* dst,
                    hos_stream_t stream);
int hos_scatter_rays(const float* src, const int32_t* ray_ids, const int32_t* flag, const int32_t* rows_live, int B, int S,
                     int C, float* dst, hos_stream_t stream);

long long hos_train_losses_workspace_floats(void);
int hos_train_losses_fwd(const float* rgb, const float* target, long long n_rays, float mse_const, float mse_count,
                         const float* pts_prev, const float* weights, const float* ray_grid, const int32_t* fg,
                         const float* cam_prev, const float* intrinsics_prev, int S,
                         const float* observe, const float* deform, long long n_cyc, const int32_t* n_cyc_dev,
                         float w_mse, float w_flow, float w_cycle, float* workspace, float* out8,
                         hos_stream_t stream);
int hos_train_losses_bwd(const float* g_total, const float* out8, const float* rgb, const float* target, long long n_rays,
                         float mse_count, const float* pts_prev, const float* weights, const float* ray_grid,
                         const int32_t* fg, const float* cam_prev, const float* intrinsics_prev, int S,
                         const float* observe, const float* deform, long long n_cyc, const int32_t* n_cyc_dev,
                         float w_mse, float w_flow, float w_cycle,
                         float* g_rgb, float* g_pts_prev, float* g_weights, float* g_deform, hos_stream_t stream);

int hos_sumsq(const float* g, int64_t n, float* sumsq, hos_stream_t stream);
int hos_adam_step(float* p, const float* g, float* m, float* v, int64_t n, float lr, float beta1,
                  float beta2, float eps, int step, float grad_scale, const float* sumsq,
                  float max_norm, hos_stream_t stream);

int hos_adam_step_dyn(float* p, const float* g, float* m, float* v, int64_t n, const float* hyper,
                      float beta1, float beta2, float eps, float grad_scale, const float* sumsq,
                      float max_norm, hos_stream_t stream);

int hos_rowdot_lrelu_fwd(const float* x, const float* W, int ldw, const float* b, int N, int K, float slope, float* y,
                         hos_stream_t stream);
int hos_rowdot_lrelu_bwd(const float* g, const float* y, const float* x, const float* W, int ldw, int N, int K, float slope,
                         float* gW, int ldgw, float* gb, float* gx, hos_stream_t stream);
int hos_volume_softmax_fwd(const float* z, const float* prior, int C, long long V3, float* vol, hos_stream_t stream);
int hos_volume_softmax_bwd(const float* g_vol, const float* vol, int C, long long V3, float* gz, hos_stream_t stream);
int hos_volume_channel_last(const float* vol, int Kb, long long V3, float* vol_cl, hos_stream_t stream);
int hos_volume_pair_bwd(const float* g_vol, const float* g_cl, int C, int Kb, long long V3, float* g, hos_stream_t stream);
int hos_copy_or_zero_n(int n, float* const* dst, const float* const* src, const long long* count, hos_stream_t stream);
int hos_debug_stamp(long long* buf, int slot, hos_stream_t stream);
int hos_clear_last_error(void);
int hos_add_n(int n, const float* const* src, long long count, float* out, hos_stream_t stream);
int hos_any_abs_below(const float* x, long long n, float thr, int32_t* flag, hos_stream_t stream);
int hos_state_embed_grad(const float* db, const float* W, int ldw, int c0, int N, int E, float* gb, float* g_embed, hos_stream_t stream);
int hos_embed_bwd_res(const float* x, const float* band_w, int num_freqs, int identity, const float* dA, int lda, int colA,
                      const float* dB, int ldb, int colB, int64_t P, const float* res, float* g_x, const int32_t* rows_dev,
                      hos_stream_t stream);
int hos_head_grad_padded(const float* g_density, const float* density, const float* g_rgb, const float* rgb, int P, float rgb_padding,
                         float* dz_density, int ld_dd, int col_dd, float* dz_rgb, int ld_dr, hos_stream_t stream);
int hos_sumsq_blocks(void);
int hos_sumsq_partials(int n, const float* const* g, const long long* count, float* partial, hos_stream_t stream);
int hos_adam_multi(int n, float* const* p, const float* const* g, float* const* m, float* const* v, const long long* count,
                   const float* const* hyper, const float* lr, int step, float beta1, float beta2, float eps, float grad_scale,
                   const float* partial, float max_norm, const unsigned int* guard, unsigned int* skipped, hos_stream_t stream);
int hos_adam_lazy_prepare(int n, const float* const* g, const long long* count, float* const* state, float beta1, float beta2,
                          const unsigned int* guard, hos_stream_t stream);
int hos_adam_multi_lazy(int n, float* const* p, const float* const* g, float* const* m, float* const* v, const long long* count,
                        const float* const* hyper, const float* const* lazy, const int* lazy_row, const float* lr, int step, float beta1, float beta2,
                        float eps, float grad_scale, const float* partial, float max_norm, const unsigned int* guard,
                        unsigned int* skipped, hos_stream_t stream);

int hos_lpips_prep(const float* x01, int64_t n_pixels, float* out, hos_stream_t stream);
int hos_im2col3x3(const float* in, int NI, int H, int W, int C, float* col, int ld, hos_stream_t stream);
int hos_col2im3x3(const float* dcol, int ld, int NI, int H, int W, int C, const float* relu_src, float* dx, hos_stream_t stream);
int hos_maxpool2x2_fwd(const float* in, int NI, int H, int W, int C, float* out, hos_stream_t stream);
int hos_maxpool2x2_bwd(const float* g_out, const float* in, int NI, int H, int W, int C, float* g_in, hos_stream_t stream);
int hos_lpips_head_fwd(const float* feats, const float* lin_w, int Np, int HW, int C, float coef, float* part, hos_stream_t stream);
int hos_lpips_head_bwd(const float* feats, const float* lin_w, int Np, int HW, int C, float coef, const float* gscale,
                       int accumulate, float* g_feats, hos_stream_t stream);
int hos_lpips_finish(const float* part, int Np, float* out, hos_stream_t stream);
int hos_lpips_part_floats(int Np);
int hos_bias_relu(float* y, const float* bias, int64_t M, int N, hos_stream_t stream);
int hos_unpack_patches_fwd(const float* rgb, const int32_t* idx, const float* bgcolor, float bg_scale, int64_t n_pixels, float* img,
                           hos_stream_t stream);
int hos_unpack_patches_bwd(const float* g_img, const int32_t* idx, int64_t n_pixels, float s0, float s1, float s2, float* g_rgb,
                           hos_stream_t stream);

int hos_stage1_loss_fwd(const float* rgb, const float* target, int B, const float* inter0, const float* inter1, int Sc, const float* dist,
                        float m_data, float m_inter, float m_dist, float charb_padding, float* out4, hos_stream_t stream);
int hos_stage1_loss_bwd(const float* rgb, const float* target, int B, int Sc, const float* fwd_out4, const float* gout, float m_data,
                        float m_inter, float m_dist, float charb_padding, float* g_rgb, float* g_inter, float* g_dist, hos_stream_t stream);

#ifdef __cplusplus
}
#endif
#endif
```

Measured before the change: 141,200.

## Batch ray gathers into one kernel and restrict warp backward to live rays

Ray gather and scatter are rewritten to work one wave per ray with vectorized copies. Several tensors can now be gathered in a single launch, and scatter uses a precomputed per-ray rank instead of an indexed loop. The human sample-warp backward can also take a live-ray selection and skip dead rays, avoiding gradient work and volume atomics for background samples. This adds plumbing through autograd nodes, where the selection is attached to the backward node, and changes the C API signatures.

```diff
diff --git a/hosnerf_amd/_lib.py b/hosnerf_amd/_lib.py
--- a/hosnerf_amd/_lib.py
+++ b/hosnerf_amd/_lib.py
@@ -100,6 +100,7 @@
     "hos_embed_fourier": [_P, _I, _P, _I, _L, _P, _I, _P, _I, _P],
     "hos_embed_fourier_rows": [_P, _I, _P, _I, _L, _P, _I, _P, _I, _P, _P],
     "hos_human_sample_warp_bwd": [_P, _P, _P, _P, _I, _P, _P, _L, _I, _P, _P, _P, _P, _P, _P, _P, _P, _P],
+    "hos_human_sample_warp_bwd_rays": [_P, _P, _P, _P, _I, _P, _P, _L, _I, _P, _P, _P, _P, _P, _P, _P, _P, _P, _P, _I, _P],
     "hos_lbs_forward_bwd": [_P, _P, _P, _P, _I, _I, _P, _P, _L, _I, _P, _P, _P, _P, _P, _P, _P],
     "hos_embed_bwd": [_P, _P, _I, _I, _P, _I, _I, _P, _I, _I, _L, _P, _I, _P, _P],
     "hos_slice_mask": [_P, _I, _I, _P, _I, _I, _L, _I, _P, _I, _P, _P],
@@ -125,9 +126,9 @@
     "hos_compact_workspace_ints": [],
     "hos_compact_rows": [_P, _F, _P, _P, _L, _P, _P, _P, _P, _P, _P],
     "hos_scatter_rows": [_P, _P, _P, _L, _P, _P],
-    "hos_select_live_rays": [_P, _F, _I, _I, _P, _P, _P, _P],
-    "hos_gather_rays": [_P, _P, _P, _I, _I, _I, _P, _P],
-    "hos_scatter_rays": [_P, _P, _P, _P, _I, _I, _I, _P, _P],
+    "hos_select_live_rays": [_P, _F, _I, _I, _P, _P, _P, _P, _P],
+    "hos_gather_rays_multi": [_I, _P, _P, _P, _P, _P, _I, _I, _P],
+    "hos_scatter_rays": [_P, _P, _P, _I, _I, _I, _P, _P],
     "hos_pose_refine_saved_floats": [],
     "hos_pose_refine_fwd": [_P, _P, _P, _P, _I, _I, _I, _P, _P, _P, _P],
     "hos_pose_refine_workspace_floats": [],
diff --git a/hosnerf_amd/csrc/hos_compact.hip b/hosnerf_amd/csrc/hos_compact.hip
--- a/hosnerf_amd/csrc/hos_compact.hip
+++ b/hosnerf_amd/csrc/hos_compact.hip
@@ -119,7 +119,7 @@
 }
 
 __global__ __launch_bounds__(LT) void live_scan_kernel(const int* __restrict__ flag, int B, int S, int* __restrict__ ray_ids,
-                                                       int* __restrict__ rows_live) {
+                                                       int* __restrict__ rank, int* __restrict__ rows_live) {
     __shared__ int wsum[LT / 64];
     __shared__ int total;
     const int t = threadIdx.x, lane = t & 63, wave = t >> 6;
@@ -134,77 +134,116 @@
     int pos = incl - c;
     for (int w = 0; w < wave; ++w) pos += wsum[w];
     if (t == LT - 1) { total = pos + c; *rows_live = (pos + c) * S; }
-    for (int k = 0; k < per; ++k)
-        if (r0 + k < B && flag[r0 + k] != 0) ray_ids[pos++] = r0 + k;
+    for (int k = 0; k < per; ++k) {
+        if (r0 + k >= B) break;
+        const bool f = flag[r0 + k] != 0;
+        rank[r0 + k] = f ? pos : -1;
+        if (f) ray_ids[pos++] = r0 + k;
+    }
     __syncthreads();
     const int n = total;
     for (int i = n + t; i < B; i += LT) ray_ids[i] = -1;
 }
 
-__global__ __launch_bounds__(256) void gather_rays_kernel(const float* __restrict__ src, const int* __restrict__ ray_ids,
-                                                         const int* __restrict__ rows_live, long P, int S, int C, float* __restrict__ dst) {
-    const long total = P * C;
-    const long live = min((long)*rows_live, P) * C;
-    for (long i = (long)blockIdx.x * blockDim.x + threadIdx.x; i < total; i += (long)gridDim.x * blockDim.x) {
-        float v = 0.f;
-        if (i < live) {
-            const long j = i / C;
-            const int c = (int)(i - j * C);
-            const long ray = ray_ids[j / S];
-            v = src[(ray * S + j % S) * C + c];
+constexpr int RAYSETS = 4;
+typedef float f32x2 __attribute__((ext_vector_type(2)));
+typedef float f32x4 __attribute__((ext_vector_type(4)));
+
+struct RayCopySet {
+    const float* src[RAYSETS];
+    float* dst[RAYSETS];
+    int n[RAYSETS];
+    int vec[RAYSETS];
+};
+
+template <typename V>
+__device__ inline void ray_copy(const float* __restrict__ s, float* __restrict__ d, int n, int lane) {
+    const int m = n / (int)(sizeof(V) / sizeof(float));
+    V* dv = reinterpret_cast<V*>(d);
+    if (s != nullptr) {
+        const V* sv = reinterpret_cast<const V*>(s);
+        for (int k = lane; k < m; k += 128) {
+            const bool two = k + 64 < m;
+            const V a = sv[k];
+            V b = V(0.f);
+            if (two) b = sv[k + 64];
+            dv[k] = a;
+            if (two) dv[k + 64] = b;
         }
-        dst[i] = v;
-    }
-}
-
-__global__ __launch_bounds__(256) void scatter_rays_kernel(const float* __restrict__ src, const int* __restrict__ ray_ids,
-                                                          const int* __restrict__ flag, const int* __restrict__ rows_live, long P, int S,
-                                                          int C, float* __restrict__ dst) {
-    const long total = P * C;
-    const long live = min((long)*rows_live, P) * C;
-    for (long i = (long)blockIdx.x * blockDim.x + threadIdx.x; i < total; i += (long)gridDim.x * blockDim.x) {
-        const long j = i / C;
-        const int c = (int)(i - j * C);
-        if (i < live) {
-            const long ray = ray_ids[j / S];
-            dst[(ray * S + j % S) * C + c] = src[i];
-        }
-        if (flag[j / S] == 0) dst[i] = 0.f;
-    }
-}
-
-inline int rays_grid(long total) {
-    long b = (total + 255) / 256;
-    return (int)(b > 4096 ? 4096 : (b < 1 ? 1 : b));
-}
-
-}
-
-extern "C" int hos_select_live_rays(const float* mask, float thr, int B, int S, int32_t* ray_ids, int32_t* flag, int32_t* rows_live,
-                                    hos_stream_t stream) {
-    if (!mask || !ray_ids || !flag || !rows_live || B <= 0 || S <= 0) return HOS_E_ARG;
+    } else {
+        for (int k = lane; k < m; k += 64) dv[k] = V(0.f);
+    }
+}
+
+template <bool SCATTER>
+__global__ __launch_bounds__(256) void move_rays_kernel(RayCopySet a, const int* __restrict__ index, const int* __restrict__ flag,
+                                                       const int* __restrict__ rows_live, int B, int S) {
+    const int lane = threadIdx.x & 63;
+    const int r = blockIdx.x * 4 + (threadIdx.x >> 6);
+    if (r >= B) return;
+    const bool has = SCATTER ? flag[r] != 0 : (long)r * S < (long)*rows_live;
+    int from = -1;
+    if (has) from = __builtin_amdgcn_readfirstlane(index[r]);
+    if (from < 0 || from >= B) from = -1;
+    const float* src = nullptr;
+    float* dst = nullptr;
+    int n = 0, vec = 1;
+#pragma unroll
+    for (int t = 0; t < RAYSETS; ++t)
+        if (t == (int)blockIdx.y) { src = a.src[t]; dst = a.dst[t]; n = a.n[t]; vec = a.vec[t]; }
+    const float* s = from >= 0 ? src + (size_t)from * n : nullptr;
+    float* d = dst + (size_t)r * n;
+    if (vec == 4) ray_copy<f32x4>(s, d, n, lane);
+    else if (vec == 2) ray_copy<f32x2>(s, d, n, lane);
+    else ray_copy<float>(s, d, n, lane);
+}
+
+inline int ray_vec(const float* src, float* dst, long n) {
+    const uintptr_t bits = reinterpret_cast<uintptr_t>(src) | reinterpret_cast<uintptr_t>(dst) | (uintptr_t)(n * sizeof(float));
+    return (bits & 15) == 0 ? 4 : ((bits & 7) == 0 ? 2 : 1);
+}
+
+inline int ray_set(int n, const float* const* src, const int32_t* C, float* const* dst, int S, RayCopySet* t) {
+    if (n <= 0 || n > RAYSETS || !src || !C || !dst) return HOS_E_ARG;
+    for (int k = 0; k < n; ++k) {
+        if (!src[k] || !dst[k] || C[k] <= 0) return HOS_E_ARG;
+        const long len = (long)S * C[k];
+        if (len > 0x7fffffffL) return HOS_E_SHAPE;
+        t->src[k] = src[k]; t->dst[k] = dst[k]; t->n[k] = (int)len; t->vec[k] = ray_vec(src[k], dst[k], len);
+    }
+    return HOS_OK;
+}
+
+}
+
+extern "C" int hos_select_live_rays(const float* mask, float thr, int B, int S, int32_t* ray_ids, int32_t* flag, int32_t* rank,
+                                    int32_t* rows_live, hos_stream_t stream) {
+    if (!mask || !ray_ids || !flag || !rank || !rows_live || B <= 0 || S <= 0) return HOS_E_ARG;
     if ((long long)B * S > 0x7fffffffLL) return HOS_E_SHAPE;
     hipStream_t s = static_cast<hipStream_t>(stream);
     hipLaunchKernelGGL(live_flag_kernel, dim3((unsigned)((B + 3) / 4)), dim3(256), 0, s, mask, thr, B, S, flag);
-    hipLaunchKernelGGL(live_scan_kernel, dim3(1), dim3(LT), 0, s, flag, B, S, ray_ids, rows_live);
-    return hos_launch_status();
-}
-
-extern "C" int hos_gather_rays(const float* src, const int32_t* ray_ids, const int32_t* rows_live, int B, int S, int C, float* dst,
-                               hos_stream_t stream) {
-    if (!src || !ray_ids || !rows_live || !dst || B <= 0 || S <= 0 || C <= 0) return HOS_E_ARG;
-    const long P = (long)B * S;
-    hipLaunchKernelGGL(gather_rays_kernel, dim3(rays_grid(P * C)), dim3(256), 0, static_cast<hipStream_t>(stream), src, ray_ids, rows_live,
-                       P, S, C, dst);
-    return hos_launch_status();
-}
-
-extern "C" int hos_scatter_rays(const float* src, const int32_t* ray_ids, const int32_t* flag, const int32_t* rows_live, int B, int S,
-                                int C, float* dst, hos_stream_t stream) {
-    if (!src || !ray_ids || !flag || !rows_live || !dst || B <= 0 || S <= 0 || C <= 0) return HOS_E_ARG;
-    const long P = (long)B * S;
-    hipLaunchKernelGGL(scatter_rays_kernel, dim3(rays_grid(P * C)), dim3(256), 0, static_cast<hipStream_t>(stream), src, ray_ids, flag,
-                       rows_live, P, S, C, dst);
+    hipLaunchKernelGGL(live_scan_kernel, dim3(1), dim3(LT), 0, s, flag, B, S, ray_ids, rank, rows_live);
+    return hos_launch_status();
+}
+
+extern "C" int hos_gather_rays_multi(int n, const float* const* src, const int32_t* C, float* const* dst, const int32_t* ray_ids,
+                                     const int32_t* rows_live, int B, int S, hos_stream_t stream) {
+    if (!ray_ids || !rows_live || B <= 0 || S <= 0) return HOS_E_ARG;
+    RayCopySet t{};
+    if (const int e = ray_set(n, src, C, dst, S, &t)) return e;
+    hipLaunchKernelGGL(move_rays_kernel<false>, dim3((unsigned)((B + 3) / 4), (unsigned)n), dim3(256), 0, static_cast<hipStream_t>(stream), t,
+                       ray_ids, static_cast<const int*>(nullptr), rows_live, B, S);
+    return hos_launch_status();
+}
+
+extern "C" int hos_scatter_rays(const float* src, const int32_t* rank, const int32_t* flag, int B, int S, int C, float* dst,
+                                hos_stream_t stream) {
+    if (!rank || !flag || B <= 0 || S <= 0) return HOS_E_ARG;
+    RayCopySet t{};
+    const int32_t c = C;
+    if (const int e = ray_set(1, &src, &c, &dst, S, &t)) return e;
+    hipLaunchKernelGGL(move_rays_kernel<true>, dim3((unsigned)((B + 3) / 4), 1u), dim3(256), 0, static_cast<hipStream_t>(stream), t, rank,
+                       flag, static_cast<const int*>(nullptr), B, S);
     return hos_launch_status();
 }
 
diff --git a/hosnerf_amd/csrc/hos_human.hip b/hosnerf_amd/csrc/hos_human.hip
--- a/hosnerf_amd/csrc/hos_human.hip
+++ b/hosnerf_amd/csrc/hos_human.hip
@@ -425,25 +425,35 @@
     const float* __restrict__ vol, int V, const float* __restrict__ bbox_min, const float* __restrict__ bbox_scale,
     long P, int K, const float* __restrict__ g_xskel, const float* __restrict__ g_mask,
     float* __restrict__ g_vol, float* __restrict__ g_R, float* __restrict__ g_T, float* __restrict__ aux,
-    const float* __restrict__ fwd_xskel, const float* __restrict__ fwd_mask) {
+    const float* __restrict__ fwd_xskel, const float* __restrict__ fwd_mask, const int* __restrict__ ray_ids,
+    const int* __restrict__ rows_live, int S) {
     __shared__ float sR[KMAX * 9], sT[KMAX * 3], sB[6], sAcc[KMAX * 12];
     for (int i = threadIdx.x; i < K * 9; i += blockDim.x) sR[i] = R[i];
     for (int i = threadIdx.x; i < K * 3; i += blockDim.x) sT[i] = T[i];
     for (int i = threadIdx.x; i < K * 12; i += blockDim.x) sAcc[i] = 0.f;
     if (threadIdx.x < 3) { sB[threadIdx.x] = bbox_min[threadIdx.x]; sB[3 + threadIdx.x] = bbox_scale[threadIdx.x]; }
     __syncthreads();
-    const long nchunks = (P + 255) / 256;
+    const long Pn = ray_ids != nullptr ? min(P, (long)*rows_live) : P;
+    const long nchunks = (Pn + 255) / 256;
     for (long chunk = blockIdx.x; chunk < nchunks; chunk += gridDim.x) {
-    const long p = chunk * 256 + threadIdx.x;
-    const bool live = p < P;
-    const long pp = live ? p : P - 1;
+    const long j = chunk * 256 + threadIdx.x;
     const int lane = threadIdx.x & 63;
-    const float px = pts[pp * 3], py = pts[pp * 3 + 1], pz = pts[pp * 3 + 2];
+    bool live = j < Pn;
+    long p = j;
+    if (ray_ids != nullptr && live) {
+        const int slot = (int)j / S;
+        const long ray = ray_ids[slot];
+        live = ray >= 0 && (ray + 1) * S <= P;
+        p = ray * S + ((int)j - slot * S);
+    }
+    const bool wave_on = __ballot(live) != 0;
+    const long pp = live ? p : 0;
+    const float px = live ? pts[pp * 3] : 0.f, py = live ? pts[pp * 3 + 1] : 0.f, pz = live ? pts[pp * 3 + 2] : 0.f;
     const size_t V3 = (size_t)V * V * V;
     float wsum, xs, ys, zs;
     if (fwd_xskel != nullptr) {
-        wsum = fwd_mask[pp];
-        xs = fwd_xskel[pp * 3]; ys = fwd_xskel[pp * 3 + 1]; zs = fwd_xskel[pp * 3 + 2];
+        wsum = live ? fwd_mask[pp] : 0.f;
+        xs = live ? fwd_xskel[pp * 3] : 0.f; ys = live ? fwd_xskel[pp * 3 + 1] : 0.f; zs = live ? fwd_xskel[pp * 3 + 2] : 0.f;
     } else {
         float ax = 0.f, ay = 0.f, az = 0.f;
         wsum = 0.f;
@@ -471,7 +481,7 @@
         for (int ii = 0; ii < 16; ++ii) {
             const int i = i0 + ii;
             float gq[3] = {0.f, 0.f, 0.f};
-            if (i < K) {
+            if (i < K && wave_on) {
                 const float* r = sR + i * 9;
                 const float qx = (r[0] * px + r[1] * py + r[2] * pz) + sT[i * 3 + 0];
                 const float qy = (r[3] * px + r[4] * py + r[5] * pz) + sT[i * 3 + 1];
@@ -521,7 +531,7 @@
     const float* __restrict__ pts, const float* __restrict__ R, const float* __restrict__ T, int V,
     const float* __restrict__ bbox_min, const float* __restrict__ bbox_scale, long P,
     const float* __restrict__ g_xskel, const float* __restrict__ g_mask, const float* __restrict__ aux,
-    float* __restrict__ g_vol) {
+    float* __restrict__ g_vol, const int* __restrict__ ray_ids, const int* __restrict__ rows_live, int S) {
     extern __shared__ float s_gvol[];
     const int i = blockIdx.y;
     const int V3 = V * V * V;
@@ -534,15 +544,27 @@
     __syncthreads();
     const int lane = threadIdx.x & 63;
     const long span = (long)gridDim.x * blockDim.x;
-    const long p_end = ((P + span - 1) / span) * span;
-    for (long p = (long)blockIdx.x * blockDim.x + threadIdx.x; p < p_end; p += span) {
-        const bool live = p < P;
-        const long pp = live ? p : P - 1;
-        const float px = pts[pp * 3], py = pts[pp * 3 + 1], pz = pts[pp * 3 + 2];
+    const long Pn = ray_ids != nullptr ? min(P, (long)*rows_live) : P;
+    const long p_end = ((Pn + span - 1) / span) * span;
+    const long j_first = (long)blockIdx.x * blockDim.x + threadIdx.x;
+    int slot = 0, rem = 0, dq = 0, dr = 0;
+    if (ray_ids != nullptr) { slot = (int)j_first / S; rem = (int)j_first - slot * S; dq = (int)span / S; dr = (int)span - dq * S; }
+    for (long j = j_first; j < p_end; j += span, slot += dq, rem += dr) {
+        if (rem >= S) { rem -= S; ++slot; }
+        bool live = j < Pn;
+        long p = j;
+        if (ray_ids != nullptr && live) {
+            const long ray = ray_ids[slot];
+            live = ray >= 0 && (ray + 1) * S <= P;
+            p = ray * S + rem;
+        }
+        const long pp = live ? p : 0;
+        const float px = live ? pts[pp * 3] : 0.f, py = live ? pts[pp * 3 + 1] : 0.f, pz = live ? pts[pp * 3 + 2] : 0.f;
         const float qx = (r[0] * px + r[1] * py + r[2] * pz) + tt[0];
         const float qy = (r[3] * px + r[4] * py + r[5] * pz) + tt[1];
         const float qz = (r[6] * px + r[7] * py + r[8] * pz) + tt[2];
-        const float gw = ((g_xskel[pp * 3] * qx + g_xskel[pp * 3 + 1] * qy + g_xskel[pp * 3 + 2] * qz) - aux[pp * 2 + 1]) / aux[pp * 2] + g_mask[pp];
+        float gw = 0.f;
+        if (live) gw = ((g_xskel[pp * 3] * qx + g_xskel[pp * 3 + 1] * qy + g_xskel[pp * 3 + 2] * qz) - aux[pp * 2 + 1]) / aux[pp * 2] + g_mask[pp];
         const float gx = (qx - bm[0]) * bs[0] - 1.f, gy = (qy - bm[1]) * bs[1] - 1.f, gz = (qz - bm[2]) * bs[2] - 1.f;
         const float ix = ((gx + 1.f) / 2.f) * (float)(V - 1), iy = ((gy + 1.f) / 2.f) * (float)(V - 1), iz = ((gz + 1.f) / 2.f) * (float)(V - 1);
         const float fx = floorf(ix), fy = floorf(iy), fz = floorf(iz);
@@ -861,14 +883,17 @@
 
 }
 
-extern "C" int hos_human_sample_warp_bwd(const float* pts, const float* R, const float* T, const float* vol, int V,
-                                         const float* bbox_min, const float* bbox_scale, int64_t P, int K,
-                                         const float* g_x_skel, const float* g_mask, float* g_vol, float* g_R,
-                                         float* g_T, float* scratch, const float* fwd_x_skel, const float* fwd_mask,
-                                         hos_stream_t stream) {
+extern "C" int hos_human_sample_warp_bwd_rays(const float* pts, const float* R, const float* T, const float* vol, int V,
+                                              const float* bbox_min, const float* bbox_scale, int64_t P, int K,
+                                              const float* g_x_skel, const float* g_mask, float* g_vol, float* g_R,
+                                              float* g_T, float* scratch, const float* fwd_x_skel, const float* fwd_mask,
+                                              const int32_t* ray_ids, const int32_t* rows_live, int S, hos_stream_t stream) {
     if (!pts || !R || !T || !vol || !bbox_min || !bbox_scale || !g_x_skel || !g_mask || !g_vol || !g_R || !g_T || P <= 0)
         return HOS_E_ARG;
     if (K <= 0 || K > KMAX || V < 2) return HOS_E_SHAPE;
+    if ((ray_ids != nullptr) != (rows_live != nullptr) || (ray_ids && (S <= 0 || P % S != 0))) return HOS_E_ARG;
+    if (ray_ids && P > 0x7fffffffLL - (1 << 20)) return HOS_E_SHAPE;
+    if (!ray_ids) S = 1;
     hipStream_t s = static_cast<hipStream_t>(stream);
     const long sw_chunks = (P + 255) / 256;
     const dim3 grid((unsigned)(sw_chunks < persist_grid ? sw_chunks : persist_grid));
@@ -876,7 +901,8 @@
     const bool split = scratch != nullptr && vol_bytes <= 128 * 1024 && P >= 8192;
     hipLaunchKernelGGL(human_sample_warp_bwd_kernel, grid, dim3(256), 0, s, pts, R, T, vol, V, bbox_min, bbox_scale, (long)P, K,
                        g_x_skel, g_mask, split ? (float*)nullptr : g_vol, g_R, g_T, split ? scratch : (float*)nullptr,
-                       (fwd_x_skel && fwd_mask) ? fwd_x_skel : (const float*)nullptr, (fwd_x_skel && fwd_mask) ? fwd_mask : (const float*)nullptr);
+                       (fwd_x_skel && fwd_mask) ? fwd_x_skel : (const float*)nullptr, (fwd_x_skel && fwd_mask) ? fwd_mask : (const float*)nullptr,
+                       ray_ids, rows_live, S);
     if (split) {
         static bool attr_set = false;
         if (!attr_set) {
@@ -887,9 +913,18 @@
         }
         const int nb = 256 / K > 0 ? 256 / K : 1;
         hipLaunchKernelGGL(sample_warp_vol_scatter_kernel, dim3(nb, K), dim3(1024), vol_bytes, s, pts, R, T, V, bbox_min,
-                           bbox_scale, (long)P, g_x_skel, g_mask, scratch, g_vol);
+                           bbox_scale, (long)P, g_x_skel, g_mask, scratch, g_vol, ray_ids, rows_live, S);
     }
     return hos_launch_status();
+}
+
+extern "C" int hos_human_sample_warp_bwd(const float* pts, const float* R, const float* T, const float* vol, int V,
+                                         const float* bbox_min, const float* bbox_scale, int64_t P, int K,
+                                         const float* g_x_skel, const float* g_mask, float* g_vol, float* g_R,
+                                         float* g_T, float* scratch, const float* fwd_x_skel, const float* fwd_mask,
+                                         hos_stream_t stream) {
+    return hos_human_sample_warp_bwd_rays(pts, R, T, vol, V, bbox_min, bbox_scale, P, K, g_x_skel, g_mask, g_vol, g_R, g_T, scratch,
+                                          fwd_x_skel, fwd_mask, nullptr, nullptr, 0, stream);
 }
 
 extern "C" int hos_lbs_forward_bwd(const float* cnl_pts, const float* R_fwd, const float* T_fwd, const float* vol_cl,
diff --git a/hosnerf_amd/human_nerf.py b/hosnerf_amd/human_nerf.py
--- a/hosnerf_amd/human_nerf.py
+++ b/hosnerf_amd/human_nerf.py
@@ -749,9 +749,10 @@
                                                                 far[sl].contiguous(), N, bmin, bscale, tr, K)
                 live = ops.select_live_rays(mask.detach().view(-1, N))
                 rows_live = live.rows
-                x_c = ops.gather_rays(x_skel.reshape(-1, 3), live)
-                mask_c = ops.gather_rays(mask.detach().reshape(-1, 1), live).view(-1)
-                pts_c = ops.gather_rays(pts.detach().reshape(-1, 3), live)
+                ops.warp_backward_rays(x_skel, live)
+                x_c, mask_c, pts_c = ops.gather_rays_multi([x_skel.reshape(-1, 3), mask.detach().reshape(-1, 1),
+                                                            pts.detach().reshape(-1, 3)], live)
+                mask_c = mask_c.view(-1)
                 cnl = _NonRigidFn.apply(self._token, self, "nr", x_c, cond, band_w, rows_live)
                 n_use = 1 + int(flow) + int(with_cycle)
                 cnl_uses = list(ops.fanout(cnl, n_use))
diff --git a/hosnerf_amd/ops.py b/hosnerf_amd/ops.py
--- a/hosnerf_amd/ops.py
+++ b/hosnerf_amd/ops.py
@@ -1310,42 +1310,48 @@
         dev = mask.device
         self.B, self.S = B, S
         self.ray_ids = torch.empty(B, dtype=torch.int32, device=dev)
+        self.rank = torch.empty(B, dtype=torch.int32, device=dev)
         self.flag = torch.empty(B, dtype=torch.int32, device=dev)
         self.rows = torch.empty(1, dtype=torch.int32, device=dev)
         call("hos_select_live_rays", ptr(mask.detach().contiguous()), float(thr), B, S, ptr(self.ray_ids, torch.int32),
-             ptr(self.flag, torch.int32), ptr(self.rows, torch.int32))
+             ptr(self.flag, torch.int32), ptr(self.rank, torch.int32), ptr(self.rows, torch.int32))
 
 
 def select_live_rays(mask: torch.Tensor, thr: float = 5e-3) -> LiveRays:
     return LiveRays(mask, thr)
 
 
-def _gather_rays_raw(src: torch.Tensor, live: LiveRays) -> torch.Tensor:
-    src = src.contiguous()
-    C = src.numel() // (live.B * live.S)
-    dst = torch.empty(live.B * live.S, C, device=src.device)
-    call("hos_gather_rays", ptr(src), ptr(live.ray_ids, torch.int32), ptr(live.rows, torch.int32), live.B, live.S, C, ptr(dst))
-    return dst
+def _gather_rays_raw(srcs, live: LiveRays):
+    import ctypes
+    srcs = [t.contiguous() for t in srcs]
+    Cs = [t.numel() // (live.B * live.S) for t in srcs]
+    dsts = [torch.empty(live.B * live.S, C, device=t.device) for t, C in zip(srcs, Cs)]
+    call("hos_gather_rays_multi", len(srcs), _table([ptr(t) for t in srcs]), _table(Cs, ctypes.c_int32), _table([ptr(t) for t in dsts]),
+         ptr(live.ray_ids, torch.int32), ptr(live.rows, torch.int32), live.B, live.S)
+    return dsts
 
 
 def _scatter_rays_raw(src: torch.Tensor, live: LiveRays) -> torch.Tensor:
     src = src.contiguous()
     C = src.numel() // (live.B * live.S)
     dst = torch.empty(live.B * live.S, C, device=src.device)
-    call("hos_scatter_rays", ptr(src), ptr(live.ray_ids, torch.int32), ptr(live.flag, torch.int32), ptr(live.rows, torch.int32),
-         live.B, live.S, C, ptr(dst))
+    call("hos_scatter_rays", ptr(src), ptr(live.rank, torch.int32), ptr(live.flag, torch.int32), live.B, live.S, C, ptr(dst))
     return dst
 
 
 class _GatherRays(torch.autograd.Function):
-    @staticmethod
-    def forward(ctx, src, live):
+
+    @staticmethod
+    def forward(ctx, src, live, *extra):
         ctx.live = live
-        return _gather_rays_raw(src, live)
-
-    @staticmethod
-    def backward(ctx, g):
-        return _scatter_rays_raw(g, ctx.live), None
+        out = _gather_rays_raw([src, *extra], live)
+        ctx.mark_non_differentiable(*out[1:])
+        ctx.set_materialize_grads(False)
+        return tuple(out)
+
+    @staticmethod
+    def backward(ctx, g, *_):
+        return (None if g is None else _scatter_rays_raw(g, ctx.live), None) + (None,) * (len(_))
 
 
 class _ScatterRays(torch.autograd.Function):
@@ -1356,11 +1362,19 @@
 
     @staticmethod
     def backward(ctx, g):
-        return _gather_rays_raw(g, ctx.live), None
+        return _gather_rays_raw([g], ctx.live)[0], None
+
+
+def gather_rays_multi(srcs, live: LiveRays):
+    if any(t.requires_grad for t in srcs[1:]):
+        raise _lib.HosLibraryError("gather_rays_multi: only the first tensor is differentiable")
+    if srcs[0].requires_grad and torch.is_grad_enabled():
+        return list(_GatherRays.apply(srcs[0], live, *srcs[1:]))
+    return _gather_rays_raw(srcs, live)
 
 
 def gather_rays(src: torch.Tensor, live: LiveRays) -> torch.Tensor:
-    return _GatherRays.apply(src, live) if (src.requires_grad and torch.is_grad_enabled()) else _gather_rays_raw(src, live)
+    return gather_rays_multi([src], live)[0]
 
 
 def scatter_rays(src: torch.Tensor, live: LiveRays) -> torch.Tensor:
@@ -1514,15 +1528,29 @@
     def backward(ctx, gz, gpts, g_xskel, g_mask):
         vol, R, T, pts, bmin, bscale, x_skel, mask = ctx.saved_tensors
         K = ctx.K
-        P = pts.shape[0] * pts.shape[1]
+        S = pts.shape[1]
+        P = pts.shape[0] * S
         g_vol, g_R, g_T = _zeros_like_many(vol, R, T)
         gx = zeros((P, 3), pts.device) if g_xskel is None else g_xskel.contiguous()
         gm = zeros(P, pts.device) if g_mask is None else g_mask.contiguous()
         scratch = torch.empty(P, 2, device=pts.device)
-        call("hos_human_sample_warp_bwd", ptr(pts), ptr(R), ptr(T), ptr(vol), vol.shape[-1], ptr(bmin), ptr(bscale), P, K,
+        live = getattr(ctx, "live_rays", None)
+        call("hos_human_sample_warp_bwd_rays", ptr(pts), ptr(R), ptr(T), ptr(vol), vol.shape[-1], ptr(bmin), ptr(bscale), P, K,
              ptr(gx), ptr(gm), ptr(g_vol), ptr(g_R), ptr(g_T), ptr(scratch),
-             ptr(x_skel), ptr(mask))
+             ptr(x_skel), ptr(mask), ptr(None if live is None else live.ray_ids, torch.int32),
+             ptr(None if live is None else live.rows, torch.int32), S)
         return g_vol, g_R, g_T, None, None, None, None, None, None, None, None, None
+
+
+def warp_backward_rays(x_skel: torch.Tensor, live: LiveRays):
+    node = x_skel.grad_fn
+    if node is None:
+        return
+    if not isinstance(node, _SampleWarp._backward_cls):
+        raise _lib.HosLibraryError("warp_backward_rays: x_skel is not an output of human_sample_warp_ad")
+    if live.B * live.S * 3 != x_skel.numel():
+        raise _lib.HosLibraryError("warp_backward_rays: the selection does not match the warp's rays")
+    node.live_rays = live
 
 
 def human_sample_warp_ad(vol, R, T, rays_o, rays_d, near, far, N, bmin, bscale, t_rand=None, K: int = 26):
diff --git a/include/hosrender.h b/include/hosrender.h
--- a/include/hosrender.h
+++ b/include/hosrender.h
@@ -225,6 +225,11 @@
                               const float* bbox_min, const float* bbox_scale, int64_t P, int K,
                               const float* g_x_skel, const float* g_mask, float* g_vol, float* g_R, float* g_T,
                               float* scratch, const float* fwd_x_skel, const float* fwd_mask, hos_stream_t stream);
+int hos_human_sample_warp_bwd_rays(const float* pts, const float* R, const float* T, const float* vol, int V,
+                                   const float* bbox_min, const float* bbox_scale, int64_t P, int K,
+                                   const float* g_x_skel, const float* g_mask, float* g_vol, float* g_R, float* g_T,
+                                   float* scratch, const float* fwd_x_skel, const float* fwd_mask,
+                                   const int32_t* ray_ids, const int32_t* rows_live, int S, hos_stream_t stream);
 int hos_lbs_forward_bwd(const float* cnl_pts, const float* R_fwd, const float* T_fwd, const float* vol_cl,
                         int V, int CL, const float* bbox_min, const float* bbox_scale, int64_t P, int K,
                         const float* g_x_deform, float* g_cnl, float* g_vol_cl, float* g_R, float* g_T,
@@ -311,12 +316,12 @@
                      int32_t* sel, float* out_a, float* out_b, int32_t* workspace, hos_stream_t stream);
 int hos_scatter_rows(const float* src, const int32_t* sel, const int32_t* count, int64_t P, float* dst, hos_stream_t stream);
 
-int hos_select_live_rays(const float* mask, float thr, int B, int S, int32_t* ray_ids, int32_t* flag, int32_t* rows_live,
-                         hos_stream_t stream);
-int hos_gather_rays(const float* src, const int32_t* ray_ids, const int32_t* rows_live, int B, int S, int C, float* dst,
-                    hos_stream_t stream);
-int hos_scatter_rays(const float* src, const int32_t* ray_ids, const int32_t* flag, const int32_t* rows_live, int B, int S,
-                     int C, float* dst, hos_stream_t stream);
+int hos_select_live_rays(const float* mask, float thr, int B, int S, int32_t* ray_ids, int32_t* flag, int32_t* rank,
+                         int32_t* rows_live, hos_stream_t stream);
+int hos_gather_rays_multi(int n, const float* const* src, const int32_t* C, float* const* dst, const int32_t* ray_ids,
+                          const int32_t* rows_live, int B, int S, hos_stream_t stream);
+int hos_scatter_rays(const float* src, const int32_t* rank, const int32_t* flag, int B, int S, int C, float* dst,
+                     hos_stream_t stream);
 
 long long hos_train_losses_workspace_floats(void);
 int hos_train_losses_fwd(const float* rgb, const float* target, long long n_rays, float mse_const, float mse_count,
```

Measured after the change: 141,800, median of 6. No clear change (+0.4%).
